# buckbaskin/parakeet_slam

Measured on AMD Instinct MI355X. Metric: particle*landmark EKF updates/sec (whole filter step), higher is better.
Workload: dtype f64

## Files before the change

### parakeet_slam_amd/csrc/pk_api.hip

```cpp
#include <hip/hip_runtime.h>

#include <cmath>
#include <cstdarg>
#include <cstdio>
#include <cstring>
#include <new>
#include <string>
#include <vector>

#include "../../include/parakeet_slam.h"
#include "pk_kernels.hpp"

using namespace pk;

extern "C" {
int pk_download_landmarks(pk_filter* f, int64_t p0, int64_t p1, double* means, double* covs, int32_t* counts);
int pk_upload_landmarks(pk_filter* f, int64_t p0, int64_t p1, const double* means, const double* covs, const int32_t* counts);
}

#ifdef PK_STAMPS
namespace pk { void debug_read_stamps(unsigned long long* out, bool reset); void debug_read_fused_stamps(unsigned long long* out, bool reset); void debug_read_regs_stamps(unsigned long long* out, bool reset); void debug_read_pub_stamps(unsigned long long* out, bool reset); void debug_read_pub_wave_stamps(unsigned long long* out, bool reset); }
#endif

namespace {

thread_local std::string g_last_error;

int fail(int code, const char* fmt, ...) {
  char buf[512];
  va_list ap;
  va_start(ap, fmt);
  vsnprintf(buf, sizeof(buf), fmt, ap);
  va_end(ap);
  g_last_error = buf;
  return code;
}

#define PK_HIP(call)                                                                         \
  do {                                                                                       \
    hipError_t e_ = (call);                                                                  \
    if (e_ != hipSuccess) {                                                                  \
      (void)hipGetLastError();                                                               \
      return fail(e_ == hipErrorOutOfMemory ? PK_ERR_NOMEM : PK_ERR_HIP, "%s failed: %s (%s:%d)", #call, \
                  hipGetErrorString(e_), __FILE__, __LINE__);                                \
    }                                                                                        \
  } while (0)

#define PK_LAUNCH_CHECK(what)                                                                \
  do {                                                                                       \
    hipError_t e_ = hipGetLastError();                                                       \
    if (e_ != hipSuccess)                                                                    \
      return fail(PK_ERR_HIP, "%s: a kernel launch failed: %s", what, hipGetErrorString(e_)); \
  } while (0)

struct TimedSpan {
  int slot;
  hipEvent_t a, b;
};

}

struct AssocLaunch {
  bool fused = false;
  bool regs = false;
  bool retry = false;
  bool big = false;
  BlobGrid grid{};
  int n9 = 0;
  const unsigned char* tables = nullptr;
  bool fast = false;
  const double* blobs = nullptr;
  const double* dir = nullptr;
  const double* exact = nullptr;
  const unsigned short* order = nullptr;
};

struct pk_filter {
  int device = 0;
  hipStream_t own_stream = nullptr;
  hipStream_t stream = nullptr;
  DeviceState d{};
  NoiseD qt{0.1, 0.1, 0.0, 0.0, 0.1, 0.0, 0.1};
  double qt16[16] = {0.1, 0, 0, 0, 0, 0.1, 0, 0, 0, 0, 0.1, 0, 0, 0, 0, 0.1};
  bool qt_dense = false;
  bool dense = false;
  std::vector<double> dense_staged;
  bool map_loaded = false;
  bool src_identity = true;
  int64_t nblocks = 0;
  int64_t device_bytes = 0;
  double* z_dev = nullptr;
  unsigned char* scan_dev = nullptr;
  size_t scan_cap = 0;
  bool gmax_fused = false;
// ... 17 lines not shown
  int64_t bal_loop_keep = -1;
  int assoc_kernel = 0;
  int assoc_dup = 1;
  struct Staged {
    bool valid = false;
    int B = 0;
    unsigned char* st = nullptr;
    int slot = 0;
    BlobGrid g{};
    int n9 = 0;
    bool use_grid = false;
    size_t tab_bytes = 0;
    bool uploaded = false;
  } staged;
  int route = PK_ROUTE_NONE;
  int upload_kernel = 1;
  int fused_step = 1;
  unsigned* bcnt_dev = nullptr;
  uint4* brec_dev = nullptr;
  int64_t bcand_cap = 0;
  int cand_lists = 1;
  int64_t loop_lo = INT64_MIN, loop_hi = INT64_MAX;
  uint4* cand_dev = nullptr;
  int regs_step = 1;
  int pub_step = 1;
  bool flag_folded = false;
  int pub_small = -1;
  int duo_park_limit = -1;
  int duo_on = 0;
  int pub_entry_limit = 0;
  uint4* erec_dev = nullptr;
  uint4* erec_dev2 = nullptr;
  unsigned* binfo_dev = nullptr;
  unsigned char* npass_dev = nullptr;
  unsigned* unm_dev = nullptr;
  int unm_words = 0;
  int64_t unm_cap = 0;
  bool grow_bits = false;
  uint4* prim_dev = nullptr;
  float4* gate4_dev = nullptr;
  uint4* far_dev = nullptr;
  int far_prune = 1;
  unsigned* glist_dev = nullptr;
  struct Split {
    bool active = false;
    AssocLaunch al;
    CandTable cand;
    int B = 0;
    bool reset = false;
  } split;
  bool adopt_local_done = false;
  int pub_ecap = 0;
  int split_reserve_cus = 16;
  int regs_retry = 1;
  int regs_warm = 1;
  int fast_observe = 1;
  uint4* sweep_results = nullptr;
  size_t sweep_cap = 0;
  unsigned* retry_seen = nullptr;
  int64_t retry_rows_min = 0;
  FastHandoff fh{};
  int64_t fh_cap_l = 0, fh_cap_b = 0;
  static constexpr int kRing = 8;
  unsigned char* stage[kRing] = {nullptr};
  hipEvent_t stage_done[kRing] = {nullptr};
  uint64_t upload_seq = 0;
  uint64_t slot_seq[kRing] = {0};
  uint64_t event_seq[kRing] = {0};
  size_t stage_cap = 0;
  int stage_next = 0;
  double* partial = nullptr;
  double* gmax = nullptr;
  double* clocal = nullptr;
  double* totals = nullptr;
  double* offsets = nullptr;
  double* sum = nullptr;
  double* out4 = nullptr;
  double* pose_part = nullptr;
  bool pose_part_ok = false;
  GrowState grow{};
  bool grow_on = false;
  int32_t* anc = nullptr;
  unsigned char* slot_tmp = nullptr;
  uint32_t timing_mask = 0;
  int timing_stride = 1;
  int64_t timing_seen[PK_T_COUNT] = {0};
  std::vector<TimedSpan> pending;
  std::vector<hipEvent_t> pool;
  double ms[PK_T_COUNT] = {0};
  int64_t launches[PK_T_COUNT] = {0};
};

namespace {

template <typename T>
int dev_alloc(pk_filter* f, T** p, size_t n) {
  *p = nullptr;
  if (n == 0) n = 1;
  hipError_t e = hipMalloc((void**)p, n * sizeof(T));
  if (e != hipSuccess) {
    (void)hipGetLastError();
    return fail(PK_ERR_NOMEM, "hipMalloc of %zu bytes failed: %s", n * sizeof(T), hipGetErrorString(e));
  }
  f->device_bytes += (int64_t)(n * sizeof(T));
  return PK_OK;
}

struct Span {
  pk_filter* f;
  int slot;
  hipEvent_t a = nullptr, b = nullptr;
  Span(pk_filter* f_, int slot_) : f(f_), slot(slot_) {
    if (!((f->timing_mask >> slot_) & 1u)) return;
    if (f->timing_seen[slot_]++ % f->timing_stride != 0) return;
    a = take();
    b = take();
    if (a) (void)hipEventRecord(a, f->stream);
  }
  hipEvent_t take() {
    if (!f->pool.empty()) {
      hipEvent_t e = f->pool.back();
      f->pool.pop_back();
      return e;
    }
    hipEvent_t e = nullptr;
    if (hipEventCreate(&e) != hipSuccess) return nullptr;
    return e;
  }
  ~Span() {
    if (!a || !b) return;
    (void)hipEventRecord(b, f->stream);
    f->pending.push_back(TimedSpan{slot, a, b});
  }
};

int drain_timings(pk_filter* f) {
  if (f->pending.empty()) return PK_OK;
  PK_HIP(hipStreamSynchronize(f->stream));
  for (auto& t : f->pending) {
    float ms = 0.f;
    if (hipEventElapsedTime(&ms, t.a, t.b) == hipSuccess) {
      f->ms[t.slot] += ms;
      f->launches[t.slot] += 1;
    }
    f->pool.push_back(t.a);
    f->pool.push_back(t.b);
  }
  f->pending.clear();
  return PK_OK;
}

int use_device(pk_filter* f) {
  PK_HIP(hipSetDevice(f->device));
  return PK_OK;
}

constexpr size_t kCtlBytes = 8 * kGmaxKeys + 64;
int ensure_scan_capacity(pk_filter* f, size_t bytes) {
  if (bytes <= f->scan_cap) return PK_OK;
  PK_HIP(hipStreamSynchronize(f->stream));
  if (f->scan_dev) (void)hipFree(f->scan_dev);
  f->scan_dev = nullptr;
  f->scan_cap = 0;
  const size_t cap = bytes + bytes / 4 + 4096;
  int rc;
  if ((rc = dev_alloc(f, &f->scan_dev, cap))) return rc;
// ... 390 lines not shown
      out->exact = reinterpret_cast<const double*>(f->scan_dev + o_exact);
      const size_t cs_b = ((size_t)(g.ncell + 1) * 2 + 15) & ~(size_t)15;
      out->order = reinterpret_cast<const unsigned short*>(f->scan_dev + o_tab + cs_b + (size_t)B * 16 + (size_t)n9 * 2);
      return PK_OK;
    }
    if (want_fast && !onepass_only && !finalize && f->fast_observe && B > 0 &&
        (sweep ? observe_sweep_plan(f->d, B).grid > 0 : observe_fast_lds_bytes(B) <= kMaxDynLds)) {
      const int slots = (sweep && (B >= 3000 || f->fast_observe == 3)) ? kSweepSlots : kFastSlots;
      if ((rc = ensure_handoff(f, B, slots))) return rc;
      f->fh.slots = slots;
      fh = f->fh;
      fh.n_flagged = ctl_n_flagged(f);
    }
    Span t(f, PK_T_ASSOC);
    CandTable cand;
    if (fh.lmpass && f->cand_lists && f->d.lay.L < 65535) {
      if (!f->cand_dev && (rc = dev_alloc(f, &f->cand_dev, ((size_t)f->d.lay.Lp + kCandSpare) * 3))) return rc;
      launch_summary_partials(f->stream, f->d, f->partial, f->out4);
      launch_candidates(f->stream, f->d, B, reinterpret_cast<const double*>(f->scan_dev + o_exact), 0, f->cand_dev, ctl_cand_over(f),
                        nullptr, nullptr, nullptr, 2 * kCandSlots, f->out4);
      cand.rec = f->cand_dev;
      cand.over = ctl_cand_over(f);
      cand.slots = 2 * kCandSlots;
    }
    launch_assoc_grid(f->stream, f->d, B, g, n9, f->scan_dev + o_tab, reinterpret_cast<const double*>(f->scan_dev + o_exact),
                      f->ids_dev, finalize, fh, cand);
    if (out) {
      out->fast = fh.lmpass != nullptr;
      out->exact = reinterpret_cast<const double*>(f->scan_dev + o_exact);
      const size_t cs_b = ((size_t)(g.ncell + 1) * 2 + 15) & ~(size_t)15;
      out->order = reinterpret_cast<const unsigned short*>(f->scan_dev + o_tab + cs_b + (size_t)B * 16 + (size_t)n9 * 2);
    }
    return PK_OK;
  }
  if (assoc_brute_lds_bytes(B) > kMaxDynLds)
    return fail(PK_ERR_UNSUPPORTED,
                "maximum-likelihood association of %d blobs: neither the colour-grid tables nor the brute-force kernel's "
                "%zu bytes of per-blob state fit the workgroup's %zu bytes of LDS", B, assoc_brute_lds_bytes(B), (size_t)kMaxDynLds);
  Span t(f, PK_T_ASSOC);
  launch_assoc_brute(f->stream, f->d, blobs_dev, dir_dev, B, f->ids_dev);
  return PK_OK;
}

int classify_covariance(const double* cov, int l) {
  double scale = 0.0;
  for (int i = 0; i < 25; ++i) {
    if (!std::isfinite(cov[i])) return fail(PK_ERR_INVALID, "landmark %d: covariance not finite", l + 1);
    if (i % 6 == 0) scale = fmax(scale, fabs(cov[i]));
  }
  const double tol = 1e-9 * (scale > 0 ? scale : 1.0);
  for (int i = 0; i < 2; ++i)
    for (int j = 2; j < 5; ++j)
      if (fabs(cov[i * 5 + j]) > 1e-14 * scale || fabs(cov[j * 5 + i]) > 1e-14 * scale) return 1;
  for (int i = 0; i < 5; ++i)
    for (int j = i + 1; j < 5; ++j)
      if (fabs(cov[i * 5 + j] - cov[j * 5 + i]) > tol) return 1;
  return 0;
}

int check_block_diagonal(const double* cov, int l) {
  double scale = 0.0;
  for (int i = 0; i < 5; ++i) scale = fmax(scale, fabs(cov[i * 6]));
  if (!(scale >= 0.0) || !std::isfinite(scale))
    return fail(PK_ERR_INVALID, "landmark %d: covariance diagonal is not finite", l + 1);
  const double tol = 1e-9 * (scale > 0 ? scale : 1.0);
  for (int i = 0; i < 2; ++i)
    for (int j = 2; j < 5; ++j)
      if (fabs(cov[i * 5 + j]) > 1e-14 * scale || fabs(cov[j * 5 + i]) > 1e-14 * scale)
        return fail(PK_ERR_UNSUPPORTED,
                    "landmark %d: covariance couples position and colour (entry [%d][%d]); the compact "
                    "device layout holds xy 2x2 (+) rgb 3x3 only",
                    l + 1, i, j);
  for (int i = 0; i < 5; ++i)
    for (int j = i + 1; j < 5; ++j) {
      if (!std::isfinite(cov[i * 5 + j])) return fail(PK_ERR_INVALID, "landmark %d: covariance not finite", l + 1);
      if (fabs(cov[i * 5 + j] - cov[j * 5 + i]) > tol)
        return fail(PK_ERR_UNSUPPORTED, "landmark %d: covariance is not symmetric", l + 1);
    }
  return PK_OK;
}

int relayout(pk_filter* f, bool dense, bool keep) {
  if (f->dense == dense) return PK_OK;
  int rc;
  DeviceState& d = f->d;
  const MapLayout old = d.lay;
  const MapLayout neu = MapLayout::make(old.L, sizeof(double), dense ? kDenseFields : (int)F_COUNT_FIELDS);
  const int64_t P = d.P;
  const int L = old.L;
  std::vector<double> means, covs;
  std::vector<int32_t> counts;
  if (keep && L > 0) {
    if ((rc = materialise(f))) return rc;
    if (!dense)
      return fail(PK_ERR_STATE, "relayout: a dense map cannot be folded back into the compact layout");
    try {
      means.resize((size_t)P * L * 5);
      covs.resize((size_t)P * L * 25);
      counts.resize((size_t)P * L);
    } catch (const std::bad_alloc&) {
      return fail(PK_ERR_NOMEM, "relayout: no host memory to stage %lld x %d landmarks for the layout conversion", (long long)P, L);
    }
    if ((rc = pk_download_landmarks(f, 0, P, means.data(), covs.data(), counts.data()))) return rc;
  }
  PK_HIP(hipStreamSynchronize(f->stream));
  for (int i = 0; i < 2; ++i) {
    if (d.map[i]) (void)hipFree(d.map[i]);
    d.map[i] = nullptr;
    f->device_bytes -= (int64_t)((size_t)P * old.slot_bytes);
  }
  if (f->slot_tmp) (void)hipFree(f->slot_tmp);
  f->slot_tmp = nullptr;
  f->device_bytes -= (int64_t)old.slot_bytes;
  d.lay = neu;
  f->dense = dense;
  d.alt = nullptr;
  for (int i = 0; i < 2; ++i) {
    if ((rc = dev_alloc(f, &d.map[i], (size_t)P * neu.slot_bytes))) return rc;
    PK_HIP(hipMemsetAsync(d.map[i], 0, (size_t)P * neu.slot_bytes, f->stream));
  }
  if ((rc = dev_alloc(f, &f->slot_tmp, neu.slot_bytes))) return rc;
  launch_iota(f->stream, d.src[0], P);
  launch_iota(f->stream, d.src[1], P);
  f->src_identity = true;
  d.mcur = 0;
  if (keep && L > 0) {
    const bool was_loaded = f->map_loaded;
    f->map_loaded = true;
    rc = pk_upload_landmarks(f, 0, P, means.data(), covs.data(), counts.data());
    f->map_loaded = was_loaded;
    if (rc) return rc;
  }
  PK_HIP(hipStreamSynchronize(f->stream));
  return PK_OK;
}

}

extern "C" {

int pk_abi_version(void) { return PK_ABI_VERSION; }

const char* pk_status_string(int status) {
  switch (status) {
    case PK_OK: return "ok";
    case PK_ERR_INVALID: return "invalid argument";
    case PK_ERR_HIP: return "HIP runtime error";
    case PK_ERR_STATE: return "invalid call order";
    case PK_ERR_UNSUPPORTED: return "unsupported by the device path";
    case PK_ERR_NOMEM: return "out of memory";
    default: return "unknown status";
  }
}

const char* pk_last_error(void) { return g_last_error.c_str(); }

int pk_device_count(void) {
  int n = 0;
  if (hipGetDeviceCount(&n) != hipSuccess) {
    (void)hipGetLastError();
    return 0;
  }
  return n;
}

int pk_create(int64_t P, int32_t L, int32_t device, pk_filter** out) {
// ... 13 lines not shown
    return code;
  };
  if ((rc = use_device(f))) return bail(rc);
  if (hipStreamCreateWithFlags(&f->own_stream, hipStreamNonBlocking) != hipSuccess)
    return bail(fail(PK_ERR_HIP, "hipStreamCreate failed"));
  f->stream = f->own_stream;
  DeviceState& d = f->d;
  d.P = P;
  d.lay = MapLayout::make(L, sizeof(double));
  d.cur = 0;
  d.mcur = 0;
  f->nblocks = (P + kScanBlock - 1) / kScanBlock;
  for (int i = 0; i < 2 && !rc; ++i) {
    if (!rc) rc = dev_alloc(f, &d.x[i], (size_t)P);
    if (!rc) rc = dev_alloc(f, &d.y[i], (size_t)P);
    if (!rc) rc = dev_alloc(f, &d.h[i], (size_t)P);
    if (!rc) rc = dev_alloc(f, &d.logw[i], (size_t)P);
    if (!rc) rc = dev_alloc(f, &d.src[i], (size_t)P);
    if (!rc) rc = dev_alloc(f, &d.map[i], (size_t)P * d.lay.slot_bytes);
  }
  if (!rc) rc = dev_alloc(f, &d.immutable, (size_t)d.lay.Lp);
  if (!rc) rc = dev_alloc(f, &f->z_dev, (size_t)P * 3);
  if (!rc) rc = dev_alloc(f, &f->partial, (size_t)4 * 1024);
  if (!rc) rc = dev_alloc(f, &f->gmax, 1);
  if (!rc) rc = dev_alloc(f, &f->clocal, (size_t)P);
  if (!rc) rc = dev_alloc(f, &f->totals, (size_t)f->nblocks);
  if (!rc) rc = dev_alloc(f, &f->offsets, (size_t)f->nblocks);
  if (!rc) rc = dev_alloc(f, &f->sum, 1);
  if (!rc) rc = dev_alloc(f, &f->out4, 4);
  if (!rc) rc = dev_alloc(f, &f->pose_part, (size_t)(4 * motion_pose_blocks(P)));
  if (!rc) rc = dev_alloc(f, &f->anc, (size_t)P);
  if (!rc) rc = dev_alloc(f, &f->slot_tmp, d.lay.slot_bytes);
  if (rc) return bail(rc);
  hipError_t e = hipSuccess;
  for (int i = 0; i < 2 && e == hipSuccess; ++i) {
    e = hipMemsetAsync(d.x[i], 0, P * sizeof(double), f->stream);
    if (e == hipSuccess) e = hipMemsetAsync(d.y[i], 0, P * sizeof(double), f->stream);
    if (e == hipSuccess) e = hipMemsetAsync(d.h[i], 0, P * sizeof(double), f->stream);
    if (e == hipSuccess) e = hipMemsetAsync(d.logw[i], 0, P * sizeof(double), f->stream);
    if (e == hipSuccess) e = hipMemsetAsync(d.map[i], 0, (size_t)P * d.lay.slot_bytes, f->stream);
  }
  if (e == hipSuccess) e = hipMemsetAsync(d.immutable, 0, d.lay.Lp, f->stream);
  if (e != hipSuccess) return bail(fail(PK_ERR_HIP, "pk_create: memset failed: %s", hipGetErrorString(e)));
  launch_iota(f->stream, d.src[0], P);
  launch_iota(f->stream, d.src[1], P);
  if (hipStreamSynchronize(f->stream) != hipSuccess) return bail(fail(PK_ERR_HIP, "pk_create: sync failed"));
  f->map_loaded = (L == 0);
  *out = f;
  return PK_OK;
}

int pk_destroy(pk_filter* f) {
  if (!f) return PK_OK;
  (void)hipSetDevice(f->device);
  if (f->stream) (void)hipStreamSynchronize(f->stream);
  for (auto& t : f->pending) {
    (void)hipEventDestroy(t.a);
    (void)hipEventDestroy(t.b);
  }
  for (auto e : f->pool) (void)hipEventDestroy(e);
  DeviceState& d = f->d;
  for (int i = 0; i < 2; ++i) {
    (void)hipFree(d.x[i]);
    (void)hipFree(d.y[i]);
    (void)hipFree(d.h[i]);
    (void)hipFree(d.logw[i]);
    (void)hipFree(d.src[i]);
    (void)hipFree(d.map[i]);
  }
  if (f->scan_dev) (void)hipFree(f->scan_dev);
  for (void* q : {(void*)f->fh.lmpass, (void*)f->fh.bcount, (void*)f->fh.pflag, (void*)f->fh.row_of, (void*)f->sweep_results, (void*)f->cand_dev, (void*)f->bcnt_dev, (void*)f->brec_dev, (void*)f->erec_dev, (void*)f->erec_dev2, (void*)f->binfo_dev, (void*)f->glist_dev, (void*)f->gate4_dev, (void*)f->npass_dev, (void*)f->far_dev, (void*)f->prim_dev, (void*)f->unm_dev})
    if (q) (void)hipFree(q);
  for (int i = 0; i < 2; ++i)
    for (void* q : {(void*)f->grow.hyp[i], (void*)f->grow.cnt[i], (void*)f->grow.slot_id[i]})
      if (q) (void)hipFree(q);
  for (void* q : {(void*)f->g_totals, (void*)f->g_offsets, (void*)f->hi_dev, (void*)f->gl_clocal, (void*)f->gl_totals, (void*)f->gl_offsets, (void*)f->plan_ticket, (void*)f->idx_dev, (void*)f->srcs_dev, (void*)f->rlohi_dev})
    if (q) (void)hipFree(q);
  for (void* q : {(void*)d.logical[0], (void*)d.logical[1], (void*)f->bal.glogw, (void*)f->bal.clocal, (void*)f->bal.totals, (void*)f->bal.offsets,
                  (void*)f->bal.sum, (void*)f->bal.H, (void*)f->bal.cloc, (void*)f->bal.ctot, (void*)f->bal.coff, (void*)f->bal.rel, (void*)f->bal.Hl,
                  (void*)f->bal.alive, (void*)f->bal.bad})
    if (q) (void)hipFree(q);
  void* rest[] = {d.immutable, f->z_dev,  f->ids_dev,
                  f->partial,  f->gmax,   f->clocal,    f->totals,      f->offsets,   f->sum,      f->out4, f->pose_part,
                  f->anc,      f->slot_tmp};
  for (void* p : rest)
    if (p) (void)hipFree(p);
  for (int i = 0; i < pk_filter::kRing; ++i) {
    if (f->stage[i]) (void)hipHostFree(f->stage[i]);
    if (f->stage_done[i]) (void)hipEventDestroy(f->stage_done[i]);
  }
  if (f->retry_seen) (void)hipHostFree(f->retry_seen);
  if (f->own_stream) (void)hipStreamDestroy(f->own_stream);
  delete f;
  return PK_OK;
}

int pk_set_stream(pk_filter* f, void* hip_stream) {
  if (!f) return fail(PK_ERR_INVALID, "pk_set_stream: NULL handle");
  int rc;
  if ((rc = use_device(f))) return rc;
  if ((rc = drain_timings(f))) return rc;
  PK_HIP(hipStreamSynchronize(f->stream));
  f->stream = hip_stream ? (hipStream_t)hip_stream : f->own_stream;
  return PK_OK;
}

int pk_synchronize(pk_filter* f) {
  if (!f) return fail(PK_ERR_INVALID, "pk_synchronize: NULL handle");
  int rc;
  if ((rc = use_device(f))) return rc;
  PK_HIP(hipStreamSynchronize(f->stream));
  return PK_OK;
}

int64_t pk_num_particles(const pk_filter* f) { return f ? f->d.P : -1; }
int32_t pk_num_landmarks(const pk_filter* f) { return f ? f->d.lay.L : -1; }
int64_t pk_device_bytes(const pk_filter* f) { return f ? f->device_bytes : -1; }

int pk_set_measurement_noise(pk_filter* f, const double Qt[16]) {
  if (!f || !Qt) return fail(PK_ERR_INVALID, "pk_set_measurement_noise: NULL argument");
  for (int i = 0; i < 16; ++i)
    if (!std::isfinite(Qt[i])) return fail(PK_ERR_INVALID, "Qt is not finite");
  double scale = 0;
  for (int i = 0; i < 4; ++i) scale = fmax(scale, fabs(Qt[i * 5]));
  bool coupled = false;
  for (int j = 1; j < 4; ++j)
    if (fabs(Qt[j]) > 1e-14 * scale || fabs(Qt[j * 4]) > 1e-14 * scale) coupled = true;
  for (int i = 1; i < 4; ++i)
    for (int j = i + 1; j < 4; ++j)
      if (fabs(Qt[i * 4 + j] - Qt[j * 4 + i]) > 1e-9 * (scale > 0 ? scale : 1.0)) coupled = true;
  int rc;
  if ((rc = use_device(f))) return rc;
  if (coupled && !f->dense && (rc = relayout(f, true, f->map_loaded))) return rc;
  for (int i = 0; i < 16; ++i) f->qt16[i] = Qt[i];
  f->qt_dense = coupled;
  f->qt = NoiseD{Qt[0], Qt[5], 0.5 * (Qt[6] + Qt[9]), 0.5 * (Qt[7] + Qt[13]), Qt[10], 0.5 * (Qt[11] + Qt[14]), Qt[15]};
  return PK_OK;
}

int pk_upload_map(pk_filter* f, const double* means, const double* covs, const uint8_t* immutable) {
  if (!f) return fail(PK_ERR_INVALID, "pk_upload_map: NULL handle");
  const MapLayout& lay = f->d.lay;
  const int L = lay.L;
  if (L > 0 && (!means || !covs)) return fail(PK_ERR_INVALID, "pk_upload_map: NULL means/covs");
  int rc;
  if ((rc = use_device(f))) return rc;
  bool need_dense = f->qt_dense;
  for (int l = 0; l < L; ++l) {
    for (int i = 0; i < 5; ++i)
      if (!std::isfinite(means[l * 5 + i])) return fail(PK_ERR_INVALID, "landmark %d: mean is not finite", l + 1);
    const int c = classify_covariance(covs + (size_t)l * 25, l);
    if (c < 0) return c;
    need_dense |= c == 1;
  }
  if ((rc = relayout(f, need_dense, false))) return rc;
  std::vector<unsigned char> slot(lay.slot_bytes, 0);
  std::vector<unsigned char> imm((size_t)lay.Lp, 0);
  for (int l = 0; l < L; ++l) {
    pack_landmark(lay, slot.data(), l, means + (size_t)l * 5, covs + (size_t)l * 25);
    imm[l] = immutable ? (immutable[l] != 0) : 0;
  }
  PK_HIP(hipMemcpyAsync(f->slot_tmp, slot.data(), lay.slot_bytes, hipMemcpyHostToDevice, f->stream));
  PK_HIP(hipMemcpyAsync(f->d.immutable, imm.data(), imm.size(), hipMemcpyHostToDevice, f->stream));
  launch_broadcast_slot(f->stream, f->d, f->slot_tmp);
  PK_HIP(hipStreamSynchronize(f->stream));
  f->src_identity = true;
  f->map_loaded = true;
  return PK_OK;
}

int pk_upload_poses(pk_filter* f, const double* xyhw) {
  if (f) f->pose_part_ok = false;
  if (!f || !xyhw) return fail(PK_ERR_INVALID, "pk_upload_poses: NULL argument");
  int rc;
  if ((rc = use_device(f))) return rc;
  const int64_t P = f->d.P;
  std::vector<double> soa((size_t)P * 4);
  for (int64_t i = 0; i < P; ++i) {
    soa[i] = xyhw[4 * i];
    soa[P + i] = xyhw[4 * i + 1];
    soa[2 * P + i] = xyhw[4 * i + 2];
    double w = xyhw[4 * i + 3];
    if (!(w >= 0.0) || !std::isfinite(w)) return fail(PK_ERR_INVALID, "pk_upload_poses: weight of particle %lld is negative, infinite or NaN", (long long)i);
    soa[3 * P + i] = std::log(w);
  }
  const int c = f->d.cur;
  PK_HIP(hipMemcpyAsync(f->d.x[c], soa.data(), P * 8, hipMemcpyHostToDevice, f->stream));
  PK_HIP(hipMemcpyAsync(f->d.y[c], soa.data() + P, P * 8, hipMemcpyHostToDevice, f->stream));
  PK_HIP(hipMemcpyAsync(f->d.h[c], soa.data() + 2 * P, P * 8, hipMemcpyHostToDevice, f->stream));
  PK_HIP(hipMemcpyAsync(f->d.logw[c], soa.data() + 3 * P, P * 8, hipMemcpyHostToDevice, f->stream));
  PK_HIP(hipStreamSynchronize(f->stream));
  f->gmax_fused = false;
  return PK_OK;
}

int pk_upload_pose(pk_filter* f, int64_t p, const double xyhw[4]) {
  if (!f || !xyhw) return fail(PK_ERR_INVALID, "pk_upload_pose: NULL argument");
  if (p < 0 || p >= f->d.P) return fail(PK_ERR_INVALID, "pk_upload_pose: particle %lld of %lld", (long long)p, (long long)f->d.P);
  for (int i = 0; i < 3; ++i)
    if (!std::isfinite(xyhw[i])) return fail(PK_ERR_INVALID, "pk_upload_pose: pose component %d is not finite", i);
  if (!(xyhw[3] >= 0.0) || !std::isfinite(xyhw[3])) return fail(PK_ERR_INVALID, "pk_upload_pose: the weight is negative, infinite or NaN");
  int rc;
  if ((rc = use_device(f))) return rc;
  f->pose_part_ok = false;
  const double v4[4] = {xyhw[0], xyhw[1], xyhw[2], std::log(xyhw[3])};
  const int c = f->d.cur;
  double* const dst[4] = {f->d.x[c] + p, f->d.y[c] + p, f->d.h[c] + p, f->d.logw[c] + p};
  for (int i = 0; i < 4; ++i) PK_HIP(hipMemcpyAsync(dst[i], &v4[i], 8, hipMemcpyHostToDevice, f->stream));
  PK_HIP(hipStreamSynchronize(f->stream));
  f->gmax_fused = false;
  return PK_OK;
}

int pk_download_poses(pk_filter* f, double* xyhw) {
  if (!f || !xyhw) return fail(PK_ERR_INVALID, "pk_download_poses: NULL argument");
  int rc;
  if ((rc = use_device(f))) return rc;
  const int64_t P = f->d.P;
  std::vector<double> soa((size_t)P * 4);
  const int c = f->d.cur;
  PK_HIP(hipMemcpyAsync(soa.data(), f->d.x[c], P * 8, hipMemcpyDeviceToHost, f->stream));
  PK_HIP(hipMemcpyAsync(soa.data() + P, f->d.y[c], P * 8, hipMemcpyDeviceToHost, f->stream));
  PK_HIP(hipMemcpyAsync(soa.data() + 2 * P, f->d.h[c], P * 8, hipMemcpyDeviceToHost, f->stream));
  PK_HIP(hipMemcpyAsync(soa.data() + 3 * P, f->d.logw[c], P * 8, hipMemcpyDeviceToHost, f->stream));
  PK_HIP(hipStreamSynchronize(f->stream));
  for (int64_t i = 0; i < P; ++i) {
    xyhw[4 * i] = soa[i];
    xyhw[4 * i + 1] = soa[P + i];
    xyhw[4 * i + 2] = soa[2 * P + i];
    xyhw[4 * i + 3] = std::exp(soa[3 * P + i]);
  }
  return PK_OK;
}

int pk_download_log_weights(pk_filter* f, double* logw) {
  if (!f || !logw) return fail(PK_ERR_INVALID, "pk_download_log_weights: NULL argument");
  int rc;
  if ((rc = use_device(f))) return rc;
  PK_HIP(hipMemcpyAsync(logw, f->d.logw[f->d.cur], (size_t)f->d.P * sizeof(double), hipMemcpyDeviceToHost, f->stream));
  PK_HIP(hipStreamSynchronize(f->stream));
  return PK_OK;
}

int pk_download_landmarks(pk_filter* f, int64_t p0, int64_t p1, double* means, double* covs, int32_t* counts) {
  if (!f) return fail(PK_ERR_INVALID, "pk_download_landmarks: NULL handle");
  if (p0 < 0 || p1 < p0 || p1 > f->d.P) return fail(PK_ERR_INVALID, "pk_download_landmarks: bad particle range");
  if (!f->map_loaded) return fail(PK_ERR_STATE, "pk_download_landmarks: no map uploaded");
  int rc;
  if ((rc = use_device(f))) return rc;
  if ((rc = materialise(f))) return rc;
  const MapLayout& lay = f->d.lay;
  const int L = lay.L;
  const int64_t chunk = std::max<int64_t>(1, (int64_t)(64u << 20) / (int64_t)lay.slot_bytes);
  std::vector<unsigned char> host((size_t)std::min<int64_t>(chunk, p1 - p0) * lay.slot_bytes);
  for (int64_t q0 = p0; q0 < p1; q0 += chunk) {
    int64_t q1 = std::min(p1, q0 + chunk);
    PK_HIP(hipMemcpyAsync(host.data(), f->d.map[f->d.mcur] + (size_t)q0 * lay.slot_bytes,
                          (size_t)(q1 - q0) * lay.slot_bytes, hipMemcpyDeviceToHost, f->stream));
    PK_HIP(hipStreamSynchronize(f->stream));
    for (int64_t q = q0; q < q1; ++q) {
      const unsigned char* slot = host.data() + (size_t)(q - q0) * lay.slot_bytes;
      const int32_t* cnt = reinterpret_cast<const int32_t*>(slot + lay.count_off);
      for (int l = 0; l < L; ++l) {
        size_t o = (size_t)(q - p0) * L + l;
        unpack_landmark(lay, slot, l, means ? means + o * 5 : nullptr, covs ? covs + o * 25 : nullptr);
        if (counts) counts[o] = cnt[l];
      }
    }
  }
  return PK_OK;
}

int pk_upload_landmarks(pk_filter* f, int64_t p0, int64_t p1, const double* means, const double* covs,
                        const int32_t* counts) {
  if (!f) return fail(PK_ERR_INVALID, "pk_upload_landmarks: NULL handle");
  if (p0 < 0 || p1 < p0 || p1 > f->d.P) return fail(PK_ERR_INVALID, "pk_upload_landmarks: bad particle range");
  if (!f->map_loaded) return fail(PK_ERR_STATE, "pk_upload_landmarks: no map uploaded");
  int rc;
  if ((rc = use_device(f))) return rc;
  if ((rc = materialise(f))) return rc;
  const int L = f->d.lay.L;
  if (means)
    for (int64_t o = 0; o < (p1 - p0) * L * 5; ++o)
      if (!std::isfinite(means[o])) return fail(PK_ERR_INVALID, "pk_upload_landmarks: mean of landmark %d not finite", (int)((o / 5) % L) + 1);
  if (covs) {
    bool need_dense = false;
    for (int64_t o = 0; o < (p1 - p0) * L; ++o) {
      const int c = classify_covariance(covs + (size_t)o * 25, (int)(o % L));
      if (c < 0) return c;
      need_dense |= c == 1;
    }
    if (need_dense && !f->dense && (rc = relayout(f, true, true))) return rc;
  }
  const MapLayout& lay = f->d.lay;
  const int64_t chunk = std::max<int64_t>(1, (int64_t)(64u << 20) / (int64_t)lay.slot_bytes);
  std::vector<unsigned char> host;
  try {
    host.resize((size_t)std::min<int64_t>(chunk, p1 - p0) * lay.slot_bytes);
  } catch (const std::bad_alloc&) {
    return fail(PK_ERR_NOMEM, "pk_upload_landmarks: no host memory for the staging buffer");
  }
  for (int64_t q0 = p0; q0 < p1; q0 += chunk) {
    int64_t q1 = std::min(p1, q0 + chunk);
    unsigned char* dev = f->d.map[f->d.mcur] + (size_t)q0 * lay.slot_bytes;
    PK_HIP(hipMemcpyAsync(host.data(), dev, (size_t)(q1 - q0) * lay.slot_bytes, hipMemcpyDeviceToHost, f->stream));
    PK_HIP(hipStreamSynchronize(f->stream));
    for (int64_t q = q0; q < q1; ++q) {
      unsigned char* slot = host.data() + (size_t)(q - q0) * lay.slot_bytes;
      int32_t* cnt = reinterpret_cast<int32_t*>(slot + lay.count_off);
      for (int l = 0; l < L; ++l) {
        size_t o = (size_t)(q - p0) * L + l;
        double m[5], c[25];
        unpack_landmark(lay, slot, l, m, c);
        pack_landmark(lay, slot, l, means ? means + o * 5 : m, covs ? covs + o * 25 : c);
        if (counts) cnt[l] = counts[o];
      }
    }
    PK_HIP(hipMemcpyAsync(dev, host.data(), (size_t)(q1 - q0) * lay.slot_bytes, hipMemcpyHostToDevice, f->stream));
    PK_HIP(hipStreamSynchronize(f->stream));
  }
  return PK_OK;
}

int pk_reset_weights(pk_filter* f) {
  if (!f) return fail(PK_ERR_INVALID, "pk_reset_weights: NULL handle");
  int rc;
  if ((rc = use_device(f))) return rc;
  launch_reset_weights(f->stream, f->d);
  f->gmax_fused = false;
  PK_LAUNCH_CHECK("pk_reset_weights");
  return PK_OK;
}

static size_t staged_upload_bytes(const pk_filter::Staged& sg) {
  const size_t o_exact = kCtlBytes + (size_t)sg.B * 6 * sizeof(double);
  const size_t o_tab = o_exact + (size_t)sg.B * 6 * sizeof(double);
  return sg.use_grid ? o_tab + sg.tab_bytes : o_exact;
}

int pk_motion(pk_filter* f, double v, double w, double dt, const double* z, uint64_t seed, uint64_t draw) {
  if (!f) return fail(PK_ERR_INVALID, "pk_motion: NULL handle");
  if (!std::isfinite(v) || !std::isfinite(w) || !std::isfinite(dt)) return fail(PK_ERR_INVALID, "pk_motion: non-finite control");
  int rc;
  if ((rc = use_device(f))) return rc;
  const double* zd = nullptr;
  if (z) {
    PK_HIP(hipMemcpyAsync(f->z_dev, z, (size_t)f->d.P * 3 * sizeof(double), hipMemcpyHostToDevice, f->stream));
    PK_HIP(hipStreamSynchronize(f->stream));
    zd = f->z_dev;
  }
  Span t(f, PK_T_MOTION);
  pk_filter::Staged& sg = f->staged;
  if (!z && sg.valid && !sg.uploaded && f->upload_kernel) {
    void* dev_view = nullptr;
    if (hipHostGetDevicePointer(&dev_view, sg.st, 0) == hipSuccess && dev_view) {
      launch_motion(f->stream, f->d, v, w, dt, nullptr, seed, draw, 0, f->scan_dev, dev_view, staged_upload_bytes(sg), f->pose_part);
      f->pose_part_ok = true;
// ... 465 lines not shown
    if ((rc = onepass_prepare(f, sp.al, sp.B, &sp.cand, p1 > p0 ? p0 : 0))) return rc;
    sp.active = true;
  } else if (!sp.active) {
    return fail(PK_ERR_STATE, "pk_observe_staged_range: no split observe in progress (first = 1)");
  }
  ObserveExtras ex;
  ex.reset = sp.reset;
  ex.gmax_key = ctl_gmax_key(f);
  if (p1 > p0 && (rc = onepass_launch(f, sp.al, sp.B, ex, sp.cand, p0, p1, (first && !last) ? f->split_reserve_cus : 0))) {
    sp.active = false;
    return rc;
  }
  if (last) {
    sp.active = false;
    if ((rc = onepass_finish(f, sp.al, sp.B, ex, sp.cand))) return rc;
    PK_LAUNCH_CHECK("pk_observe_staged_range");
    f->src_identity = true;
    f->d.alt = nullptr;
    f->gmax_fused = true;
  }
  return PK_OK;
}

int pk_motion_range(pk_filter* f, double v, double w, double dt, uint64_t seed, uint64_t draw, int64_t p0, int64_t p1) {
  if (f) f->pose_part_ok = false;
  if (!f) return fail(PK_ERR_INVALID, "pk_motion_range: NULL handle");
  if (!std::isfinite(v) || !std::isfinite(w) || !std::isfinite(dt)) return fail(PK_ERR_INVALID, "pk_motion_range: non-finite control");
  if (p0 < 0 || p1 < p0 || p1 > f->d.P) return fail(PK_ERR_INVALID, "pk_motion_range: bad particle range [%lld, %lld)", (long long)p0, (long long)p1);
  int rc;
  if ((rc = use_device(f))) return rc;
  Span t(f, PK_T_MOTION);
  launch_motion_range(f->stream, f->d, v, w, dt, seed, draw, p0, p1);
  PK_LAUNCH_CHECK("pk_motion_range");
  return PK_OK;
}

int pk_associate(pk_filter* f, const double* blobs, int32_t B, int32_t* ids_out) {
  if (!f || !ids_out) return fail(PK_ERR_INVALID, "pk_associate: NULL argument");
  if (B < 0 || (B > 0 && !blobs)) return fail(PK_ERR_INVALID, "pk_associate: bad blobs");
  if (!f->map_loaded) return fail(PK_ERR_STATE, "pk_associate: no map uploaded (pk_upload_map)");
  if (B == 0) return PK_OK;
  int rc;
  if ((rc = use_device(f))) return rc;
  for (int i = 0; i < 4 * B; ++i)
    if (!std::isfinite(blobs[i])) return fail(PK_ERR_INVALID, "pk_associate: blob %d is not finite", i / 4);
  if (f->dense) return dense_observe(f, blobs, B, nullptr, ids_out, false, false);
  if ((rc = enqueue_association(f, blobs, B, true, false, nullptr))) return rc;
  PK_LAUNCH_CHECK("pk_associate");
  PK_HIP(hipMemcpyAsync(ids_out, f->ids_dev, (size_t)f->d.P * B * 4, hipMemcpyDeviceToHost, f->stream));
  PK_HIP(hipStreamSynchronize(f->stream));
  return PK_OK;
}

int pk_set_option(pk_filter* f, const char* name, int64_t value) {
  if (!f || !name) return fail(PK_ERR_INVALID, "pk_set_option: NULL argument");
  if (!strcmp(name, "assoc_kernel")) {
    if (value != 0 && value != 1) return fail(PK_ERR_INVALID, "assoc_kernel: 0 (colour grid) or 1 (brute force)");
    f->assoc_kernel = (int)value;
    return PK_OK;
  }
  if (!strcmp(name, "fast_observe")) {
    if (value < 0 || value > 3)
      return fail(PK_ERR_INVALID, "fast_observe: 0 (general kernels), 1 (default), 2 (always the sweep kernel) or 3 (... with eight slots)");
    f->fast_observe = (int)value;
    return PK_OK;
  }
  if (!strcmp(name, "timing_stride")) {
    if (value < 1 || value > 1000000) return fail(PK_ERR_INVALID, "timing_stride: 1 .. 1000000");
    f->timing_stride = (int)value;
    return PK_OK;
  }
  if (!strcmp(name, "upload_kernel")) {
    f->upload_kernel = value != 0;
    return PK_OK;
  }
  if (!strcmp(name, "fused_step")) {
    f->fused_step = value != 0;
    return PK_OK;
  }
  if (!strcmp(name, "cand_lists")) {
    f->cand_lists = value != 0;
    return PK_OK;
  }
  if (!strcmp(name, "pub_step")) {
    f->pub_step = value != 0;
    return PK_OK;
  }
  if (!strcmp(name, "pub_small")) {
    f->pub_small = value < 0 ? -1 : (value != 0 ? 1 : 0);
    return PK_OK;
  }
  if (!strcmp(name, "far_prune")) {
    f->far_prune = value != 0;
    return PK_OK;
  }
  if (!strcmp(name, "pub_duo")) {
    if (value < 0 || value > 2) return fail(PK_ERR_INVALID, "pub_duo: 0 (off), 1 (two 512-lane workgroups per CU) or 2 (three 256-lane workgroups per CU)");
    f->duo_on = (int)value;
    return PK_OK;
  }
  if (!strcmp(name, "pub_duo_park_limit")) {
    if (value < -1 || value > 65535) return fail(PK_ERR_INVALID, "pub_duo_park_limit: -1 (what LDS holds) .. 65535");
    f->duo_park_limit = (int)value;
    return PK_OK;
  }
  if (!strcmp(name, "pub_entry_limit")) {
    if (value < 0 || value > 65534) return fail(PK_ERR_INVALID, "pub_entry_limit: 0 (what LDS holds) .. 65534");
    f->pub_entry_limit = (int)value;
    return PK_OK;
  }
  if (!strcmp(name, "regs_step")) {
    f->regs_step = value != 0;
    return PK_OK;
  }
  if (!strcmp(name, "split_loopback_lo") || !strcmp(name, "split_loopback_hi")) {
    if (value < 0 || value > f->d.P) return fail(PK_ERR_INVALID, "%s: 0..P", name);
    (name[15] == 'l' ? f->loop_lo : f->loop_hi) = value;
    return PK_OK;
  }
  if (!strcmp(name, "balanced_loopback_keep")) {
    if (value < -1 || value > f->d.P) return fail(PK_ERR_INVALID, "balanced_loopback_keep: -1 (off) .. P");
    f->bal_loop_keep = value;
    return PK_OK;
  }
  if (!strcmp(name, "split_reserve_cus")) {
    if (value < 0 || value > 128) return fail(PK_ERR_INVALID, "split_reserve_cus: 0..128");
    f->split_reserve_cus = (int)value;
    return PK_OK;
  }
  if (!strcmp(name, "regs_retry")) {
    if (value != 0 && value != 1) return fail(PK_ERR_INVALID, "regs_retry: 0 or 1");
    f->regs_retry = (int)value;
    return PK_OK;
  }
  if (!strcmp(name, "regs_warm")) {
    if (value < 0 || value > 2) return fail(PK_ERR_INVALID, "regs_warm: 0 (off), 1 (mean rows) or 2 (whole slot)");
    f->regs_warm = (int)value;
    return PK_OK;
  }
  if (!strcmp(name, "assoc_dup")) {
    f->assoc_dup = value != 0;
    return PK_OK;
  }
  if (!strcmp(name, "observe_landmarks_per_lane")) {
    if (value < 0 || value > 2) return fail(PK_ERR_INVALID, "observe_landmarks_per_lane: 0 (default), 1 or 2");
    g_observe_nv = (int)value;
    return PK_OK;
  }
  return fail(PK_ERR_INVALID, "pk_set_option: unknown option '%s'", name);
}

int pk_resample(pk_filter* f, double u, int32_t weight_domain, int64_t* ancestors_out) {
  if (f) f->pose_part_ok = false;
  if (!f) return fail(PK_ERR_INVALID, "pk_resample: NULL handle");
  if (!(u >= 0.0 && u < 1.0)) return fail(PK_ERR_INVALID, "pk_resample: u = %g outside [0,1)", u);
  if (weight_domain != PK_WEIGHTS_LINEAR && weight_domain != PK_WEIGHTS_LOG)
    return fail(PK_ERR_INVALID, "pk_resample: weight_domain %d", weight_domain);
  if (f->split.active) return fail(PK_ERR_STATE, "pk_resample: a split observe is in progress (half the particles observed)");
  if (f->d.logical[0]) return fail(PK_ERR_STATE, "pk_resample: the balanced placement is active on this filter (its slots carry logical indices): resample through pk_shard_plan_balanced_dev / pk_shard_adopt_balanced_dev");
  int rc;
  if ((rc = use_device(f))) return rc;
  DeviceState& d = f->d;
  {
    Span t(f, PK_T_WEIGHTS);
    const unsigned long long* key = nullptr;
    if (weight_domain == PK_WEIGHTS_LOG) {
// ... 8 lines not shown
    } else {
      launch_scan_blocks(f->stream, f->totals, f->nblocks, f->offsets, f->sum);
      launch_ancestors(f->stream, f->clocal, f->totals, f->offsets, f->sum, f->nblocks, d.P, d.P, u, 0, d.P, f->anc, &d);
    }
  }
  if (f->grow_on) launch_grow_gather(f->stream, f->grow, f->anc, d.P);
  PK_LAUNCH_CHECK("pk_resample");
  f->src_identity = false;
  f->gmax_fused = false;
  if (ancestors_out) {
    std::vector<int32_t> a((size_t)d.P);
    PK_HIP(hipMemcpyAsync(a.data(), f->anc, (size_t)d.P * 4, hipMemcpyDeviceToHost, f->stream));
    PK_HIP(hipStreamSynchronize(f->stream));
    for (int64_t i = 0; i < d.P; ++i) ancestors_out[i] = a[i];
  }
  return PK_OK;
}

int pk_summary(pk_filter* f, double out[3]) {
  if (!f || !out) return fail(PK_ERR_INVALID, "pk_summary: NULL argument");
  int rc;
  if ((rc = use_device(f))) return rc;
  {
    Span t(f, PK_T_SUMMARY);
    launch_summary_partials(f->stream, f->d, f->partial, f->out4);
  }
  double s[4];
  PK_HIP(hipMemcpyAsync(s, f->out4, sizeof(s), hipMemcpyDeviceToHost, f->stream));
  PK_HIP(hipStreamSynchronize(f->stream));
  const double n = (double)f->d.P;
  out[0] = s[0] / n;
  out[1] = s[1] / n;
  out[2] = std::atan2(s[2], s[3]);
  return PK_OK;
}

int pk_pose_sums(pk_filter* f, double out[4]) {
  if (!f || !out) return fail(PK_ERR_INVALID, "pk_pose_sums: NULL argument");
  int rc;
  if ((rc = use_device(f))) return rc;
  {
    Span t(f, PK_T_SUMMARY);
    launch_summary_partials(f->stream, f->d, f->partial, f->out4);
  }
  PK_HIP(hipMemcpyAsync(out, f->out4, 4 * sizeof(double), hipMemcpyDeviceToHost, f->stream));
  PK_HIP(hipStreamSynchronize(f->stream));
  return PK_OK;
}

int pk_step(pk_filter* f, double v, double w, double dt, const double* z, uint64_t seed, uint64_t draw,
            const double* blobs, int32_t B, const int32_t* ids, double u, int32_t weight_domain) {
  int rc;
  if (f && !f->dense && !f->grow_on && !z && !ids && B > 0 && blobs && f->map_loaded && f->upload_kernel && std::isfinite(v) && std::isfinite(w) &&
      std::isfinite(dt)) {
    bool finite = true;
    for (int i = 0; i < 4 * B && finite; ++i) finite = std::isfinite(blobs[i]);
    if (finite && B <= 65535) {
      if ((rc = use_device(f))) return rc;
      if ((rc = stage_ml_scan(f, blobs, B))) return rc;
      pk_filter::Staged& sg = f->staged;
      void* dev_view = nullptr;
      if (hipHostGetDevicePointer(&dev_view, sg.st, 0) == hipSuccess && dev_view) {
        {
          Span t(f, PK_T_MOTION);
          launch_motion(f->stream, f->d, v, w, dt, nullptr, seed, draw, 0, f->scan_dev, dev_view, staged_upload_bytes(sg), f->pose_part);
      f->pose_part_ok = true;
        }
        sg.uploaded = true;
        f->gmax_fused = false;
        if ((rc = note_upload(f, sg.slot))) return rc;
        const double* staged_blobs = reinterpret_cast<const double*>(sg.st + kCtlBytes);
        if ((rc = observe_impl(f, staged_blobs, B, nullptr, nullptr, true))) return rc;
        return pk_resample(f, u, weight_domain, nullptr);
      }
      (void)hipGetLastError();
    }
  }
  if ((rc = pk_motion(f, v, w, dt, z, seed, draw))) return rc;
  if ((rc = observe_impl(f, blobs, B, ids, nullptr, true))) return rc;
  return pk_resample(f, u, weight_domain, nullptr);
}

int pk_grow_enable(pk_filter* f, int32_t preset_landmarks, int32_t reading_capacity, double pair_threshold) {
  if (!f) return fail(PK_ERR_INVALID, "pk_grow_enable: NULL handle");
  const int L = f->d.lay.L;
  if (preset_landmarks < 0 || preset_landmarks >= L)
    return fail(PK_ERR_INVALID, "pk_grow_enable: %d preset landmarks leave no spare slot among the filter's %d", preset_landmarks, L);
  if (reading_capacity < 1 || reading_capacity > 65536) return fail(PK_ERR_INVALID, "pk_grow_enable: reading_capacity %d outside 1..65536", reading_capacity);
  if (!(pair_threshold >= 0.0)) return fail(PK_ERR_INVALID, "pk_grow_enable: pair_threshold %g", pair_threshold);
  if (f->grow_on) return fail(PK_ERR_STATE, "pk_grow_enable: already enabled on this filter");
  if (f->dense)
    return fail(PK_ERR_STATE, "pk_grow_enable: the bookkeeping kernel writes the compact landmark layout; this filter is on the dense one "
                              "(a covariance or Qt that couples position and colour)");
  int rc;
  if ((rc = use_device(f))) return rc;
  GrowState& g = f->grow;
  g.L0 = preset_landmarks;
  g.S = L - preset_landmarks;
  g.R = reading_capacity;
  g.pair_threshold = pair_threshold;
  g.cur = 0;
  const size_t P = (size_t)f->d.P;
  for (int i = 0; i < 2; ++i) {
    if ((rc = dev_alloc(f, &g.hyp[i], P * g.R * 8))) return rc;
    if ((rc = dev_alloc(f, &g.cnt[i], P * 4))) return rc;
    if ((rc = dev_alloc(f, &g.slot_id[i], P * g.S))) return rc;
  }
  std::vector<int32_t> c0(P * 4, 0);
  for (size_t p = 0; p < P; ++p) c0[4 * p + 2] = preset_landmarks + 1;
  PK_HIP(hipMemcpyAsync(g.cnt[0], c0.data(), P * 16, hipMemcpyHostToDevice, f->stream));
  PK_HIP(hipStreamSynchronize(f->stream));
  f->grow_on = true;
  return PK_OK;
}

static int grow_range(pk_filter* f, const char* who, int64_t p0, int64_t p1) {
  if (!f) return fail(PK_ERR_INVALID, "%s: NULL handle", who);
  if (!f->grow_on) return fail(PK_ERR_STATE, "%s: pk_grow_enable was not called on this filter", who);
  if (p0 < 0 || p1 < p0 || p1 > f->d.P) return fail(PK_ERR_INVALID, "%s: particles [%lld, %lld) of %lld", who, (long long)p0, (long long)p1, (long long)f->d.P);
  return use_device(f);
}

int pk_grow_download(pk_filter* f, int64_t p0, int64_t p1, int32_t* counters, double* readings, int32_t* slot_ids) {
  int rc;
  if ((rc = grow_range(f, "pk_grow_download", p0, p1))) return rc;
  const GrowState& g = f->grow;
  const size_t n = (size_t)(p1 - p0);
  if (n == 0) return PK_OK;
  if (counters) PK_HIP(hipMemcpyAsync(counters, g.cnt[g.cur] + 4 * p0, n * 16, hipMemcpyDeviceToHost, f->stream));
  if (readings) PK_HIP(hipMemcpyAsync(readings, g.hyp[g.cur] + (size_t)p0 * g.R * 8, n * g.R * 64, hipMemcpyDeviceToHost, f->stream));
  if (slot_ids) PK_HIP(hipMemcpyAsync(slot_ids, g.slot_id[g.cur] + (size_t)p0 * g.S, n * g.S * 4, hipMemcpyDeviceToHost, f->stream));
  PK_HIP(hipStreamSynchronize(f->stream));
  return PK_OK;
}

int pk_grow_upload(pk_filter* f, int64_t p0, int64_t p1, const int32_t* counters, const double* readings, const int32_t* slot_ids) {
  int rc;
  if ((rc = grow_range(f, "pk_grow_upload", p0, p1))) return rc;
  const GrowState& g = f->grow;
  const size_t n = (size_t)(p1 - p0);
  if (n == 0) return PK_OK;
  if (counters)
    for (size_t i = 0; i < n; ++i)
      if (counters[4 * i] < 0 || counters[4 * i] > g.R || counters[4 * i + 1] < 0 || counters[4 * i + 1] > g.S || counters[4 * i + 3] < 0)
        return fail(PK_ERR_INVALID, "pk_grow_upload: particle %lld: %d readings of %d, %d spare slots of %d in use", (long long)(p0 + (int64_t)i),
                    counters[4 * i], g.R, counters[4 * i + 1], g.S);
  if (counters) PK_HIP(hipMemcpyAsync(g.cnt[g.cur] + 4 * p0, counters, n * 16, hipMemcpyHostToDevice, f->stream));
  if (readings) PK_HIP(hipMemcpyAsync(g.hyp[g.cur] + (size_t)p0 * g.R * 8, readings, n * g.R * 64, hipMemcpyHostToDevice, f->stream));
  if (slot_ids) PK_HIP(hipMemcpyAsync(g.slot_id[g.cur] + (size_t)p0 * g.S, slot_ids, n * g.S * 4, hipMemcpyHostToDevice, f->stream));
  PK_HIP(hipStreamSynchronize(f->stream));
  return PK_OK;
}

int pk_grow_shape(const pk_filter* f, int32_t* preset_landmarks, int32_t* spare_slots, int32_t* reading_capacity) {
  if (!f) return fail(PK_ERR_INVALID, "pk_grow_shape: NULL handle");
  if (preset_landmarks) *preset_landmarks = f->grow_on ? f->grow.L0 : 0;
  if (spare_slots) *spare_slots = f->grow_on ? f->grow.S : 0;
  if (reading_capacity) *reading_capacity = f->grow_on ? f->grow.R : 0;
  return PK_OK;
}

int pk_shard_max_logw(pk_filter* f, double* max_logw) {
  if (!f || !max_logw) return fail(PK_ERR_INVALID, "pk_shard_max_logw: NULL argument");
  int rc;
  if ((rc = use_device(f))) return rc;
  launch_block_max(f->stream, f->d, f->partial, f->gmax);
  PK_HIP(hipMemcpyAsync(max_logw, f->gmax, sizeof(double), hipMemcpyDeviceToHost, f->stream));
  PK_HIP(hipStreamSynchronize(f->stream));
  return PK_OK;
}

int64_t pk_shard_num_blocks(const pk_filter* f) { return f ? f->nblocks : -1; }

int pk_shard_block_totals(pk_filter* f, double gmax, int32_t weight_domain, double* totals) {
  if (!f || !totals) return fail(PK_ERR_INVALID, "pk_shard_block_totals: NULL argument");
  int rc;
  if ((rc = use_device(f))) return rc;
  PK_HIP(hipMemcpyAsync(f->gmax, &gmax, sizeof(double), hipMemcpyHostToDevice, f->stream));
  launch_scan_local(f->stream, f->d, f->gmax, weight_domain, f->clocal, f->totals);
  PK_HIP(hipMemcpyAsync(totals, f->totals, (size_t)f->nblocks * sizeof(double), hipMemcpyDeviceToHost, f->stream));
  PK_HIP(hipStreamSynchronize(f->stream));
  return PK_OK;
}

int pk_set_shard(pk_filter* f, int64_t global_offset) {
  if (!f || global_offset < 0) return fail(PK_ERR_INVALID, "pk_set_shard: bad argument");
  f->d.global_offset = global_offset;
  return PK_OK;
}

int pk_shard_offspring(pk_filter* f, const double* global_totals, int64_t n_global_blocks, int64_t first_block,
                       int64_t global_particles, double u, int32_t last_shard, int64_t* slot_hi) {
  if (!f || !global_totals || !slot_hi) return fail(PK_ERR_INVALID, "pk_shard_offspring: NULL argument");
  if (!(u >= 0.0 && u < 1.0)) return fail(PK_ERR_INVALID, "pk_shard_offspring: u = %g outside [0,1)", u);
  if (first_block < 0 || first_block + f->nblocks > n_global_blocks || global_particles < f->d.P)
    return fail(PK_ERR_INVALID, "pk_shard_offspring: shard [%lld, +%lld) does not fit %lld global blocks",
                (long long)first_block, (long long)f->nblocks, (long long)n_global_blocks);
  int rc;
  if ((rc = use_device(f))) return rc;
  if (n_global_blocks > f->gblocks_cap) {
    PK_HIP(hipStreamSynchronize(f->stream));
    if (f->g_totals) (void)hipFree(f->g_totals);
    if (f->g_offsets) (void)hipFree(f->g_offsets);
    f->g_totals = f->g_offsets = nullptr;
    f->gblocks_cap = 0;
    if ((rc = dev_alloc(f, &f->g_totals, (size_t)n_global_blocks))) return rc;
    if ((rc = dev_alloc(f, &f->g_offsets, (size_t)n_global_blocks + 1))) return rc;
    f->gblocks_cap = n_global_blocks;
  }
  if (!f->hi_dev && (rc = dev_alloc(f, &f->hi_dev, (size_t)f->d.P + 1))) return rc;
  PK_HIP(hipMemcpyAsync(f->g_totals, global_totals, (size_t)n_global_blocks * sizeof(double), hipMemcpyHostToDevice,
                        f->stream));
  {
    Span t(f, PK_T_WEIGHTS);
    launch_scan_blocks(f->stream, f->g_totals, n_global_blocks, f->g_offsets, f->sum);
    launch_offspring(f->stream, f->clocal, f->g_offsets, f->sum, first_block, f->d.P, global_particles, u,
                     last_shard ? 1 : 0, f->hi_dev);
  }
  PK_HIP(hipMemcpyAsync(slot_hi, f->hi_dev, ((size_t)f->d.P + 1) * sizeof(int64_t), hipMemcpyDeviceToHost, f->stream));
  PK_HIP(hipStreamSynchronize(f->stream));
  return PK_OK;
}

static size_t record_stride(const pk_filter* f) { return kPoseRecordBytes + f->d.lay.slot_bytes + (f->grow_on ? grow_tail_bytes(f->grow) : 0); }
int64_t pk_particle_bytes(const pk_filter* f) { return f ? (int64_t)record_stride(f) : -1; }

int pk_pack_particles(pk_filter* f, const int64_t* local_idx, int64_t n, void* dev_buf) {
  if (!f || n < 0 || (n > 0 && (!local_idx || !dev_buf))) return fail(PK_ERR_INVALID, "pk_pack_particles: bad argument");
  if (f->grow_on) return fail(PK_ERR_STATE, "pk_pack_particles: the new-landmark bookkeeping (pk_grow_enable) travels with the balanced placement only (pk_shard_*_balanced_dev)");
  if (n > f->d.P) return fail(PK_ERR_INVALID, "pk_pack_particles: %lld records from %lld particles", (long long)n, (long long)f->d.P);
  for (int64_t i = 0; i < n; ++i)
    if (local_idx[i] < 0 || local_idx[i] >= f->d.P) return fail(PK_ERR_INVALID, "pk_pack_particles: index %lld out of range", (long long)local_idx[i]);
  if (n == 0) return PK_OK;
  int rc;
  if ((rc = use_device(f))) return rc;
  if (!f->idx_dev && (rc = dev_alloc(f, &f->idx_dev, (size_t)f->d.P))) return rc;
  PK_HIP(hipMemcpyAsync(f->idx_dev, local_idx, (size_t)n * sizeof(int64_t), hipMemcpyHostToDevice, f->stream));
  {
    Span t(f, PK_T_RESAMPLE);
    launch_pack(f->stream, f->d, f->idx_dev, n, static_cast<unsigned char*>(dev_buf));
  }
  PK_HIP(hipStreamSynchronize(f->stream));
  return PK_OK;
}

int pk_adopt_particles(pk_filter* f, const int64_t* src, const void* dev_buf, int64_t n_received) {
  if (f) f->pose_part_ok = false;
  if (!f || !src || n_received < 0 || (n_received > 0 && !dev_buf)) return fail(PK_ERR_INVALID, "pk_adopt_particles: bad argument");
  if (f->grow_on) return fail(PK_ERR_STATE, "pk_adopt_particles: the new-landmark bookkeeping (pk_grow_enable) travels with the balanced placement only (pk_shard_*_balanced_dev)");
  const int64_t P = f->d.P;
  for (int64_t k = 0; k < P; ++k)
    if (src[k] >= P || src[k] < -n_received) return fail(PK_ERR_INVALID, "pk_adopt_particles: src[%lld] = %lld out of range", (long long)k, (long long)src[k]);
  if (f->d.logical[0]) return fail(PK_ERR_STATE, "pk_adopt_particles: the balanced placement is active on this filter (its slots carry logical indices): resample through pk_shard_plan_balanced_dev / pk_shard_adopt_balanced_dev");
  int rc;
  if ((rc = use_device(f))) return rc;
  if (f->d.alt) {
    f->src_identity = false;
    if ((rc = materialise(f))) return rc;
  }
  if (!f->srcs_dev && (rc = dev_alloc(f, &f->srcs_dev, (size_t)P))) return rc;
  PK_HIP(hipMemcpyAsync(f->srcs_dev, src, (size_t)P * sizeof(int64_t), hipMemcpyHostToDevice, f->stream));
  {
    Span t(f, PK_T_RESAMPLE);
    launch_adopt(f->stream, f->d, f->srcs_dev, static_cast<const unsigned char*>(dev_buf));
  }
  if (n_received == 0) f->d.alt = nullptr;
  f->src_identity = false;
  f->gmax_fused = false;
  PK_HIP(hipStreamSynchronize(f->stream));
  return PK_OK;
}

int pk_shard_max_logw_dev(pk_filter* f, double* dev_out) {
  if (!f || !dev_out) return fail(PK_ERR_INVALID, "pk_shard_max_logw_dev: NULL argument");
  int rc;
  if ((rc = use_device(f))) return rc;
  Span t(f, PK_T_WEIGHTS);
  if (f->gmax_fused)
    launch_keys_max(f->stream, ctl_gmax_key(f), dev_out);
  else
    launch_block_max(f->stream, f->d, f->partial, dev_out);
  return PK_OK;
}

int pk_shard_block_totals_dev(pk_filter* f, const double* dev_gmax, int32_t weight_domain, double* dev_totals) {
  if (!f || !dev_totals || (weight_domain == PK_WEIGHTS_LOG && !dev_gmax))
    return fail(PK_ERR_INVALID, "pk_shard_block_totals_dev: NULL argument");
  int rc;
  if ((rc = use_device(f))) return rc;
  Span t(f, PK_T_WEIGHTS);
  launch_scan_local(f->stream, f->d, dev_gmax ? dev_gmax : f->gmax, weight_domain, f->clocal, dev_totals);
  return PK_OK;
}

int pk_shard_plan_dev(pk_filter* f, const double* dev_global_totals, int64_t n_global_blocks, int64_t first_block,
                      int64_t global_particles, double u, int32_t last_shard, int32_t world, int64_t* dev_ranges) {
  if (!f || !dev_global_totals || !dev_ranges || world < 1) return fail(PK_ERR_INVALID, "pk_shard_plan_dev: bad argument");
  if (!(u >= 0.0 && u < 1.0)) return fail(PK_ERR_INVALID, "pk_shard_plan_dev: u = %g outside [0,1)", u);
  if (first_block < 0 || first_block + f->nblocks > n_global_blocks || global_particles != (int64_t)world * f->d.P)
    return fail(PK_ERR_INVALID, "pk_shard_plan_dev: shard geometry (%lld blocks from %lld of %lld, %lld particles x %d)",
                (long long)f->nblocks, (long long)first_block, (long long)n_global_blocks, (long long)f->d.P, world);
  int rc;
  if ((rc = use_device(f))) return rc;
  if (n_global_blocks > f->gblocks_cap) {
    PK_HIP(hipStreamSynchronize(f->stream));
    if (f->g_totals) (void)hipFree(f->g_totals);
    if (f->g_offsets) (void)hipFree(f->g_offsets);
    f->g_totals = f->g_offsets = nullptr;
    f->gblocks_cap = 0;
    if ((rc = dev_alloc(f, &f->g_totals, (size_t)n_global_blocks))) return rc;
    if ((rc = dev_alloc(f, &f->g_offsets, (size_t)n_global_blocks + 1))) return rc;
    f->gblocks_cap = n_global_blocks;
  }
  if (!f->hi_dev && (rc = dev_alloc(f, &f->hi_dev, (size_t)f->d.P + 1))) return rc;
  if (!f->plan_ticket) {
    if ((rc = dev_alloc(f, &f->plan_ticket, (size_t)1))) return rc;
    PK_HIP(hipMemsetAsync(f->plan_ticket, 0, sizeof(unsigned), f->stream));
  }
  Span t(f, PK_T_WEIGHTS);
  if (n_global_blocks <= kAncestorsScanMaxBlocks) {
    launch_offspring_plan(f->stream, f->clocal, dev_global_totals, n_global_blocks, first_block, f->d.P, global_particles, u,
                          last_shard ? 1 : 0, f->hi_dev, world, dev_ranges, f->plan_ticket);
    return PK_OK;
  }
  launch_scan_blocks(f->stream, dev_global_totals, n_global_blocks, f->g_offsets, f->sum);
  launch_offspring(f->stream, f->clocal, f->g_offsets, f->sum, first_block, f->d.P, global_particles, u,
                   last_shard ? 1 : 0, f->hi_dev);
  launch_shard_ranges(f->stream, f->hi_dev, f->d.P, world, dev_ranges);
  return PK_OK;
// ... 9 lines not shown

int pk_shard_plan_global_dev(pk_filter* f, const double* dev_global_logw, int64_t global_particles, const double* dev_gmax,
                             int32_t weight_domain, double u, int32_t last_shard, int32_t world, int64_t* dev_ranges) {
  if (!f || !dev_global_logw || !dev_ranges || world < 1) return fail(PK_ERR_INVALID, "pk_shard_plan_global_dev: bad argument");
  if (weight_domain == PK_WEIGHTS_LOG && !dev_gmax) return fail(PK_ERR_INVALID, "pk_shard_plan_global_dev: NULL maximum");
  if (!(u >= 0.0 && u < 1.0)) return fail(PK_ERR_INVALID, "pk_shard_plan_global_dev: u = %g outside [0,1)", u);
  const int64_t P = f->d.P, goff = f->d.global_offset;
  if (global_particles != (int64_t)world * P || goff < 0 || goff + P > global_particles)
    return fail(PK_ERR_INVALID, "pk_shard_plan_global_dev: shard [%lld, +%lld) of %lld particles, world %d", (long long)goff,
                (long long)P, (long long)global_particles, world);
  int rc;
  if ((rc = use_device(f))) return rc;
  const int64_t nbg = (global_particles + kScanBlock - 1) / kScanBlock;
  if (global_particles > f->gl_cap) {
    PK_HIP(hipStreamSynchronize(f->stream));
    for (double** q : {&f->gl_clocal, &f->gl_totals, &f->gl_offsets}) {
      if (*q) (void)hipFree(*q);
      *q = nullptr;
    }
    f->gl_cap = 0;
    if ((rc = dev_alloc(f, &f->gl_clocal, (size_t)global_particles))) return rc;
    if ((rc = dev_alloc(f, &f->gl_totals, (size_t)nbg))) return rc;
    if ((rc = dev_alloc(f, &f->gl_offsets, (size_t)nbg + 1))) return rc;
    f->gl_cap = global_particles;
  }
  if (!f->hi_dev && (rc = dev_alloc(f, &f->hi_dev, (size_t)P + 1))) return rc;
  Span t(f, PK_T_WEIGHTS);
  launch_scan_local_of(f->stream, dev_global_logw, global_particles, dev_gmax ? dev_gmax : f->gmax, weight_domain, f->gl_clocal,
                       f->gl_totals);
  launch_scan_blocks(f->stream, f->gl_totals, nbg, f->gl_offsets, f->sum);
  launch_offspring_global(f->stream, f->gl_clocal, f->gl_offsets, f->sum, goff, P, global_particles, u, last_shard ? 1 : 0,
                          f->hi_dev);
  launch_shard_ranges(f->stream, f->hi_dev, P, world, dev_ranges);
  PK_LAUNCH_CHECK("pk_shard_plan_global_dev");
  return PK_OK;
}

int pk_shard_download_offspring(pk_filter* f, int64_t* slot_hi) {
  if (!f || !slot_hi) return fail(PK_ERR_INVALID, "pk_shard_download_offspring: NULL argument");
  if (!f->hi_dev) return fail(PK_ERR_STATE, "pk_shard_download_offspring: no plan yet");
  int rc;
  if ((rc = use_device(f))) return rc;
  PK_HIP(hipMemcpyAsync(slot_hi, f->hi_dev, ((size_t)f->d.P + 1) * sizeof(int64_t), hipMemcpyDeviceToHost, f->stream));
  PK_HIP(hipStreamSynchronize(f->stream));
  return PK_OK;
}

int pk_shard_pack_dev(pk_filter* f, const int64_t* ranges, int32_t world, int32_t rank, void* dev_buf) {
  if (f && f->grow_on) return fail(PK_ERR_STATE, "pk_shard_pack_dev: the new-landmark bookkeeping (pk_grow_enable) travels with the balanced placement only (pk_shard_*_balanced_dev)");
  if (!f || !ranges || world < 1 || rank < 0 || rank >= world) return fail(PK_ERR_INVALID, "pk_shard_pack_dev: bad argument");
  if (!f->hi_dev) return fail(PK_ERR_STATE, "pk_shard_pack_dev: call pk_shard_plan_dev first");
  int rc;
  if ((rc = use_device(f))) return rc;
  const int64_t P = f->d.P;
  const size_t stride = kPoseRecordBytes + f->d.lay.slot_bytes;
  int64_t rec = 0;
  Span t(f, PK_T_RESAMPLE);
  for (int d = 0; d < world; ++d) {
    if (d == rank) continue;
    const int64_t j0 = ranges[2 * d], j1 = ranges[2 * d + 1];
    if (j0 < 0 || j1 < j0 || j1 > P) return fail(PK_ERR_INVALID, "pk_shard_pack_dev: range [%lld, %lld) for rank %d", (long long)j0, (long long)j1, d);
    if (j1 > j0 && !dev_buf) return fail(PK_ERR_INVALID, "pk_shard_pack_dev: NULL buffer");
    launch_pack_range(f->stream, f->d, f->hi_dev, j0, j1 - j0, (int64_t)d * P, (int64_t)(d + 1) * P,
                      static_cast<unsigned char*>(dev_buf) + (size_t)rec * stride);
    rec += j1 - j0;
  }
  return PK_OK;
}

int pk_shard_pack_slots_dev(pk_filter* f, int64_t j0, int64_t j1, int64_t slot_lo, int64_t slot_hi, void* dev_buf) {
  if (f && f->grow_on) return fail(PK_ERR_STATE, "pk_shard_pack_slots_dev: the new-landmark bookkeeping (pk_grow_enable) travels with the balanced placement only (pk_shard_*_balanced_dev)");
  if (!f || j0 < 0 || j1 < j0 || j1 > f->d.P || slot_hi < slot_lo) return fail(PK_ERR_INVALID, "pk_shard_pack_slots_dev: bad argument");
  if (!f->hi_dev) return fail(PK_ERR_STATE, "pk_shard_pack_slots_dev: call pk_shard_plan_dev first");
  if (j1 > j0 && !dev_buf) return fail(PK_ERR_INVALID, "pk_shard_pack_slots_dev: NULL buffer");
  int rc;
  if ((rc = use_device(f))) return rc;
  Span t(f, PK_T_RESAMPLE);
  launch_pack_range(f->stream, f->d, f->hi_dev, j0, j1 - j0, slot_lo, slot_hi, static_cast<unsigned char*>(dev_buf));
  PK_LAUNCH_CHECK("pk_shard_pack_slots_dev");
  return PK_OK;
}

int pk_shard_adopt_dev(pk_filter* f, int32_t rank, const void* dev_recv, int64_t n_received) {
  if (f && f->grow_on) return fail(PK_ERR_STATE, "pk_shard_adopt_dev: the new-landmark bookkeeping (pk_grow_enable) travels with the balanced placement only (pk_shard_*_balanced_dev)");
  if (f) f->pose_part_ok = false;
  if (!f || rank < 0 || n_received < 0 || (n_received > 0 && !dev_recv)) return fail(PK_ERR_INVALID, "pk_shard_adopt_dev: bad argument");
  if (!f->hi_dev) return fail(PK_ERR_STATE, "pk_shard_adopt_dev: call pk_shard_plan_dev first");
  if (f->d.logical[0]) return fail(PK_ERR_STATE, "pk_shard_adopt_dev: the balanced placement is active on this filter (its slots carry logical indices): resample through pk_shard_plan_balanced_dev / pk_shard_adopt_balanced_dev");
  int rc;
  if ((rc = use_device(f))) return rc;
  if (f->d.alt) {
    f->src_identity = false;
    if ((rc = materialise(f))) return rc;
  }
  if (n_received > f->rlohi_cap) {
    PK_HIP(hipStreamSynchronize(f->stream));
    if (f->rlohi_dev) (void)hipFree(f->rlohi_dev);
    f->rlohi_dev = nullptr;
    f->rlohi_cap = 0;
    if ((rc = dev_alloc(f, &f->rlohi_dev, (size_t)(2 * n_received + 2 * n_received / 4 + 16)))) return rc;
    f->rlohi_cap = n_received + n_received / 4;
  }
  Span t(f, PK_T_RESAMPLE);
  launch_adopt_dev(f->stream, f->d, f->hi_dev, (int64_t)rank * f->d.P, static_cast<const unsigned char*>(dev_recv),
                   n_received, f->rlohi_dev);
  f->src_identity = false;
  f->gmax_fused = false;
  return PK_OK;
}

int pk_shard_adopt_local_dev(pk_filter* f, int32_t rank) {
  if (f && f->grow_on) return fail(PK_ERR_STATE, "pk_shard_adopt_local_dev: the new-landmark bookkeeping (pk_grow_enable) travels with the balanced placement only (pk_shard_*_balanced_dev)");
  if (f) f->pose_part_ok = false;
  if (!f || rank < 0) return fail(PK_ERR_INVALID, "pk_shard_adopt_local_dev: bad argument");
  if (!f->hi_dev) return fail(PK_ERR_STATE, "pk_shard_adopt_local_dev: call pk_shard_plan_dev first");
  if (f->d.logical[0]) return fail(PK_ERR_STATE, "pk_shard_adopt_local_dev: the balanced placement is active on this filter (its slots carry logical indices): resample through pk_shard_plan_balanced_dev / pk_shard_adopt_balanced_dev");
  int rc;
  if ((rc = use_device(f))) return rc;
  if (f->d.alt) {
    f->src_identity = false;
    if ((rc = materialise(f))) return rc;
  }
  Span t(f, PK_T_RESAMPLE);
  const int64_t base = (int64_t)rank * f->d.P;
  launch_adopt_dev(f->stream, f->d, f->hi_dev, base, nullptr, 0, nullptr, 1, f->loop_lo == INT64_MIN ? INT64_MIN : base + f->loop_lo,
                   f->loop_hi == INT64_MAX ? INT64_MAX : base + f->loop_hi);
  f->src_identity = false;
  f->gmax_fused = false;
  f->adopt_local_done = true;
  return PK_OK;
}

int pk_shard_adopt_remote_dev(pk_filter* f, int32_t rank, const void* dev_recv, int64_t n_received) {
  if (f && f->grow_on) return fail(PK_ERR_STATE, "pk_shard_adopt_remote_dev: the new-landmark bookkeeping (pk_grow_enable) travels with the balanced placement only (pk_shard_*_balanced_dev)");
  if (f) f->pose_part_ok = false;
  if (!f || rank < 0 || n_received < 0 || (n_received > 0 && !dev_recv)) return fail(PK_ERR_INVALID, "pk_shard_adopt_remote_dev: bad argument");
  if (!f->hi_dev) return fail(PK_ERR_STATE, "pk_shard_adopt_remote_dev: call pk_shard_plan_dev first");
  if (!f->adopt_local_done)
    return fail(PK_ERR_STATE, "pk_shard_adopt_remote_dev: pk_shard_adopt_local_dev first (it makes the new generation current)");
  f->adopt_local_done = false;
  int rc;
  if ((rc = use_device(f))) return rc;
  if (n_received > f->rlohi_cap) {
    PK_HIP(hipStreamSynchronize(f->stream));
    if (f->rlohi_dev) (void)hipFree(f->rlohi_dev);
    f->rlohi_dev = nullptr;
    f->rlohi_cap = 0;
    if ((rc = dev_alloc(f, &f->rlohi_dev, (size_t)(2 * n_received + 2 * n_received / 4 + 16)))) return rc;
    f->rlohi_cap = n_received + n_received / 4;
  }
  Span t(f, PK_T_RESAMPLE);
  const int64_t base = (int64_t)rank * f->d.P;
  launch_adopt_dev(f->stream, f->d, f->hi_dev, base, static_cast<const unsigned char*>(dev_recv), n_received, f->rlohi_dev, 2,
                   f->loop_lo == INT64_MIN ? INT64_MIN : base + f->loop_lo, f->loop_hi == INT64_MAX ? INT64_MAX : base + f->loop_hi);
  f->loop_lo = INT64_MIN;
  f->loop_hi = INT64_MAX;
  return PK_OK;
}

int pk_shard_local_span_dev(pk_filter* f, int64_t* dev_out2) {
  if (!f || !dev_out2) return fail(PK_ERR_INVALID, "pk_shard_local_span_dev: NULL argument");
  if (!f->hi_dev) return fail(PK_ERR_STATE, "pk_shard_local_span_dev: no plan yet");
  int rc;
  if ((rc = use_device(f))) return rc;
  PK_HIP(hipMemcpyAsync(dev_out2, f->hi_dev, sizeof(int64_t), hipMemcpyDeviceToDevice, f->stream));
  PK_HIP(hipMemcpyAsync(dev_out2 + 1, f->hi_dev + f->d.P, sizeof(int64_t), hipMemcpyDeviceToDevice, f->stream));
  return PK_OK;
}

static int ensure_logical(pk_filter* f) {
  DeviceState& d = f->d;
  if (d.logical[0]) return PK_OK;
  int rc;
  int64_t *a = nullptr, *b = nullptr;
  if ((rc = dev_alloc(f, &a, (size_t)d.P))) return rc;
  if ((rc = dev_alloc(f, &b, (size_t)d.P))) {
    (void)hipFree(a);
    return rc;
  }
  launch_iota64(f->stream, a, d.P, d.global_offset);
  launch_iota64(f->stream, b, d.P, d.global_offset);
  d.logical[0] = a;
  d.logical[1] = b;
  return PK_OK;
}

int pk_shard_reset_placement(pk_filter* f) {
  if (!f) return fail(PK_ERR_INVALID, "pk_shard_reset_placement: NULL handle");
  int rc;
  if ((rc = use_device(f))) return rc;
  if (f->d.logical[0]) launch_iota64(f->stream, f->d.logical[f->d.cur], f->d.P, f->d.global_offset);
  return PK_OK;
}

int pk_shard_download_logical(pk_filter* f, int64_t* logical) {
  if (!f || !logical) return fail(PK_ERR_INVALID, "pk_shard_download_logical: NULL argument");
  int rc;
  if ((rc = use_device(f))) return rc;
  if (!f->d.logical[0]) {
    for (int64_t j = 0; j < f->d.P; ++j) logical[j] = f->d.global_offset + j;
    return PK_OK;
  }
  PK_HIP(hipMemcpyAsync(logical, f->d.logical[f->d.cur], (size_t)f->d.P * sizeof(int64_t), hipMemcpyDeviceToHost, f->stream));
  PK_HIP(hipStreamSynchronize(f->stream));
  return PK_OK;
}

int pk_shard_upload_logical(pk_filter* f, const int64_t* logical) {
  if (!f || !logical) return fail(PK_ERR_INVALID, "pk_shard_upload_logical: NULL argument");
  for (int64_t j = 0; j < f->d.P; ++j)
    if (logical[j] < 0 || logical[j] >= ((int64_t)1 << 31)) return fail(PK_ERR_INVALID, "pk_shard_upload_logical: logical[%lld] = %lld", (long long)j, (long long)logical[j]);
  if (f->split.active) return fail(PK_ERR_STATE, "pk_shard_upload_logical: a split observe is in progress");
  int rc;
  if ((rc = use_device(f))) return rc;
  if ((rc = ensure_logical(f))) return rc;
  PK_HIP(hipMemcpyAsync(f->d.logical[f->d.cur], logical, (size_t)f->d.P * sizeof(int64_t), hipMemcpyHostToDevice, f->stream));
// ... 66 lines not shown
    if (!b.alive && (rc = dev_alloc(f, &b.alive, (size_t)P))) return rc;
    if (!b.bad) {
      if ((rc = dev_alloc(f, &b.bad, (size_t)1))) return rc;
      PK_HIP(hipMemsetAsync(b.bad, 0, sizeof(int), f->stream));
    }
    b.cap = Pg;
  }
  Span t(f, PK_T_WEIGHTS);
  launch_bal_plan(f->stream, f->d, dev_global_state, Pg, world, rank, dev_gmax ? dev_gmax : f->gmax, weight_domain, u, b, dev_table);
  PK_LAUNCH_CHECK("pk_shard_plan_balanced_dev");
  f->bal_m = -1;
  return PK_OK;
}

int pk_shard_download_balanced_offspring(pk_filter* f, int64_t global_particles, int64_t* H) {
  if (!f || !H) return fail(PK_ERR_INVALID, "pk_shard_download_balanced_offspring: NULL argument");
  if (!f->bal.H || global_particles != f->bal.cap) return fail(PK_ERR_STATE, "pk_shard_download_balanced_offspring: no balanced plan of %lld particles yet", (long long)global_particles);
  int rc;
  if ((rc = use_device(f))) return rc;
  PK_HIP(hipMemcpyAsync(H, f->bal.H, ((size_t)global_particles + 1) * sizeof(int64_t), hipMemcpyDeviceToHost, f->stream));
  PK_HIP(hipStreamSynchronize(f->stream));
  return PK_OK;
}

static int balanced_row_check(const int64_t* table, int world, int64_t P, const char* who) {
  const int row = 2 * world + 4;
  int64_t e_sum = 0, d_sum = 0;
  for (int r = 0; r < world; ++r) {
    const int64_t n = table[(size_t)r * row + 2 * world], m = table[(size_t)r * row + 2 * world + 1];
    if (n < 0 || m != (n < P ? n : P) || table[(size_t)r * row + 2 * world + 2] != e_sum || table[(size_t)r * row + 2 * world + 3] != d_sum)
      return fail(PK_ERR_INVALID, "%s: the plan table is not one pk_shard_plan_balanced_dev wrote (rank %d)", who, r);
    e_sum += n - m;
    d_sum += P - m;
    for (int d = 0; d < world; ++d) {
      const int64_t a0 = table[(size_t)r * row + 2 * d], a1 = table[(size_t)r * row + 2 * d + 1];
      if (a0 < 0 || a1 < a0 || a1 > P) return fail(PK_ERR_INVALID, "%s: range [%lld, %lld) from rank %d to rank %d", who, (long long)a0, (long long)a1, r, d);
    }
  }
  if (e_sum != d_sum) return fail(PK_ERR_INVALID, "%s: excess %lld and free slots %lld differ", who, (long long)e_sum, (long long)d_sum);
  return PK_OK;
}

int pk_shard_pack_balanced_dev(pk_filter* f, const int64_t* table, int32_t world, int32_t rank, void* dev_buf) {
  if (!f || !table || world < 1 || world > 64 || rank < 0 || rank >= world) return fail(PK_ERR_INVALID, "pk_shard_pack_balanced_dev: bad argument");
  if (!f->bal.rel || !f->d.logical[0]) return fail(PK_ERR_STATE, "pk_shard_pack_balanced_dev: call pk_shard_plan_balanced_dev first");
  int rc;
  const int64_t P = f->d.P;
  if ((rc = balanced_row_check(table, world, P, "pk_shard_pack_balanced_dev"))) return rc;
  if ((rc = use_device(f))) return rc;
  const int row = 2 * world + 4;
  const size_t stride = record_stride(f);
  const int64_t ebase_s = table[(size_t)rank * row + 2 * world + 2];
  int64_t rec = 0;
  Span t(f, PK_T_RESAMPLE);
  for (int d = 0; d < world; ++d) {
    if (d == rank) continue;
    const int64_t a0 = table[(size_t)rank * row + 2 * d], a1 = table[(size_t)rank * row + 2 * d + 1];
    if (a1 <= a0) continue;
    if (!dev_buf) return fail(PK_ERR_INVALID, "pk_shard_pack_balanced_dev: NULL buffer");
    const int64_t m_d = table[(size_t)d * row + 2 * world + 1], dbase_d = table[(size_t)d * row + 2 * world + 3];
    launch_bal_pack(f->stream, f->d, f->bal, a0, a1 - a0, ebase_s, dbase_d, P - m_d, m_d,
                    static_cast<unsigned char*>(dev_buf) + (size_t)rec * stride, stride, f->grow_on ? &f->grow : nullptr);
    rec += a1 - a0;
  }
  PK_LAUNCH_CHECK("pk_shard_pack_balanced_dev");
  return PK_OK;
}

int pk_shard_pack_balanced_loop_dev(pk_filter* f, int64_t keep, int64_t a0, int64_t a1, void* dev_buf) {
  if (!f || keep < 0 || keep > f->d.P || a0 < 0 || a1 < a0 || a1 > f->d.P || (a1 > a0 && !dev_buf))
    return fail(PK_ERR_INVALID, "pk_shard_pack_balanced_loop_dev: bad argument");
  if (!f->bal.rel || !f->d.logical[0]) return fail(PK_ERR_STATE, "pk_shard_pack_balanced_loop_dev: call pk_shard_plan_balanced_dev first");
  int rc;
  if ((rc = use_device(f))) return rc;
  Span t(f, PK_T_RESAMPLE);
  launch_bal_pack(f->stream, f->d, f->bal, a0, a1 - a0, 0, 0, f->d.P - keep, keep, static_cast<unsigned char*>(dev_buf), record_stride(f),
                  f->grow_on ? &f->grow : nullptr, keep);
  PK_LAUNCH_CHECK("pk_shard_pack_balanced_loop_dev");
  return PK_OK;
}

int pk_shard_adopt_balanced_dev(pk_filter* f, const int64_t* table, int32_t world, int32_t rank, const void* dev_recv,
                                int64_t n_received, int32_t mode) {
  if (f) f->pose_part_ok = false;
  if (!f || !table || world < 1 || world > 64 || rank < 0 || rank >= world || n_received < 0 || mode < 0 || mode > 2 ||
      (n_received > 0 && !dev_recv))
    return fail(PK_ERR_INVALID, "pk_shard_adopt_balanced_dev: bad argument");
  if (!f->bal.rel || !f->d.logical[0]) return fail(PK_ERR_STATE, "pk_shard_adopt_balanced_dev: call pk_shard_plan_balanced_dev first");
  if (f->grow_on && mode != 0) return fail(PK_ERR_STATE, "pk_shard_adopt_balanced_dev: the new-landmark bookkeeping (pk_grow_enable) is adopted whole (mode 0)");
  int rc;
  const int64_t P = f->d.P;
  if ((rc = balanced_row_check(table, world, P, "pk_shard_adopt_balanced_dev"))) return rc;
  const int row = 2 * world + 4;
  int64_t m = table[(size_t)rank * row + 2 * world + 1];
  const bool loop = f->bal_loop_keep >= 0 && world == 1;
  if (loop) m = f->bal_loop_keep < m ? f->bal_loop_keep : m;
  if (mode == 2) {
    if (!f->adopt_local_done) return fail(PK_ERR_STATE, "pk_shard_adopt_balanced_dev: mode 1 first (it makes the new generation current)");
    f->adopt_local_done = false;
  }
  if (mode != 1) {
    int64_t expect = 0;
    for (int s = 0; s < world; ++s)
      if (s != rank) expect += table[(size_t)s * row + 2 * rank + 1] - table[(size_t)s * row + 2 * rank];
    if (!loop && expect != n_received) return fail(PK_ERR_INVALID, "pk_shard_adopt_balanced_dev: %lld records received, the plan sends %lld", (long long)n_received, (long long)expect);
    if (m < P && n_received == 0) return fail(PK_ERR_INVALID, "pk_shard_adopt_balanced_dev: %lld free slots and no records", (long long)(P - m));
    f->bal_loop_keep = -1;
  }
  if ((rc = use_device(f))) return rc;
  if (mode != 2 && f->d.alt) {
    f->src_identity = false;
    if ((rc = materialise(f))) return rc;
  }
  if (3 * n_received > 2 * f->rlohi_cap) {
    PK_HIP(hipStreamSynchronize(f->stream));
    if (f->rlohi_dev) (void)hipFree(f->rlohi_dev);
    f->rlohi_dev = nullptr;
    f->rlohi_cap = 0;
    if ((rc = dev_alloc(f, &f->rlohi_dev, (size_t)(3 * n_received + 3 * n_received / 4 + 16)))) return rc;
    f->rlohi_cap = (3 * n_received + 3 * n_received / 4) / 2;
  }
  Span t(f, PK_T_RESAMPLE);
  const size_t stride = record_stride(f);
  launch_bal_adopt(f->stream, f->d, f->bal, m, static_cast<const unsigned char*>(dev_recv), n_received, f->rlohi_dev, mode, stride,
                   f->grow_on ? f->anc : nullptr);
  if (f->grow_on)
    launch_grow_gather(f->stream, f->grow, f->anc, P, static_cast<const unsigned char*>(dev_recv), stride, kPoseRecordBytes + f->d.lay.slot_bytes);
  PK_LAUNCH_CHECK("pk_shard_adopt_balanced_dev");
  f->src_identity = false;
  f->gmax_fused = false;
  if (mode == 1) f->adopt_local_done = true;
  return PK_OK;
}

int pk_shard_balanced_errors(pk_filter* f, int64_t* count) {
  if (!f || !count) return fail(PK_ERR_INVALID, "pk_shard_balanced_errors: NULL argument");
  *count = 0;
  if (!f->bal.bad) return PK_OK;
  int rc;
  if ((rc = use_device(f))) return rc;
  int v = 0;
  PK_HIP(hipMemcpyAsync(&v, f->bal.bad, sizeof(int), hipMemcpyDeviceToHost, f->stream));
  PK_HIP(hipStreamSynchronize(f->stream));
  *count = v;
  return PK_OK;
}

int pk_probe(int32_t device, const double pose[3], const double mean[5], const double cov[25],
             const double blob[4], const double Qt[16], double* out) {
  if (!pose || !mean || !cov || !blob || !Qt || !out) return fail(PK_ERR_INVALID, "pk_probe: NULL argument");
  int ndev = pk_device_count();
  if (ndev <= 0) return fail(PK_ERR_HIP, "pk_probe: no HIP device visible (the HIP path has no CPU fallback)");
  if (device < 0 || device >= ndev) return fail(PK_ERR_INVALID, "pk_probe: device %d of %d", device, ndev);
  const int cls = classify_covariance(cov, 0);
  if (cls < 0) return cls;
  for (int i = 0; i < 16; ++i)
    if (!std::isfinite(Qt[i])) return fail(PK_ERR_INVALID, "pk_probe: Qt is not finite");
  bool dense = cls == 1;
  {
    double scale = 0;
    for (int i = 0; i < 4; ++i) scale = fmax(scale, fabs(Qt[i * 5]));
    for (int j = 1; j < 4; ++j)
      if (fabs(Qt[j]) > 1e-14 * scale || fabs(Qt[j * 4]) > 1e-14 * scale) dense = true;
    for (int i = 1; i < 4; ++i)
      for (int j = i + 1; j < 4; ++j)
        if (fabs(Qt[i * 4 + j] - Qt[j * 4 + i]) > 1e-9 * (scale > 0 ? scale : 1.0)) dense = true;
// ... 153 lines not shown
```

### parakeet_slam_amd/csrc/pk_k_step_pub.hip

```cpp
#include <type_traits>

#include "pk_device.hpp"
#include "pk_pub_math.hpp"
#include "pk_pub_layout.hpp"

namespace pk {

#ifndef PK_PUB_ABLATE
#define PK_PUB_ABLATE 0
#endif

typedef double Double2 __attribute__((ext_vector_type(2)));
typedef int Int2 __attribute__((ext_vector_type(2)));

__device__ __forceinline__ double pose_scalar(const double* a, int64_t p) {
  return ((const __attribute__((address_space(4))) double*)a)[p];
}
__device__ __forceinline__ int32_t regs_source_pub(const int32_t* src, int64_t p) {
  return ((const __attribute__((address_space(4))) int32_t*)src)[p];
}

struct PubArgs {
  SlotSource ss;
  unsigned char* map_dst;
  size_t count_off;
  int32_t* src;
  const double *x, *y, *h;
  double* logw;
  const double* exact;
  const unsigned short* order;
  const unsigned char* immutable;
  const uint4* cand;
  const uint4* erec;
  const unsigned* glist;
  const unsigned* skip;
  const float4* gate4;
  const uint4* far;
  unsigned char* pflag_out;
  unsigned* n_flagged;
  int64_t P, p_begin;
  int L, Lp, B;
  int ecap;
  int reset;
  unsigned long long* gmax_key;
  Noise<double> qt;
  const unsigned* stats;
  int tbytes;
  const uint4* prim;
  unsigned* unm;
  int unm_words;
};

constexpr int kPubUnmWords = 176;
template <int THREADS>
__device__ __forceinline__ void pub_note_unmatched(int tid, const unsigned char* anyc, const unsigned short* order, int B, unsigned Bp, unsigned* ubits) {
  for (unsigned w = (unsigned)tid; w < Bp / 4u; w += THREADS) {
    const unsigned v = reinterpret_cast<const unsigned*>(anyc)[w];
#pragma unroll
    for (int b = 0; b < 4; ++b)
      if ((int)(4 * w + b) < B && ((v >> (8 * b)) & 0xFFu) == 0u) {
        const unsigned o = order[4 * w + b];
        atomicOr(&ubits[o >> 5], 1u << (o & 31u));
      }
  }
}
template <int THREADS>
__device__ __forceinline__ void pub_store_unmatched(int tid, unsigned* ubits, unsigned* row, int words) {
  for (int w = tid; w < words; w += THREADS) {
    row[w] = ubits[w];
    ubits[w] = 0u;
  }
}

struct PubPrim {
  const uint4* tab;
  size_t Lpp;
  int lc;
  __device__ __forceinline__ double2 z01(int j) const { return reinterpret_cast<const double2*>(tab + Lpp)[lc + j]; }
  __device__ __forceinline__ double2 z23(int j) const { return reinterpret_cast<const double2*>(tab + 2 * Lpp)[lc + j]; }
  __device__ __forceinline__ double2 dir(int j) const { return reinterpret_cast<const double2*>(tab + 3 * Lpp)[lc + j]; }
  __device__ __forceinline__ unsigned t0(int j) const { return reinterpret_cast<const unsigned*>(tab + 4 * Lpp)[lc + j]; }
};

constexpr size_t kPubImmBytes = 2048;
__host__ __device__ inline size_t pub_bound_lds_bytes(bool small) { return (small ? 512 : 2048) * 8; }
__host__ __device__ inline size_t pub_fixed_lds_bytes(int B, bool small = false) {
  const size_t Bp = ((size_t)B + 15) & ~(size_t)15;
  return Bp * 48 + 16 + Bp * 4 + Bp * 2 + 2 * (Bp + 16) + kPubImmBytes + pub_bound_lds_bytes(small);
}
size_t step_pub_lds_bytes(int B, int ecap, bool small) { return pub_fixed_lds_bytes(B, small) + (size_t)ecap * 8; }
int step_pub_entry_capacity(int B) {
  const size_t fixed = pub_fixed_lds_bytes(B);
  if (fixed + 64 * 8 > kMaxDynLds) return 0;
  const size_t e = (kMaxDynLds - fixed) / 8;
  return (int)(e > 65534 ? 65534 : e);
}

int step_pub_entry_capacity_small(int B) {
  const size_t budget = 52 * 1024, fixed = pub_fixed_lds_bytes(B, true);
  if (fixed + 64 * 8 > budget) return 0;
  return (int)((budget - fixed) / 8);
}

template <int SL>
struct PubSlotsT {
  unsigned s[SL];
  unsigned st;
};
using PubSlots = PubSlotsT<kPubSlots>;
constexpr PubSlots kPubNoSlots = {{0xFFFFFFFFu, 0xFFFFFFFFu, 0xFFFFFFFFu, 0xFFFFFFFFu}, 0u};
template <int SL>
__device__ __forceinline__ void pub_rotate(PubSlotsT<SL>& q) {
  const unsigned w = q.s[0];
#pragma unroll
  for (int k = 0; k + 1 < SL; ++k) q.s[k] = q.s[k + 1];
  q.s[SL - 1] = w;
  if constexpr (SL == 8) {
    q.st = (q.st >> 4) | (q.st << 28);
  } else {
    const unsigned lowmask = (1u << (4 * SL)) - 1u, low = q.st & lowmask;
    q.st = (((low >> 4) | (low << (4 * SL - 4))) & lowmask) | (q.st & ~lowmask);
  }
}

__device__ __forceinline__ double pub_inf() { return __longlong_as_double(0x7FF0000000000000ll); }

struct PubGateIn {
  uint4 ref;
  uint4 cw[2], ew[2];
  double mx, my, mr, mg, mb;
  bool has;
  double fk, fi;
};
// ... 622 lines not shown
      const double2 z23 = *reinterpret_cast<const double2*>(rec + 2);
      BlobT<double> z{z01.x, z01.y, z23.x, z23.y};
      acc += ekf_update(lm, sx, sy, z, qt, imm, (EkfAux<double>*)nullptr, fresh ? &pse : (const double*)nullptr, prod);
      fresh = imm;
    }
  }
  return acc;
}

template <bool PRIM = false>
__device__ __forceinline__ double pub_apply_loop(const PubSlots& q, const double* ex, const unsigned short* order, const Noise<double>& qt,
                                            Landmark<double>& lm, bool imm, double sx, double sy, double pse,
                                            const char* ptab = nullptr, size_t pstride = 0, int pidx = 0, unsigned t0 = 0xFFFFu,
                                            double* prod = nullptr) {
  double acc = 0.0;
  unsigned tk = q.st & 0x4444u;
  bool fresh = true;
#pragma unroll 1
  for (int it = 0; it < kPubSlots; ++it) {
    if (__ballot(tk != 0u) == 0ull) break;
    unsigned w, bit;
    if (__ballot((tk & (tk - 1u)) != 0u) == 0ull) {
      w = (tk & 0x0004u) ? q.s[0] : (tk & 0x0040u) ? q.s[1] : (tk & 0x0400u) ? q.s[2] : q.s[3];
      bit = tk;
    } else {
      const unsigned sw[kPubSlots] = {q.s[0], q.s[1], q.s[2], q.s[3]};
      unsigned best = 0xFFFFFFFFu;
      w = 0u;
      bit = 0u;
#pragma unroll
      for (int s = 0; s < kPubSlots; ++s) {
        const bool on = ((tk >> (4 * s)) & 4u) != 0u;
        const unsigned o = order[on ? (sw[s] & 0xFFFFu) : 0u];
        const bool first = on && o < best;
        best = first ? o : best;
        w = first ? sw[s] : w;
        bit = first ? (4u << (4 * s)) : bit;
      }
    }
    const char* rb0 = reinterpret_cast<const char*>(ex);
    size_t rks = 16;
    bool onp = false;
    if constexpr (PRIM) {
      onp = __ballot(tk != 0u && (w & 0xFFFFu) != t0) == 0ull;
      rb0 = onp ? ptab : rb0;
      rks = onp ? pstride : rks;
    }
    if (tk != 0u) {
      const unsigned roff = (PRIM && onp) ? (unsigned)pidx * 16u : (w & 0xFFFFu) * 48u;
      const double2 z01 = *reinterpret_cast<const double2*>(rb0 + roff);
      const double2 z23 = *reinterpret_cast<const double2*>(rb0 + rks + roff);
      BlobT<double> z{z01.x, z01.y, z23.x, z23.y};
      acc += ekf_update(lm, sx, sy, z, qt, imm, (EkfAux<double>*)nullptr, fresh ? &pse : (const double*)nullptr, prod);
      fresh = imm;
    }
    tk &= ~bit;
  }
  return acc;
}

#ifdef PK_STAMPS
__device__ unsigned long long pk_pstamp_wave[8][12];
#define PK_PSTAMP(slot, a, b) pst[slot] += (b) - (a);
void debug_read_pub_wave_stamps(unsigned long long* out, bool reset) {
  (void)hipDeviceSynchronize();
  (void)hipMemcpyFromSymbol(out, HIP_SYMBOL(pk_pstamp_wave), sizeof(unsigned long long) * 96);
  if (reset) {
    unsigned long long z[96] = {0};
    (void)hipMemcpyToSymbol(HIP_SYMBOL(pk_pstamp_wave), z, sizeof(z));
  }
}
void debug_read_pub_stamps(unsigned long long* out, bool reset) {
  (void)hipDeviceSynchronize();
  (void)hipMemcpyFromSymbol(out, HIP_SYMBOL(pk_pstamp_acc), sizeof(unsigned long long) * 16);
  if (reset) {
    unsigned long long z[16] = {0};
    (void)hipMemcpyToSymbol(HIP_SYMBOL(pk_pstamp_acc), z, sizeof(z));
  }
}
#else
#define PK_PSTAMP(slot, a, b)
#endif

typedef const __attribute__((address_space(4))) PubArgs* PubArgsPtr;
__device__ __forceinline__ PubArgsPtr pub_args_now(PubArgsPtr rp) {
  asm volatile("" : "+s"(rp));
  return rp;
}
__device__ __forceinline__ SlotSource pub_slot_source(PubArgsPtr R) {
  return SlotSource{R->ss.map, R->ss.slot_bytes, R->ss.alt, R->ss.alt_stride, R->ss.alt_off};
}
__device__ __forceinline__ Noise<double> pub_noise(PubArgsPtr R) {
  return Noise<double>{R->qt.q00, R->qt.rr, R->qt.rg, R->qt.rb, R->qt.gg, R->qt.gb, R->qt.bb, R->qt.diag};
}

#ifdef PK_DIAG_NO_XCD_RUNS
__device__ __forceinline__ int64_t pub_walk_first(int64_t p_begin, int64_t) { return p_begin + blockIdx.x; }
__device__ __forceinline__ int64_t pub_walk_stride() { return (int64_t)gridDim.x; }
__device__ __forceinline__ int64_t pub_walk_limit(int64_t, int64_t p_end) { return p_end; }
#else
__device__ __forceinline__ int64_t pub_walk_first(int64_t p_begin, int64_t p_end) {
  const unsigned g = gridDim.x, b = blockIdx.x;
  if ((g & 7u) != 0u) return p_begin + b;
  const int64_t chunk = (p_end - p_begin + 7) / 8;
  return p_begin + (int64_t)(b & 7u) * chunk + (int64_t)(b >> 3);
}
__device__ __forceinline__ int64_t pub_walk_stride() { return (gridDim.x & 7u) != 0u ? (int64_t)gridDim.x : (int64_t)(gridDim.x >> 3); }
__device__ __forceinline__ int64_t pub_walk_limit(int64_t p_begin, int64_t p_end) {
  const unsigned g = gridDim.x, b = blockIdx.x;
  if ((g & 7u) != 0u) return p_end;
  const int64_t chunk = (p_end - p_begin + 7) / 8, e = p_begin + (int64_t)((b & 7u) + 1u) * chunk;
  return e < p_end ? e : p_end;
}
#endif
template <int NP, int THREADS>
__global__ void __launch_bounds__(THREADS, THREADS == 256 ? 3 : 1) k_step_pub(PubArgs a_unused) {
  constexpr int kPubThreads = THREADS, kPubWaves = THREADS / kWave;
  extern __shared__ __align__(16) unsigned char smem[];
  __shared__ double red[2][kPubWaves];
  __shared__ int wg_flag[2];
  constexpr bool kPerm = NP == 2 && THREADS == 512;
  __shared__ unsigned short s_perm[kPerm ? 2 * kPubOctets : 1];
  __shared__ unsigned s_rb[kCandSlots];
  constexpr int kUnmWords = THREADS == kPubSmallThreads ? 32 : 96;
  __shared__ unsigned s_ubits[kUnmWords];
#define PK_PUB_L0(q_, t_) (!kPerm ? 2 * kPubThreads * (q_) + 2 * (t_) : (int)(((lw >> (16 + 8 * (q_))) & 0xFFu) << 4) + 2 * ((t_)&7))
  PubArgsPtr rp = (PubArgsPtr)__builtin_amdgcn_kernarg_segment_ptr();
  const int tid0 = threadIdx.x;
  int B, Lp, L, ecap;
  {
    PubArgsPtr R = pub_args_now(rp);
    if (*R->skip != 0u) return;
    B = R->B;
    Lp = R->Lp;
    L = R->L;
    ecap = R->ecap;
  }
  const unsigned Bp = ((unsigned)B + 15u) & ~15u;
  const unsigned o_pub = Bp * 48u, o_binfo = o_pub + ((unsigned)ecap + 2u) * 8u, o_order = o_binfo + Bp * 4u, o_any = o_order + Bp * 2u;
  const unsigned o_imm = o_any + 2u * (Bp + 16u);
  const unsigned o_bnd = o_imm + (unsigned)kPubImmBytes;
  const unsigned dump = (unsigned)ecap, anydump = Bp;
  unsigned G;
  {
    const int tid = tid0;
    PubArgsPtr R = pub_args_now(rp);
    {
      const uint4* gf = R->far;
      float2* bnd = reinterpret_cast<float2*>(smem + o_bnd);
      for (int i = tid; i < Lp; i += kPubThreads) {
        float2 v = make_float2(-3.0e38f, 0.f);
        if (gf) {
          const uint4 hdr = gf[2 * (size_t)i];
          if (hdr.z != 0u) v = make_float2(__uint_as_float(hdr.x), __uint_as_float(hdr.y));
        }
        bnd[i] = v;
      }
    }
    double* ex = reinterpret_cast<double*>(smem);
    const double* gex = R->exact;
    for (int i = tid; i < 6 * B; i += kPubThreads) ex[i] = gex[i];
    unsigned* glist = reinterpret_cast<unsigned*>(smem + o_binfo);
    unsigned short* order = reinterpret_cast<unsigned short*>(smem + o_order);
    const unsigned* gb = R->glist;
    const unsigned short* go = R->order;
    G = gb[B];
    for (int i = tid; i < B; i += kPubThreads) {
      glist[i] = (unsigned)i < G ? gb[i] : 0u;
      order[i] = go[i];
    }
    for (unsigned i = (unsigned)tid; i < 2u * (Bp + 16u) / 4u; i += kPubThreads) reinterpret_cast<unsigned*>(smem + o_any)[i] = 0u;
    const unsigned char* gi = R->immutable;
    for (int i = tid; i < Lp; i += kPubThreads) smem[o_imm + (unsigned)i] = i < L ? gi[i] : (unsigned char)0;
    if constexpr (kPerm) {
      if (tid < 2 * kPubOctets) s_perm[tid] = reinterpret_cast<const unsigned short*>(gb + B + 1)[tid];
    }
    if (tid < kCandSlots) s_rb[tid] = gb[B + 1 + kPubTailWords + tid];
    for (int i = tid; i < kUnmWords; i += kPubThreads) s_ubits[i] = 0u;
    if (tid == 0) {
      wg_flag[0] = 0;
      wg_flag[1] = 0;
    }
  }
  __syncthreads();

  int64_t prev = -1;
  int cur = 0;
  int32_t nsrc;
  {
    PubArgsPtr R = pub_args_now(rp);
    const int64_t p0 = pub_walk_first(R->p_begin, R->P), pl = pub_walk_limit(R->p_begin, R->P);
    nsrc = regs_source_pub(R->src, p0 < pl ? p0 : pl - 1);
  }
#ifdef PK_STAMPS
  unsigned long long pst[12] = {0, 0, 0, 0, 0, 0, 0, 0, 0, 0, 0, 0};
#endif
#define PK_PUB_ROW(q_, field, F)                                                                  \
  {                                                                                               \
    const Double2 v_ = *reinterpret_cast<const Double2*>(sf_ + (size_t)F * Lp + lbq_);            \
    S[2 * (q_)].field = v_.x;                                                                     \
    S[2 * (q_) + 1].field = v_.y;                                                                 \
  }
#define PK_PUB_LOAD_MEANS(q_, sslot_, lb_)                                                        \
  {                                                                                               \
    const double* sf_ = reinterpret_cast<const double*>(sslot_);                                  \
    const int lbq_ = (lb_);                                                                       \
    PK_PUB_ROW(q_, mx, F_MX)                                                                      \
    PK_PUB_ROW(q_, my, F_MY)                                                                      \
    PK_PUB_ROW(q_, mr, F_MR)                                                                      \
    PK_PUB_ROW(q_, mg, F_MG)                                                                      \
    PK_PUB_ROW(q_, mb, F_MB)                                                                      \
    asm volatile("" ::: "memory");                                                                \
  }
#define PK_PUB_LOAD_COVS(q_, sslot_, coff_, lb_)                                                  \
  {                                                                                               \
    const double* sf_ = reinterpret_cast<const double*>(sslot_);                                  \
    const int* sc_ = reinterpret_cast<const int*>((sslot_) + (coff_));                            \
    const int lbq_ = (lb_);                                                                       \
    PK_PUB_ROW(q_, pxx, F_PXX)                                                                    \
    PK_PUB_ROW(q_, pxy, F_PXY)                                                                    \
    PK_PUB_ROW(q_, pyy, F_PYY)                                                                    \
    PK_PUB_ROW(q_, crr, F_CRR)                                                                    \
    PK_PUB_ROW(q_, crg, F_CRG)                                                                    \
    PK_PUB_ROW(q_, crb, F_CRB)                                                                    \
    PK_PUB_ROW(q_, cgg, F_CGG)                                                                    \
    PK_PUB_ROW(q_, cgb, F_CGB)                                                                    \
    PK_PUB_ROW(q_, cbb, F_CBB)                                                                    \
    const Int2 c_ = *reinterpret_cast<const Int2*>(sc_ + lbq_);                                   \
    S[2 * (q_)].count = c_.x;                                                                     \
    S[2 * (q_) + 1].count = c_.y;                                                                 \
    asm volatile("" ::: "memory");                                                                \
  }
#define PK_PUB_LOAD_PAIR(q_, sslot_, coff_, lb_)                                                  \
  {                                                                                               \
    const double* sf_ = reinterpret_cast<const double*>(sslot_);                                  \
    const int* sc_ = reinterpret_cast<const int*>((sslot_) + (coff_));                            \
    const int lbq_ = (lb_);                                                                       \
    PK_PUB_ROW(q_, mx, F_MX)                                                                      \
    PK_PUB_ROW(q_, my, F_MY)                                                                      \
    PK_PUB_ROW(q_, mr, F_MR)                                                                      \
    PK_PUB_ROW(q_, mg, F_MG)                                                                      \
    PK_PUB_ROW(q_, mb, F_MB)                                                                      \
    asm volatile("" ::: "memory");                                                                \
    PK_PUB_ROW(q_, pxx, F_PXX)                                                                    \
    PK_PUB_ROW(q_, pxy, F_PXY)                                                                    \
    PK_PUB_ROW(q_, pyy, F_PYY)                                                                    \
    PK_PUB_ROW(q_, crr, F_CRR)                                                                    \
    PK_PUB_ROW(q_, crg, F_CRG)                                                                    \
    PK_PUB_ROW(q_, crb, F_CRB)                                                                    \
    PK_PUB_ROW(q_, cgg, F_CGG)                                                                    \
    PK_PUB_ROW(q_, cgb, F_CGB)                                                                    \
    PK_PUB_ROW(q_, cbb, F_CBB)                                                                    \
    const Int2 c_ = *reinterpret_cast<const Int2*>(sc_ + lbq_);                                   \
    S[2 * (q_)].count = c_.x;                                                                     \
    S[2 * (q_) + 1].count = c_.y;                                                                 \
    asm volatile("" ::: "memory");                                                                \
  }
  Landmark<double> S[2 * NP];
  constexpr int kPipe = 1;
  unsigned lane_word = (unsigned)tid0;
  if constexpr (kPerm) {
    const unsigned octs = (unsigned)(s_perm[tid0 >> 3] & 0xFFu) | ((unsigned)(s_perm[kPubOctets + (tid0 >> 3)] & 0xFFu) << 8);
    lane_word = (unsigned)tid0 | (octs << 16);
  }
  {
    const unsigned lw = lane_word;
    PubArgsPtr R = pub_args_now(rp);
    const unsigned char* ns = pub_slot_source(R).at(nsrc);
    const int coff = R->count_off;
#pragma unroll
    for (int q = 0; q < kPipe; ++q) PK_PUB_LOAD_PAIR(q, ns, coff, min(PK_PUB_L0(q, tid0), Lp - 2))
  }
  for (int64_t p = pub_walk_first(pub_args_now(rp)->p_begin, pub_args_now(rp)->P);; p += pub_walk_stride(), cur ^= 1) {
    unsigned lw = lane_word;
    asm volatile("" : "+v"(lw));
    int tid;
    if constexpr (!kPerm) {
      tid = (int)lw;
    } else {
      tid = (int)(lw & 0xFFFFu);
    }
    double* ex = reinterpret_cast<double*>(smem);
    double* pub = reinterpret_cast<double*>(smem + o_pub);
    const unsigned* glist = reinterpret_cast<const unsigned*>(smem + o_binfo);
    const unsigned short* order = reinterpret_cast<const unsigned short*>(smem + o_order);
    unsigned char* anyc = smem + o_any + (unsigned)cur * (Bp + 16u);
    PubSlots Q[2 * NP];
    double pse[2 * NP];
    bool done;
    PK_STAMP(s0)
#ifdef PK_STAMPS
    unsigned long long s3 = s0;
#endif
    {
      PubArgsPtr R = pub_args_now(rp);
      const int64_t Pn = pub_walk_limit(R->p_begin, R->P);
      done = p >= Pn;
      const int64_t pc = done ? Pn - 1 : p;
      {
        const SlotSource ss = pub_slot_source(R);
        const unsigned char* sslot = ss.at(nsrc);
        const double sx = pose_scalar(R->x, pc), sy = pose_scalar(R->y, pc), sh = pose_scalar(R->h, pc);
        int lbase[NP];
#pragma unroll
        for (int q = 0; q < NP; ++q) lbase[q] = min(PK_PUB_L0(q, tid), Lp - 2);
        uint4 cref[2 * NP], ccw[2 * NP], cew[2 * NP];
        auto request_cand = [&](int q) {
          PubArgsPtr R2 = pub_args_now(rp);
#ifdef PK_DIAG_TAIL_LISTS
          const int lc = lbase[q];
#else
          const int lc = min(PK_PUB_L0(q, tid), Lp);
#endif
          const uint4* cr = R2->cand + 2 * (size_t)lc;
          const uint4* er = R2->erec + lc;
          cref[2 * q] = cr[0];
          ccw[2 * q] = cr[1];
          cref[2 * q + 1] = cr[2];
          ccw[2 * q + 1] = cr[3];
          cew[2 * q] = er[0];
          cew[2 * q + 1] = er[1];
        };
        request_cand(0);
        asm volatile("" ::: "memory");
        {
          PubArgsPtr R4 = pub_args_now(rp);
          const int64_t pn = p + pub_walk_stride(), pl = pub_walk_limit(R4->p_begin, R4->P);
          nsrc = regs_source_pub(R4->src, pn < pl ? pn : pl - 1);
          asm volatile("" : "+s"(nsrc));
        }
        PK_STAMP(s1)
        PK_PSTAMP(0, s0, s1)
        auto do_pair = [&](auto qc) {
          constexpr int q = decltype(qc)::value;

    const int l0 = PK_PUB_L0(q, tid);
    const PubGateIn gi[2] = {{cref[2 * q], {ccw[2 * q], ccw[2 * q]}, {cew[2 * q], cew[2 * q]}, S[2 * q].mx, S[2 * q].my,
                              S[2 * q].mr, S[2 * q].mg, S[2 * q].mb, l0 < L},
                             {cref[2 * q + 1], {ccw[2 * q + 1], ccw[2 * q + 1]}, {cew[2 * q + 1], cew[2 * q + 1]},
                              S[2 * q + 1].mx, S[2 * q + 1].my, S[2 * q + 1].mr, S[2 * q + 1].mg, S[2 * q + 1].mb,
                              l0 + 1 < L}};
    PubSlots qq[2] = {kPubNoSlots,
                      kPubNoSlots};
    double pp[2] = {0.0, 0.0};
    if constexpr (THREADS == kPubSmallThreads) {
      
#pragma unroll
      for (int j_ = 0; j_ < 2; ++j_) {
        const PubGateIn g1[1] = {gi[j_]};
        PubSlots q1[1] = {qq[j_]};
        double p1[1] = {0.0};
        const Landmark<double>* const l1[1] = {&S[2 * q + j_]};
        if (PK_PUB_ABLATE < 4) pub_gatesN<1>(q1, p1, g1, ex, pub, dump, &wg_flag[cur], sx, sy, sh);
        if (PK_PUB_ABLATE < 3) {
          struct Chk1 {
            const float2* bnd_;
            int l_, L_, Lp_;
            PubArgsPtr rp_;
            double sh;
            __device__ __forceinline__ float2 bnd(int) const { return bnd_[min(l_, Lp_ - 1)]; }
            __device__ __forceinline__ bool has(int) const { return l_ < L_; }
            __device__ __forceinline__ const uint4* far_row() const {
              const uint4* fr = pub_args_now(rp_)->far;
              return fr ? fr + 2 * (size_t)min(l_, Lp_) : nullptr;
            }
          };
          const Chk1 chk{reinterpret_cast<const float2*>(smem + o_bnd), l0 + j_, L, Lp, rp, sh};
          pub_keysN<1, kPubSlots, false, true, 1, Chk1>(q1, l1, p1, ex, pub, dump, anyc, anydump, &wg_flag[cur], sx, sy, nullptr, nullptr, chk);
        }
        qq[j_] = q1[0];
        pp[j_] = p1[0];
      }
    } else {
      const Landmark<double>* const l2[2] = {&S[2 * q], &S[2 * q + 1]};
      if (PK_PUB_ABLATE < 4) pub_gatesN<2, 1, kPubSlots, true>(qq, pp, gi, ex, pub, dump, &wg_flag[cur], sx, sy, sh);
      PK_STAMP(sk0_)
      if (PK_PUB_ABLATE < 3) {
        struct Chk2 {
          const float2* bnd_;
          unsigned lw, tid_;
          int L_, Lp_;
          PubArgsPtr rp_;
          double sh;
          __device__ __forceinline__ int l0() const { const unsigned lw = this->lw; const int tid = (int)tid_; (void)tid; return PK_PUB_L0(q, tid); }
          __device__ __forceinline__ float2 bnd(int j) const { return bnd_[min(l0() + j, Lp_ - 1)]; }
          __device__ __forceinline__ bool has(int j) const { return l0() + j < L_; }
          __device__ __forceinline__ const uint4* far_row() const {
            const uint4* fr = pub_args_now(rp_)->far;
            return fr ? fr + 2 * (size_t)min(l0(), Lp_) : nullptr;
          }
        };
        const Chk2 chk{reinterpret_cast<const float2*>(smem + o_bnd), lw, (unsigned)tid, L, Lp, rp, sh};
        pub_keysN<2, kPubSlots, false, true, 1, Chk2>(qq, l2, pp, ex, pub, dump, anyc, anydump, &wg_flag[cur], sx, sy, nullptr, nullptr, chk);
        {
          PubArgsPtr R9 = pub_args_now(rp);
          const int lc9 = min(l0, Lp);
          if (pub_refill_slots<2>(qq, R9->cand + 2 * (size_t)lc9, R9->erec + lc9, &wg_flag[cur]))
            pub_keysN<2>(qq, l2, pp, ex, pub, dump, anyc, anydump, &wg_flag[cur], sx, sy);
        }
      }
      PK_STAMP(sk1_)
      PK_PSTAMP(2, sk0_, sk1_)
    }
    Q[2 * q] = qq[0];
    Q[2 * q + 1] = qq[1];
    pse[2 * q] = pp[0];
    pse[2 * q + 1] = pp[1];
  
        };
        if (!done) {
          do_pair(std::integral_constant<int, 0>{});
          if constexpr (NP > 1) {
            PK_PUB_LOAD_MEANS(1, sslot, lbase[1])
            request_cand(NP - 1);
            {
              asm volatile("" ::: "memory");
              PubArgsPtr R7 = pub_args_now(rp);
              PK_PUB_LOAD_COVS(1, sslot, R7->count_off, lbase[1])
            }
            do_pair(std::integral_constant<int, 1>{});
          }
        }
        PK_STAMP(s2)
        PK_PSTAMP(1, s1, s2)
#ifdef PK_STAMPS
        s3 = s2;
#endif
      }
    }
    lds_barrier();
    PK_STAMP(s4)
    PK_PSTAMP(3, s3, s4)
    if (prev >= 0 && tid == 0) {
      PubArgsPtr R = pub_args_now(rp);
      double tot = red[cur ^ 1][0];
#pragma unroll
      for (int i = 1; i < kPubWaves; ++i) tot += red[cur ^ 1][i];
      double* logw = R->logw;
      const double w = (R->reset ? 0.0 : logw[prev]) + tot;
      logw[prev] = w;
      unsigned long long* gk = R->gmax_key;
      if (gk) atomicMax(gk + (prev & (kGmaxKeys - 1)), double_to_key(w));
      R->src[prev] = (int32_t)prev;
    }
    if (done) break;
    prev = -1;
    double acc;
    {
      int nun = 0;
      for (unsigned w = (unsigned)tid; w < Bp / 4u; w += kPubThreads) {
        const unsigned v = reinterpret_cast<const unsigned*>(anyc)[w];
#pragma unroll
        for (int b = 0; b < 4; ++b) nun += ((int)(4 * w + b) < B && ((v >> (8 * b)) & 0xFFu) == 0u) ? 1 : 0;
      }
      acc = (double)nun * Consts<double>::log_no_match;
      unsigned* anyn = reinterpret_cast<unsigned*>(smem + o_any + (unsigned)(cur ^ 1) * (Bp + 16u));
      for (unsigned w = (unsigned)tid; w < Bp / 4u; w += kPubThreads) anyn[w] = 0u;
      if (tid == 0) wg_flag[cur ^ 1] = 0;
    }
    if (pub_args_now(rp)->unm != nullptr) pub_note_unmatched<THREADS>(tid, anyc, order, B, Bp, s_ubits);
    if (PK_PUB_ABLATE < 2) pub_settle_blobs<THREADS>(tid, glist, G, pub, dump, &wg_flag[cur], s_rb);
    PK_STAMP(s5)
    PK_PSTAMP(4, s4, s5)
    lds_barrier();
    {
      PubArgsPtr Ru = pub_args_now(rp);
      if (Ru->unm != nullptr) pub_store_unmatched<THREADS>(tid, s_ubits, Ru->unm + (size_t)p * Ru->unm_words, Ru->unm_words);
    }
#pragma unroll
    for (int i = 0; i < 2 * NP; ++i)
      if (PK_PUB_ABLATE < 2) pub_take(Q[i], pub, dump);
    lds_barrier();
    PK_STAMP(s6)
    PK_PSTAMP(5, s5, s6)
    if (wg_flag[cur] && PK_PUB_ABLATE == 0) {
      if (tid == 0) {
        PubArgsPtr R = pub_args_now(rp);
        R->pflag_out[p] = 1;
        atomicAdd(R->n_flagged, 1u);
      }
      {
        PubArgsPtr R6 = pub_args_now(rp);
        const unsigned char* ns = pub_slot_source(R6).at(nsrc);
        const int coff = R6->count_off;
#pragma unroll
        for (int q = 0; q < kPipe; ++q) PK_PUB_LOAD_PAIR(q, ns, coff, min(PK_PUB_L0(q, tid), Lp - 2))
      }
      continue;
    }
    {
      PubArgsPtr R = pub_args_now(rp);
      if (tid == 0) R->pflag_out[p] = 0;
      const Noise<double> qt = pub_noise(R);
      const double sx = pose_scalar(R->x, p), sy = pose_scalar(R->y, p);
      unsigned char* dslot = R->map_dst + (size_t)p * R->ss.slot_bytes;
      double* df = reinterpret_cast<double*>(dslot);
      int* dc = reinterpret_cast<int*>(dslot + R->count_off);
      const unsigned char* immutable = smem + o_imm;
      {
        double nprod = 1.0;
        auto do_apply = [&](auto qc) {
          constexpr int q = decltype(qc)::value;
          const int l0 = PK_PUB_L0(q, tid);
#pragma unroll
          for (int j = 0; j < 2; ++j) {
            const int i = 2 * q + j;
            const bool imm = immutable[min(l0 + j, Lp - 1)] != 0;
            if (PK_PUB_ABLATE < 1)
              acc += THREADS == kPubSmallThreads ? pub_apply_loop(Q[i], ex, order, qt, S[i], imm, sx, sy, pse[i], nullptr, 0, 0, 0xFFFFu, PK_PROD_PTR(nprod))
                                                 : pub_apply(Q[i], ex, order, qt, S[i], imm, sx, sy, pse[i], PK_PROD_PTR(nprod));
          }
          pub_fold_norms(acc, nprod, q == NP - 1);
        };
        auto do_store = [&](auto qc) {
          constexpr int q = decltype(qc)::value;
          const int l0 = PK_PUB_L0(q, tid);
          PK_STAMP(su0_)
          if (l0 < Lp) {
#define PK_PUB_STORE(field, F)                                                             \
    {                                                                                        \
      const Double2 v = {S[2 * q].field, S[2 * q + 1].field};                                \
      __builtin_nontemporal_store(v, reinterpret_cast<Double2*>(df + (size_t)F * Lp + l0)); \
    }
            PK_PUB_STORE(mx, F_MX)
            PK_PUB_STORE(my, F_MY)
            PK_PUB_STORE(mr, F_MR)
            PK_PUB_STORE(mg, F_MG)
            PK_PUB_STORE(mb, F_MB)
            PK_PUB_STORE(pxx, F_PXX)
            PK_PUB_STORE(pxy, F_PXY)
            PK_PUB_STORE(pyy, F_PYY)
            PK_PUB_STORE(crr, F_CRR)
            PK_PUB_STORE(crg, F_CRG)
            PK_PUB_STORE(crb, F_CRB)
            PK_PUB_STORE(cgg, F_CGG)
            PK_PUB_STORE(cgb, F_CGB)
            PK_PUB_STORE(cbb, F_CBB)
#undef PK_PUB_STORE
            const Int2 c = {S[2 * q].count, S[2 * q + 1].count};
            __builtin_nontemporal_store(c, reinterpret_cast<Int2*>(dc + l0));
          }
          if (q < kPipe) {
            PubArgsPtr R6 = pub_args_now(rp);
            const unsigned char* ns = pub_slot_source(R6).at(nsrc);
            PK_PUB_LOAD_PAIR(q, ns, R6->count_off, min(PK_PUB_L0(q, tid), Lp - 2))
          }
          PK_STAMP(su1_)
          PK_PSTAMP(10, su0_, su1_)
        };
        using Q0 = std::integral_constant<int, 0>;
        using Q1 = std::integral_constant<int, 1>;
        do_apply(Q0{});
        do_store(Q0{});
        if constexpr (NP == 2) {
          do_apply(Q1{});
          do_store(Q1{});
        }
      }
    }
    PK_STAMP(s7)
    PK_PSTAMP(6, s6, s7)
    {
      const double ws = wave_sum(acc);
      if ((tid & (kWave - 1)) == 0) red[cur][tid / kWave] = ws;
      prev = p;
    }
    PK_STAMP(s8)
    PK_PSTAMP(7, s7, s8)
    PK_PSTAMP(8, s0, s8)
#ifdef PK_STAMPS
    pst[9] += 1ull;
#endif
  }
#ifdef PK_STAMPS
  if ((tid0 & 63) == 0)
    for (int k = 0; k < 12; ++k) {
      atomicAdd(&pk_pstamp_acc[k], pst[k]);
      if (THREADS == 512) atomicAdd(&pk_pstamp_wave[tid0 >> 6][k], pst[k]);
    }
#endif
}

constexpr int kPubBigSlots = 2 * kCandSlots;
constexpr int kPubBigGateSlots = 8;
__device__ __forceinline__ PubSlots pub_keep_positive(const PubSlotsT<kPubBigGateSlots>& g, int* flag) {
  PubSlots o = kPubNoSlots;
#pragma unroll
  for (int k = kPubBigGateSlots - 1; k >= 0; --k) {
    const bool pos = ((g.st >> (4 * k)) & 1u) != 0u;
    o.s[3] = pos ? o.s[2] : o.s[3];
    o.s[2] = pos ? o.s[1] : o.s[2];
    o.s[1] = pos ? o.s[0] : o.s[1];
    o.s[0] = pos ? g.s[k] : o.s[0];
    o.st = pos ? ((o.st << 4) | 1u) : o.st;
  }
  if (flag && __popc(g.st & 0x11111111u) > kPubSlots) *flag = 1;
  o.st &= 0xFFFFu;
  return o;
}
__device__ __forceinline__ uint4 pub_positive_beyond_four(const PubSlotsT<kPubBigGateSlots>& g) {
  unsigned x[4] = {0xFFFFFFFFu, 0xFFFFFFFFu, 0xFFFFFFFFu, 0xFFFFFFFFu};
  int c = 0;
#pragma unroll
  for (int k = 0; k < kPubBigGateSlots; ++k) {
    const bool pos = ((g.st >> (4 * k)) & 1u) != 0u;
    x[0] = (pos && c == 4) ? g.s[k] : x[0];
    x[1] = (pos && c == 5) ? g.s[k] : x[1];
    x[2] = (pos && c == 6) ? g.s[k] : x[2];
    x[3] = (pos && c == 7) ? g.s[k] : x[3];
    c += pos ? 1 : 0;
  }
  return make_uint4(x[0], x[1], x[2], x[3]);
}
__device__ __forceinline__ void pub_park_beyond_four(PubSlots& q, const PubSlotsT<kPubBigGateSlots>& g, uint4* ovf, unsigned n_places, unsigned* counter,
                                                     int* flag) {
  if (__popc(g.st & 0x11111111u) > kPubSlots) {
    const unsigned place = atomicAdd(counter, 1u);
    if (place < n_places) {
      ovf[place] = pub_positive_beyond_four(g);
      q.st |= (place + 1u) << 16;
    } else {
      *flag = 1;
    }
  }
}
__device__ __forceinline__ void pub_take_parked(PubSlots& q, const uint4* ovf, const double* pub, unsigned dump, int* flag) {
  const unsigned pl = q.st >> 16;
  if (__ballot(pl != 0u) == 0ull) return;
  if (pl != 0u) {
    const uint4 s4 = ovf[pl - 1u];
    const unsigned xw[4] = {s4.x, s4.y, s4.z, s4.w};
    double m[4];
#pragma unroll
    for (int x = 0; x < 4; ++x) {
      const unsigned e = xw[x] >> 16;
      m[x] = pub[e == 0xFFFFu ? dump : e];
    }
#pragma unroll
    for (int x = 0; x < 4; ++x) {
      const unsigned e = xw[x] >> 16;
      const bool take = (xw[x] & 0xFFFFu) != 0xFFFFu && (e == 0xFFFFu || m[x] == pub_marker());
      bool placed = !take;
#pragma unroll
      for (int sidx = 0; sidx < kPubSlots; ++sidx) {
        const bool here = !placed && ((q.st >> (4 * sidx)) & 4u) == 0u;
        q.s[sidx] = here ? xw[x] : q.s[sidx];
        q.st = here ? ((q.st & ~(0xFu << (4 * sidx))) | (5u << (4 * sidx))) : q.st;
        placed |= here;
      }
      if (!placed) *flag = 1;
    }
  }
  q.st &= 0xFFFFu;
}
__host__ __device__ inline size_t pub_big_fixed_lds_bytes(int B) {
  const size_t Bp = ((size_t)B + 15) & ~(size_t)15;
  return 16 + Bp * 4 + 2 * (Bp + 16);
}
int step_pub_big_entry_capacity(int B) {
  const size_t fixed = pub_big_fixed_lds_bytes(B);
  if (fixed + 64 * 8 > kMaxDynLds) return 0;
  const size_t e = (kMaxDynLds - fixed) / 8;
  return (int)(e > 65534 ? 65534 : e);
}
// ... 405 lines not shown
          PK_BIG_STORE(crr, F_CRR)
          PK_BIG_STORE(crg, F_CRG)
          PK_BIG_STORE(crb, F_CRB)
          PK_BIG_STORE(cgg, F_CGG)
          PK_BIG_STORE(cgb, F_CGB)
          PK_BIG_STORE(cbb, F_CBB)
          const Int2 c2_ = {SA.count, SB.count};
          __builtin_nontemporal_store(c2_, reinterpret_cast<Int2*>(dc + l0));
        }
        {
          const bool more = kBack ? q > 0 : (q + 1 < NCH && 2 * kPubThreads * (q + 1) < Lp);
          const int ln = min(PK_BIG_L0(more ? (kBack ? q - 1 : q + 1) : 0, tid), Lp - 2);
          const int32_t sn = more ? csrc : nsrc;
          PK_BIG_ROWS(SA, SB, ln, sn)
        }
        PK_STAMP(d3)
        PK_PSTAMP(10, d2, d3)
      }
#pragma unroll
      for (int i = 0; i + 2 < 2 * NCH; ++i) {
        Q[i] = Q[i + 2];
        pse[i] = pse[i + 2];
      }
    }
#undef PK_BIG_STORE
#undef PK_BIG_ROWS
#undef PK_BIG_LOAD
    pub_fold_norms(acc, nprod, true);
    {
      const double ws = wave_sum(acc);
      if ((tid & (kWave - 1)) == 0) red[cur][tid / kWave] = ws;
      prev = p;
    }
#ifdef PK_STAMPS
    {
      PK_STAMP(b5)
      PK_PSTAMP(11, b0, b5)
      pst[9] += 1ull;
    }
#endif
  }
#ifdef PK_STAMPS
  if ((tid0 & 63) == 0)
    for (int k = 0; k < 12; ++k) atomicAdd(&pk_pstamp_wave[tid0 >> 6][k], pst[k]);
#endif
#undef PK_BIG_WAIT_ALL
}

void launch_step_pub_big(hipStream_t s, DeviceState& d, int B, const double* exact_dev, const unsigned short* order_dev,
                         const FastHandoff& fh, const NoiseD& qt, const ObserveExtras& ex, const CandTable& cand, const uint4* erec_dev,
                         const unsigned* glist_dev, const unsigned* skip_dev, int ecap, const float4* gate4_dev, int64_t p0, int64_t p1,
                         int reserve_cus, const uint4* prim_dev, const unsigned* stats_dev) {
  if (p1 < 0) p1 = d.P;
  if (d.P == 0 || p1 <= p0 || !prim_dev || !stats_dev) return;
  static bool attr_set[kMaxDevices] = {false};
  if (first_time_on_this_device(attr_set)) {
    for (const void* fn : {reinterpret_cast<const void*>(k_step_pub_big<3>), reinterpret_cast<const void*>(k_step_pub_big<5>),
                           reinterpret_cast<const void*>(k_step_pub_big<6>)})
      if (hipFuncSetAttribute(fn, hipFuncAttributeMaxDynamicSharedMemorySize, (int)kMaxDynLds) != hipSuccess) (void)hipGetLastError();
  }
  PubArgs a;
  a.ss = slot_source(d);
  a.map_dst = d.map[d.mcur ^ 1];
  a.count_off = d.lay.count_off;
  a.src = d.src[d.cur];
  a.x = d.x[d.cur];
  a.y = d.y[d.cur];
  a.h = d.h[d.cur];
  a.logw = d.logw[d.cur];
  a.exact = exact_dev;
  a.order = order_dev;
  a.immutable = d.immutable;
  a.cand = cand.rec;
  a.erec = erec_dev;
  a.glist = glist_dev;
  a.skip = skip_dev;
  a.gate4 = gate4_dev;
  a.far = cand.far;
  a.prim = prim_dev;
  a.stats = stats_dev;
  a.tbytes = 0;
  a.unm = ex.unm;
  a.unm_words = ex.unm_words;
  a.pflag_out = fh.pflag;
  a.n_flagged = fh.n_flagged;
  a.P = p1;
  a.p_begin = p0;
  a.L = d.lay.L;
  a.Lp = d.lay.Lp;
  a.B = B;
  a.ecap = ecap;
  a.reset = ex.reset ? 1 : 0;
  a.gmax_key = ex.gmax_key;
  a.qt = make_noise(qt.q00, qt.rr, qt.rg, qt.rb, qt.gg, qt.gb, qt.bb);
  const int n_cu = device_cu_count();
  int64_t grid_n = n_cu - (reserve_cus > 0 && reserve_cus < n_cu ? reserve_cus : 0);
  if (grid_n > p1 - p0) grid_n = p1 - p0;
  const size_t lds = step_pub_big_lds_bytes(B, ecap);
  const int nch = (d.lay.Lp + 2 * kPubThreads - 1) / (2 * kPubThreads);
  if (nch <= 3)
    hipLaunchKernelGGL(k_step_pub_big<3>, dim3((unsigned)grid_n), dim3(kPubThreads), lds, s, a);
  else if (nch <= 5)
    hipLaunchKernelGGL(k_step_pub_big<5>, dim3((unsigned)grid_n), dim3(kPubThreads), lds, s, a);
  else
    hipLaunchKernelGGL(k_step_pub_big<6>, dim3((unsigned)grid_n), dim3(kPubThreads), lds, s, a);
}

void launch_step_pub(hipStream_t s, DeviceState& d, int B, const double* exact_dev, const unsigned short* order_dev,
                     const FastHandoff& fh, const NoiseD& qt, const ObserveExtras& ex, const CandTable& cand, const uint4* erec_dev,
                     const unsigned* glist_dev, const unsigned* skip_dev, int ecap, int64_t p0, int64_t p1, int reserve_cus) {
  if (p1 < 0) p1 = d.P;
  if (d.P == 0 || p1 <= p0) return;
  static bool attr_set[kMaxDevices] = {false};
  if (first_time_on_this_device(attr_set)) {
    for (const void* fn : {reinterpret_cast<const void*>(k_step_pub<1, kPubSmallThreads>), reinterpret_cast<const void*>(k_step_pub<1, kPubThreads>),
                           reinterpret_cast<const void*>(k_step_pub<2, kPubThreads>)})
      if (hipFuncSetAttribute(fn, hipFuncAttributeMaxDynamicSharedMemorySize, (int)kMaxDynLds) != hipSuccess) (void)hipGetLastError();
  }
  PubArgs a;
  a.ss = slot_source(d);
  a.map_dst = d.map[d.mcur ^ 1];
  a.count_off = d.lay.count_off;
  a.src = d.src[d.cur];
  a.x = d.x[d.cur];
  a.y = d.y[d.cur];
  a.h = d.h[d.cur];
  a.logw = d.logw[d.cur];
  a.exact = exact_dev;
  a.order = order_dev;
  a.immutable = d.immutable;
  a.cand = cand.rec;
  a.erec = erec_dev;
  a.glist = glist_dev;
  a.skip = skip_dev;
  a.gate4 = nullptr;
  a.prim = nullptr;
  a.stats = nullptr;
  a.tbytes = 0;
  a.unm = ex.unm;
  a.unm_words = ex.unm_words;
  a.far = cand.far;
  a.pflag_out = fh.pflag;
  a.n_flagged = fh.n_flagged;
  a.P = p1;
  a.p_begin = p0;
  a.L = d.lay.L;
  a.Lp = d.lay.Lp;
  a.B = B;
  a.ecap = ecap;
  a.reset = ex.reset ? 1 : 0;
  a.gmax_key = ex.gmax_key;
  a.qt = make_noise(qt.q00, qt.rr, qt.rg, qt.rb, qt.gg, qt.gb, qt.bb);
  const int n_cu = device_cu_count();
  const bool small = d.lay.Lp <= 2 * kPubSmallThreads;
  const size_t lds = step_pub_lds_bytes(B, ecap, small);
  int per_cu = 1;
  if (small) per_cu = (int)std::min<size_t>(3, std::max<size_t>(1, (160 * 1024 - 1024) / (lds + 256)));
  int64_t grid_n = (int64_t)(n_cu - (reserve_cus > 0 && reserve_cus < n_cu ? reserve_cus : 0)) * per_cu;
  if (grid_n > p1 - p0) grid_n = p1 - p0;
  if (small)
    hipLaunchKernelGGL((k_step_pub<1, kPubSmallThreads>), dim3((unsigned)grid_n), dim3(kPubSmallThreads), lds, s, a);
  else if (d.lay.Lp <= 2 * kPubThreads)
    hipLaunchKernelGGL((k_step_pub<1, kPubThreads>), dim3((unsigned)grid_n), dim3(kPubThreads), lds, s, a);
  else
    hipLaunchKernelGGL((k_step_pub<2, kPubThreads>), dim3((unsigned)grid_n), dim3(kPubThreads), lds, s, a);
}

#include "pk_k_step_duo.inl"

}
```

### parakeet_slam_amd/csrc/pk_kernels.hpp

```cpp
#pragma once
#include <hip/hip_runtime.h>

#include <cstdint>

#include "pk_layout.hpp"

namespace pk {

struct NoiseD {
  double q00, rr, rg, rb, gg, gb, bb;
};

struct DeviceState {
  int64_t P;
  MapLayout lay;
  double* x[2];
  double* y[2];
  double* h[2];
  double* logw[2];
  int32_t* src[2];
  int cur;
  unsigned char* map[2];
  int mcur;
  unsigned char* immutable;
  const unsigned char* alt = nullptr;
  size_t alt_stride = 0, alt_off = 0;
  int64_t global_offset = 0;
  int64_t* logical[2] = {nullptr, nullptr};
};

struct GrowState {
  double* hyp[2] = {nullptr, nullptr};
  int32_t* cnt[2] = {nullptr, nullptr};
  int32_t* slot_id[2] = {nullptr, nullptr};
  int cur = 0;
  int L0 = 0, S = 0, R = 0;
  double pair_threshold = 0.0;
};
__host__ __device__ inline size_t grow_tail_readings_off(int S) { return 16 + (((size_t)S * 4 + 15) & ~(size_t)15); }
inline size_t grow_tail_bytes(const GrowState& g) { return g.R > 0 ? grow_tail_readings_off(g.S) + (size_t)g.R * 64 : 0; }

struct SlotSource {
  const unsigned char* map;
  size_t slot_bytes;
  const unsigned char* alt;
  size_t alt_stride, alt_off;
  __host__ __device__ const unsigned char* at(int32_t src) const {
    return src >= 0 ? map + (size_t)src * slot_bytes : alt + (size_t)(-(src + 1)) * alt_stride + alt_off;
  }
};
inline SlotSource slot_source(const DeviceState& d) {
  return SlotSource{d.map[d.mcur], d.lay.slot_bytes, d.alt, d.alt_stride, d.alt_off};
}

constexpr int kScanBlock = 1024;

void launch_motion(hipStream_t s, DeviceState& d, double v, double w, double dt, const double* z_dev,
                   uint64_t seed, uint64_t draw, int64_t global_offset, void* up_dst_dev = nullptr,
                   const void* up_src_host_mapped = nullptr, size_t up_bytes = 0, double* pose_part_dev = nullptr);
inline int64_t motion_pose_blocks(int64_t P) { return (P + 255) / 256; }
void launch_motion_range(hipStream_t s, DeviceState& d, double v, double w, double dt, uint64_t seed, uint64_t draw,
                         int64_t p0, int64_t p1);
void launch_reset_weights(hipStream_t s, DeviceState& d);
void launch_assoc_brute(hipStream_t s, DeviceState& d, const double* blobs_dev, const double* blobdir_dev,
                        int B, int32_t* ids_dev);
struct BlobGrid {
  double lo[3];
  double inv_h;
  int G[3];
  int ncell;
  float thr32;
  float thrb32;
};
constexpr double kGridCell = 17.5;
constexpr int kGridMax = 16;
__host__ __device__ inline size_t grid_cs_bytes(int ncell) { return ((size_t)(ncell + 1) * 2 + 15) & ~(size_t)15; }
size_t blob_grid_table_bytes(int ncell, int B, int n9);
size_t assoc_grid_lds_bytes(int ncell, int B, int n9);
constexpr size_t kMaxDynLds = 156 * 1024;
constexpr int kMaxDevices = 64;
inline bool first_time_on_this_device(bool (&done)[kMaxDevices]) {
  int dev = 0;
  if (hipGetDevice(&dev) != hipSuccess || dev < 0 || dev >= kMaxDevices) return true;
  if (done[dev]) return false;
  done[dev] = true;
  return true;
}
inline int device_cu_count() {
  static int n_cu[kMaxDevices] = {0};
  int dev = 0;
  const bool known = hipGetDevice(&dev) == hipSuccess && dev >= 0 && dev < kMaxDevices;
  if (known && n_cu[dev] > 0) return n_cu[dev];
  int n = 256;
  hipDeviceProp_t prop;
  if (known && hipGetDeviceProperties(&prop, dev) == hipSuccess && prop.multiProcessorCount > 0) n = prop.multiProcessorCount;
  (void)hipGetLastError();
  if (known) n_cu[dev] = n;
  return n;
}
struct FastHandoff {
  uint4* lmpass = nullptr;
  int slots = 4;
  bool flags_only = false;
  unsigned char* bcount = nullptr;
  unsigned char* pflag = nullptr;
  unsigned* n_flagged = nullptr;
  int32_t* row_of = nullptr;
  unsigned* row_next = nullptr;
  int64_t row_cap = 0;
  bool retry = false;
};
// ... 2 lines not shown
  const unsigned char* only_flagged = nullptr;
  const unsigned* n_flagged = nullptr;
  int sweep_only_value = 0;
  bool flip = true;
  bool reset = false;
  unsigned long long* gmax_key = nullptr;
  bool single_sightings = false;
  unsigned* unm = nullptr;
  int unm_words = 0;
};
constexpr int kFastSlots = 4;
constexpr int kSweepSlots = 8;
constexpr int kFastMaxL = 512;
void launch_assoc_grid(hipStream_t s, DeviceState& d, int B, const BlobGrid& grid, int n9,
                       const unsigned char* tables_dev, const double* exact_dev, int32_t* ids_dev,
                       bool finalize, const FastHandoff& fh);
size_t observe_fast_lds_bytes(int B);
void launch_observe_fast(hipStream_t s, DeviceState& d, int B, const double* exact_dev,
                         const unsigned short* order_dev, const FastHandoff& fh, const NoiseD& qt,
                         const ObserveExtras& ex = ObserveExtras());
void launch_observe(hipStream_t s, DeviceState& d, const double* blobs_dev, const double* blobdir_dev, int B,
                    const int32_t* first_dev, const int32_t* next_dev, int n_unmatched,
                    int32_t* ids_dev, const NoiseD& qt, const ObserveExtras& ex = ObserveExtras());
struct SweepPlan {
  int grid = 0;
  size_t lds = 0;
  int qcap = 0;
  size_t results_per_wg = 0;
};
SweepPlan observe_sweep_plan(const DeviceState& d, int B);
void launch_observe_sweep(hipStream_t s, DeviceState& d, int B, const double* exact_dev,
                          const unsigned short* order_dev, const FastHandoff& fh, const NoiseD& qt,
                          const ObserveExtras& ex, const SweepPlan& plan, uint4* results_dev);
size_t fused_lds_bytes(int ncell, int B, int n9, bool exact_lds = false);
constexpr size_t kFusedMaxLds = 78 * 1024;
void launch_step_fused(hipStream_t s, DeviceState& d, int B, const BlobGrid& grid, int n9,
                       const unsigned char* tables_dev, const double* exact_dev, const unsigned short* order_dev,
                       const FastHandoff& fh, const NoiseD& qt, const ObserveExtras& ex, const unsigned* pub_skipped_dev = nullptr);
constexpr int kCandSlots = 8;
constexpr int kCandSpare = 2;
constexpr double kCandBearing = 0.2;
constexpr double kCandColour = 1.5;
struct CandTable {
  const uint4* rec = nullptr;
  const uint4* brec = nullptr;
  const unsigned* over = nullptr;
  const unsigned* skip_cand = nullptr;
  const unsigned* n_stray = nullptr;
  const uint4* far = nullptr;
  int slots = kCandSlots;
};
void launch_assoc_grid(hipStream_t s, DeviceState& d, int B, const BlobGrid& grid, int n9,
                       const unsigned char* tables_dev, const double* exact_dev, int32_t* ids_dev,
                       bool finalize, const FastHandoff& fh, const CandTable& cand);
void launch_candidates(hipStream_t s, DeviceState& d, int B, const double* exact_dev, int64_t ref_particle, uint4* rec_dev,
                       unsigned* over_dev, unsigned* bcnt_dev = nullptr, uint4* brec_dev = nullptr, unsigned* stray_dev = nullptr,
                       int slots = kCandSlots, const double* pose_sums4_dev = nullptr, unsigned char* npass_dev = nullptr,
                       uint4* far_dev = nullptr, const double* pose_part_dev = nullptr);
constexpr int kRegsMaxL = 2048;
size_t regs_lds_bytes(int ncell, int B, int n9);
size_t regs_cand_lds_bytes(int Lp, int B);
void launch_step_regs(hipStream_t s, DeviceState& d, int B, const BlobGrid& grid, int n9, const unsigned char* tables_dev,
                      const double* exact_dev, const unsigned short* order_dev, const FastHandoff& fh, const NoiseD& qt,
                      const ObserveExtras& ex, int warm, const CandTable& cand = CandTable(), int64_t p0 = 0, int64_t p1 = -1,
                      int reserve_cus = 0);
int step_pub_entry_capacity(int B);
int step_pub_entry_capacity_small(int B);
size_t step_pub_lds_bytes(int B, int ecap, bool small = false);
struct DuoLimits {
  int tbytes = 0;
  int ecap = 0;
  int gcap = 0;
  int nl = 1;
  int park_limit = -1;
};
void launch_cand_entries(hipStream_t s, const DeviceState& d, int B, const uint4* cand_dev, uint4* erec_dev, unsigned* bcnt_dev,
                         uint4* brec_dev, unsigned* binfo_dev, unsigned* glist_dev, const unsigned* over_dev, unsigned* skip_pub_dev,
                         unsigned* skip_cand_dev, int ecap, int slots = kCandSlots, const double* exact_dev = nullptr,
                         float4* gate4_dev = nullptr, const unsigned char* npass_dev = nullptr, bool pruned = false,
                         unsigned* stats_dev = nullptr, unsigned* skip_duo_dev = nullptr, unsigned* skip_big_dev = nullptr,
                         const DuoLimits& duo = DuoLimits(), uint4* prim_dev = nullptr, unsigned char* flag_all_dev = nullptr,
                         unsigned* n_flagged_dev = nullptr);
inline size_t prim_table_uint4(int Lp) { const size_t Lpp = (size_t)Lp + kCandSpare; return 4 * Lpp + (Lpp + 3) / 4; }
void launch_step_pub(hipStream_t s, DeviceState& d, int B, const double* exact_dev, const unsigned short* order_dev,
                     const FastHandoff& fh, const NoiseD& qt, const ObserveExtras& ex, const CandTable& cand, const uint4* erec_dev,
                     const unsigned* glist_dev, const unsigned* skip_dev, int ecap, int64_t p0 = 0, int64_t p1 = -1,
                     int reserve_cus = 0);
void launch_flag_range_if(hipStream_t s, const unsigned* over_dev, unsigned char* pflag_dev, unsigned* n_flagged_dev, int64_t p0, int64_t p1);
constexpr int kPubBigMaxL = 6144;
int step_pub_big_entry_capacity(int B);
size_t step_pub_big_lds_bytes(int B, int ecap);
void launch_step_pub_big(hipStream_t s, DeviceState& d, int B, const double* exact_dev, const unsigned short* order_dev,
                         const FastHandoff& fh, const NoiseD& qt, const ObserveExtras& ex, const CandTable& cand, const uint4* erec_dev,
                         const unsigned* glist_dev, const unsigned* skip_dev, int ecap, const float4* gate4_dev = nullptr, int64_t p0 = 0,
                         int64_t p1 = -1, int reserve_cus = 0, const uint4* prim_dev = nullptr, const unsigned* stats_dev = nullptr);
void step_pub_duo_limits(int B, int Lp, int nl, DuoLimits* out);
size_t step_pub_duo_lds_bytes(int B, const DuoLimits& lim);
void launch_step_pub_duo(hipStream_t s, DeviceState& d, int B, const double* exact_dev, const unsigned short* order_dev,
                         const FastHandoff& fh, const NoiseD& qt, const ObserveExtras& ex, const CandTable& cand, const uint4* erec_dev,
                         const unsigned* glist_dev, const unsigned* skip_duo_dev, const unsigned* stats_dev, const DuoLimits& lim,
                         const float4* gate4_dev, const uint4* prim_dev, int64_t p0 = 0, int64_t p1 = -1, int reserve_cus = 0);
extern int g_observe_nv;
inline size_t observe_general_lds_bytes(int Lp, int B) { return sizeof(int32_t) * ((size_t)Lp + 2 * (size_t)B); }
inline size_t assoc_brute_lds_bytes(int B) { return (size_t)B * 12; }
void launch_block_max(hipStream_t s, DeviceState& d, double* partial_dev, double* gmax_dev);
void launch_keys_max(hipStream_t s, const unsigned long long* keys_dev, double* gmax_dev);
void launch_scan_local(hipStream_t s, DeviceState& d, const double* gmax_dev, int domain,
                       double* clocal_dev, double* totals_dev, const unsigned long long* gmax_key_dev = nullptr);
void launch_scan_blocks(hipStream_t s, const double* totals_dev, int64_t nb, double* offsets_dev,
                        double* sum_dev);
constexpr int64_t kAncestorsScanMaxBlocks = 256;
void launch_ancestors(hipStream_t s, const double* clocal_dev, const double* totals_dev,
                      const double* offsets_dev, const double* sum_dev, int64_t nb, int64_t P_global,
                      int64_t P_scan, double u, int64_t slot0, int64_t n, int32_t* anc_dev,
                      DeviceState* gather = nullptr);
void launch_summary_partials(hipStream_t s, DeviceState& d, double* partial_dev, double* out4_dev);
void launch_materialise(hipStream_t s, DeviceState& d);
void launch_broadcast_slot(hipStream_t s, DeviceState& d, const unsigned char* slot_dev);
void launch_probe(hipStream_t s, const double* in_dev, double* out_dev);
size_t dense_lds_bytes(int Lp, int B);
void launch_observe_dense(hipStream_t s, DeviceState& d, const double* blobs_dev, const double* blobdir_dev, int B,
                          const int32_t* ids_in_dev, int32_t* ids_out_dev, const double Qt[16], bool update,
                          const ObserveExtras& ex);
void launch_probe_dense(hipStream_t s, const double* in_dev, double* out_dev);
constexpr size_t kPoseRecordBytes = 8 * sizeof(double);
struct BalancedBuffers {
  double* glogw = nullptr;
  double* clocal = nullptr;
  double* totals = nullptr;
  double* offsets = nullptr;
  double* sum = nullptr;
  int64_t* H = nullptr;
  long long* cloc = nullptr;
  long long* ctot = nullptr;
  long long* coff = nullptr;
  int64_t* rel = nullptr;
  int64_t* Hl = nullptr;
  int32_t* alive = nullptr;
  int* bad = nullptr;
  int64_t cap = 0;
};
void launch_iota64(hipStream_t s, int64_t* p, int64_t n, int64_t off);
void launch_bal_state(hipStream_t s, const DeviceState& d, double* out_dev);
void launch_bal_plan(hipStream_t s, const DeviceState& d, const double* gstate_dev, int64_t Pg, int world, int rank,
                     const double* gmax_dev, int domain, double u, BalancedBuffers& b, int64_t* table_dev);
void launch_bal_pack(hipStream_t s, DeviceState& d, const BalancedBuffers& b, int64_t a0, int64_t n, int64_t ebase_s,
                     int64_t dbase_d, int64_t dd_d, int64_t m_d, unsigned char* buf_dev, size_t stride, const GrowState* g,
                     int64_t keep = -1);
void launch_bal_adopt(hipStream_t s, DeviceState& d, const BalancedBuffers& b, int64_t m, const unsigned char* buf_dev,
                      int64_t n_recv, int64_t* rh_dev, int mode, size_t stride, int32_t* anc_dev);
void launch_offspring(hipStream_t s, const double* clocal_dev, const double* offsets_dev, const double* sum_dev,
                      int64_t first_block, int64_t P_local, int64_t P_global, double u, int last_shard,
                      int64_t* hi_dev);
void launch_offspring_plan(hipStream_t s, const double* clocal_dev, const double* global_totals_dev,
                           int64_t n_global_blocks, int64_t first_block, int64_t P_local, int64_t P_global, double u,
                           int last_shard, int64_t* hi_dev, int world, int64_t* ranges_dev, unsigned* ticket_dev);
void launch_offspring_global(hipStream_t s, const double* clocal_global_dev, const double* offsets_dev, const double* sum_dev,
                             int64_t goff, int64_t P_local, int64_t P_global, double u, int last_shard, int64_t* hi_dev);
void launch_scan_local_of(hipStream_t s, const double* logw_dev, int64_t n, const double* gmax_dev, int domain,
                          double* clocal_dev, double* totals_dev);
void launch_pack(hipStream_t s, DeviceState& d, const int64_t* idx_dev, int64_t n, unsigned char* buf_dev);
void launch_adopt(hipStream_t s, DeviceState& d, const int64_t* src_dev, const unsigned char* buf_dev);
void launch_shard_ranges(hipStream_t s, const int64_t* hi_dev, int64_t P_local, int world, int64_t* ranges_dev);
void launch_pack_range(hipStream_t s, DeviceState& d, const int64_t* hi_dev, int64_t j0, int64_t n, int64_t slot_start,
                       int64_t slot_end, unsigned char* buf_dev);
void launch_adopt_dev(hipStream_t s, DeviceState& d, const int64_t* hi_dev, int64_t slot_start,
// ... 10 lines not shown
```

### parakeet_slam_amd/csrc/pk_math.hpp

```cpp
#pragma once
#include <hip/hip_runtime.h>

namespace pk {

template <typename T>
struct Consts;
template <>
struct Consts<double> {
  static constexpr double two_pi = 6.283185307179586476925286766559;
  static constexpr double half_pi = 1.5707963267948966192313216916398;
  static constexpr double log_two_pi = 1.8378770664093454835606594728112;
  static constexpr double log_no_match = -2.3025850929940456840179914546844;
};

template <typename T>
struct Landmark {
  T mx, my, mr, mg, mb;
  T pxx, pxy, pyy;
  T crr, crg, crb, cgg, cgb, cbb;
  int count;
};

constexpr int kPotentialBit = 0x40000000;
__device__ __forceinline__ void count_update(int& count) {
// ... 108 lines not shown
    ny = sy;
  } else {
    nx = sx + ux * mag;
    ny = sy + uy * mag;
  }
}

template <typename T>
__device__ __forceinline__ T prob_position_match(const Landmark<T>& f, T sx, T sy, T pse, T bearing,
                                                 T ux, T uy, T* near_xy = nullptr) {
  T nx, ny;
  closest_point(f.mx, f.my, sx, sy, ux, uy, nx, ny);
  if (near_xy) {
    near_xy[0] = nx;
    near_xy[1] = ny;
  }
  if (fabs(pse - bearing) > Consts<T>::half_pi) return T(0);
  T ex = nx - f.mx, ey = ny - f.my;
  T det = f.pxx * f.pyy - f.pxy * f.pxy;
  T maha = (f.pyy * ex * ex - T(2) * f.pxy * ex * ey + f.pxx * ey * ey) / det;
  return exp(T(-0.5) * (T(2) * Consts<T>::log_two_pi + log(det) + maha));
}

template <typename T>
__device__ __forceinline__ T prob_color_match(const Landmark<T>& f, T r, T g, T b) {
  T det;
  Sym3<T> inv = sym3_inverse(Sym3<T>{f.crr, f.crg, f.crb, f.cgg, f.cgb, f.cbb}, det);
  T maha = sym3_quad(inv, r - f.mr, g - f.mg, b - f.mb);
  return exp(T(-0.5) * (T(3) * Consts<T>::log_two_pi + log(det) + maha));
}

template <typename T>
__device__ __forceinline__ T color_distance2(T mr, T mg, T mb, T r, T g, T b) {
  T dr = r - mr, dg = g - mg, db = b - mb;
  return dr * dr + dg * dg + db * db;
}

template <typename T>
__device__ __forceinline__ T probability_of_match(const Landmark<T>& f, T sx, T sy, T heading,
                                                  const BlobT<T>& z, T ux, T uy) {
  T pse = pk_atan2(f.my - sy, f.mx - sx);
  T delb = z.bearing - (pse - heading);
  if (fabs(delb) > T(0.5)) return T(0);
  T cd = color_distance2(f.mr, f.mg, f.mb, z.r, z.g, z.b);
  if (fabs(cd) > T(300)) return T(0);
  T bp = T(500) * prob_position_match(f, sx, sy, pse, z.bearing, ux, uy);
  T cp = T(500) * prob_color_match(f, z.r, z.g, z.b);
  return bp * cp / T(250000);
}

__device__ __forceinline__ double log_few_ulp(double x) {
  if (!(x > 2.3e-308 && x < 1.7e308)) return log(x);
  int e = 0;
  double m = frexp(x, &e);
  if (m < 0.70710678118654752440) {
    m *= 2.0;
    e -= 1;
  }
  const double s = (m - 1.0) / (m + 1.0);
  const double z = s * s;
  double p = 1.0 / 21.0;
  p = fma_k(p, z, 1.0 / 19.0);
  p = fma_k(p, z, 1.0 / 17.0);
  p = fma_k(p, z, 1.0 / 15.0);
  p = fma_k(p, z, 1.0 / 13.0);
  p = fma_k(p, z, 1.0 / 11.0);
  p = fma_k(p, z, 1.0 / 9.0);
  p = fma_k(p, z, 1.0 / 7.0);
  p = fma_k(p, z, 1.0 / 5.0);
  p = fma_k(p, z, 1.0 / 3.0);
  const double lm = 2.0 * s + 2.0 * s * (z * p);
  const double ed = (double)e;
  return ed * 0.69314718055994528623 + (ed * 2.3190468138462995584e-17 + lm);
}

__device__ __forceinline__ double pr_from_parts(double det2, double det3, double num2, double num3) {
  const double maha2 = num2 / det2, maha3 = num3 / det3;
  const double bp = 500.0 * exp(-0.5 * (2.0 * Consts<double>::log_two_pi + log_few_ulp(det2) + maha2));
  const double cp = 500.0 * exp(-0.5 * (3.0 * Consts<double>::log_two_pi + log_few_ulp(det3) + maha3));
  return bp * cp / 250000.0;
}

template <typename T>
struct EkfAux {
  T zhat0, h0, h1;
  T q00;
  Sym3<T> qc;
  T k0, k1;
  T kc[9];
};

template <typename T>
__device__ __forceinline__ T ekf_update(Landmark<T>& f, T sx, T sy, const BlobT<T>& z,
                                        const Noise<T>& qt, bool immutable,
                                        EkfAux<T>* aux = nullptr, const T* zhat0_known = nullptr, T* fro_prod = nullptr) {
  T dx = f.mx - sx, dy = f.my - sy;
  T zhat0 = zhat0_known ? *zhat0_known : pk_atan2(dy, dx);
  T q = dx * dx + dy * dy;
  T h0, h1;
  if (q == T(0)) {
    h0 = T(0);
    h1 = T(0);
  } else {
    T iq = T(1) / q;
    h0 = dy * iq;
    h1 = dx * iq;
  }
  T a0 = f.pxx * h0 + f.pxy * h1;
  T a1 = f.pxy * h0 + f.pyy * h1;
  T q00 = h0 * a0 + h1 * a1 + qt.q00;
  Sym3<T> qc{f.crr + qt.rr, f.crg + qt.rg, f.crb + qt.rb, f.cgg + qt.gg, f.cgb + qt.gb, f.cbb + qt.bb};
  T detc;
  Sym3<T> qci = sym3_inverse(qc, detc);
  T iq00 = T(1) / q00;

  T d0 = z.bearing - zhat0;
  T d1 = z.r - f.mr, d2 = z.g - f.mg, d3 = z.b - f.mb;

  T fro2 = q00 * q00 + qc.a * qc.a + qc.d * qc.d + qc.f * qc.f +
           T(2) * (qc.b * qc.b + qc.c * qc.c + qc.e * qc.e);
  T v0 = qci.a * d1 + qci.b * d2 + qci.c * d3;
  T v1 = qci.b * d1 + qci.d * d2 + qci.e * d3;
  T v2 = qci.c * d1 + qci.e * d2 + qci.f * d3;
  T maha = d0 * d0 * iq00 + (d1 * v0 + d2 * v1 + d3 * v2);
  T logw;
  if (fro_prod) {
    logw = T(-0.5) * Consts<T>::log_two_pi - T(0.5) * maha;
    if (f.count & kPotentialBit)
      logw = (T)Consts<double>::log_no_match;
    else
      *fro_prod *= fro2;
  } else {
    logw = T(-0.5) * (Consts<T>::log_two_pi + T(0.5) * log_few_ulp(fro2)) - T(0.5) * maha;
    if (f.count & kPotentialBit) logw = (T)Consts<double>::log_no_match;
  }
  T k0 = a0 * iq00, k1 = a1 * iq00;

  if (aux) {
    aux->zhat0 = zhat0;
    aux->h0 = h0;
    aux->h1 = h1;
    aux->q00 = q00;
    aux->qc = qc;
    aux->k0 = k0;
    aux->k1 = k1;
    const T C[3][3] = {{f.crr, f.crg, f.crb}, {f.crg, f.cgg, f.cgb}, {f.crb, f.cgb, f.cbb}};
    const T I[3][3] = {{qci.a, qci.b, qci.c}, {qci.b, qci.d, qci.e}, {qci.c, qci.e, qci.f}};
    for (int i = 0; i < 3; ++i)
      for (int j = 0; j < 3; ++j) aux->kc[i * 3 + j] = C[i][0] * I[0][j] + C[i][1] * I[1][j] + C[i][2] * I[2][j];
  }

  if (!immutable) {
    f.mx += k0 * d0;
    f.my += k1 * d0;
    T nr = f.mr + (f.crr * v0 + f.crg * v1 + f.crb * v2);
    T ng = f.mg + (f.crg * v0 + f.cgg * v1 + f.cgb * v2);
    T nb = f.mb + (f.crb * v0 + f.cgb * v1 + f.cbb * v2);
    T nxx = f.pxx - k0 * a0;
    T nxy = f.pxy - T(0.5) * (k0 * a1 + k1 * a0);
    T nyy = f.pyy - k1 * a1;
    T nrr, nrg, nrb, ngg, ngb, nbb;
    T m00 = qci.a * f.crr + qci.b * f.crg + qci.c * f.crb;
    T m01 = qci.a * f.crg + qci.b * f.cgg + qci.c * f.cgb;
    T m02 = qci.a * f.crb + qci.b * f.cgb + qci.c * f.cbb;
    T m11 = qci.b * f.crg + qci.d * f.cgg + qci.e * f.cgb;
    T m12 = qci.b * f.crb + qci.d * f.cgb + qci.e * f.cbb;
    T m22 = qci.c * f.crb + qci.e * f.cgb + qci.f * f.cbb;
    if (qt.diag) {
      nrr = qt.rr * m00;
      nrg = qt.rr * m01;
      nrb = qt.rr * m02;
      ngg = qt.gg * m11;
      ngb = qt.gg * m12;
      nbb = qt.bb * m22;
    } else {
      T m10 = qci.b * f.crr + qci.d * f.crg + qci.e * f.crb;
      T m20 = qci.c * f.crr + qci.e * f.crg + qci.f * f.crb;
      T m21 = qci.c * f.crg + qci.e * f.cgg + qci.f * f.cgb;
      nrr = f.crr - (f.crr * m00 + f.crg * m10 + f.crb * m20);
      nrg = f.crg - (f.crr * m01 + f.crg * m11 + f.crb * m21);
      nrb = f.crb - (f.crr * m02 + f.crg * m12 + f.crb * m22);
      ngg = f.cgg - (f.crg * m01 + f.cgg * m11 + f.cgb * m21);
      ngb = f.cgb - (f.crg * m02 + f.cgg * m12 + f.cgb * m22);
      nbb = f.cbb - (f.crb * m02 + f.cgb * m12 + f.cbb * m22);
    }
    f.mr = nr;
    f.mg = ng;
    f.mb = nb;
    f.pxx = nxx;
    f.pxy = nxy;
    f.pyy = nyy;
    f.crr = nrr;
    f.crg = nrg;
    f.crb = nrb;
    f.cgg = ngg;
    f.cgb = ngb;
    f.cbb = nbb;
    count_update(f.count);
  }
  return logw;
}

template <typename T>
__device__ __forceinline__ void motion_model(T& x, T& y, T& h, T v, T w, T dt, T n0, T n1, T n2) {
  T dheading = w * dt;
  T ds = v * dt + n0;
  T h1 = h + dheading / T(2) + n1;
  T h2 = h1 + dheading / T(2) + n2;
  T s, c;
  sincos(h1, &s, &c);
  x += ds * c;
  y += ds * s;
  h = wrap_heading(h2);
}

}
```

Baseline: 19.52 billion.

## Share per-generation colour covariance table across particles in the pub step

The colour block of each landmark covariance evolves deterministically with its update count and does not depend on pose. So a small per-landmark, per-generation table is precomputed once at map upload. A new k_step_pub_tab variant reads the colour covariance from this table instead of loading six per-particle rows, which cuts global memory reads in the memory-bound step. The table is turned off on any event that could break the shared-state assumption (uploads, grow, adoption, noise change, relayout), and a landmark whose generation is past the table size falls back to the slot rows. Only maps with Lp between 2x and 4x the pub thread count take the new path.

```diff
diff --git a/parakeet_slam_amd/csrc/pk_api.hip b/parakeet_slam_amd/csrc/pk_api.hip
--- a/parakeet_slam_amd/csrc/pk_api.hip
+++ b/parakeet_slam_amd/csrc/pk_api.hip
@@ -10,6 +10,7 @@
 
 #include "../../include/parakeet_slam.h"
 #include "pk_kernels.hpp"
+#include "pk_pub_layout.hpp"
 
 using namespace pk;
 
@@ -193,6 +194,10 @@
   bool grow_on = false;
   int32_t* anc = nullptr;
   unsigned char* slot_tmp = nullptr;
+  double* ctab_dev = nullptr;
+  int ctab_cap = 0;
+  int shared_colour = 1;
+  int shared_colour_gens = 0;
   uint32_t timing_mask = 0;
   int timing_stride = 1;
   int64_t timing_seen[PK_T_COUNT] = {0};
@@ -749,6 +754,7 @@
 
 int relayout(pk_filter* f, bool dense, bool keep) {
   if (f->dense == dense) return PK_OK;
+  f->d.ctab_gens = 0;
   int rc;
   DeviceState& d = f->d;
   const MapLayout old = d.lay;
@@ -928,7 +934,7 @@
     if (q) (void)hipFree(q);
   void* rest[] = {d.immutable, f->z_dev,  f->ids_dev,
                   f->partial,  f->gmax,   f->clocal,    f->totals,      f->offsets,   f->sum,      f->out4, f->pose_part,
-                  f->anc,      f->slot_tmp};
+                  f->anc,      f->slot_tmp, f->ctab_dev};
   for (void* p : rest)
     if (p) (void)hipFree(p);
   for (int i = 0; i < pk_filter::kRing; ++i) {
@@ -963,6 +969,33 @@
 int32_t pk_num_landmarks(const pk_filter* f) { return f ? f->d.lay.L : -1; }
 int64_t pk_device_bytes(const pk_filter* f) { return f ? f->device_bytes : -1; }
 
+constexpr int kColourTableGens = 128;
+constexpr int kColourTableMaxGens = 1024;
+static void colour_table_off(pk_filter* f) { f->d.ctab_gens = 0; }
+static bool colour_table_route(const pk_filter* f) {
+  return !f->dense && !f->qt_dense && !f->grow_on && f->d.lay.Lp > 2 * kPubThreads && f->d.lay.Lp <= 4 * kPubThreads;
+}
+static int colour_table_build(pk_filter* f) {
+  colour_table_off(f);
+  if (!f->shared_colour || !colour_table_route(f)) return PK_OK;
+  const int gens = f->shared_colour_gens > 0 ? f->shared_colour_gens : kColourTableGens;
+  if (f->ctab_cap < gens) {
+    if (f->ctab_dev) {
+      PK_HIP(hipStreamSynchronize(f->stream));
+      (void)hipFree(f->ctab_dev);
+      f->device_bytes -= (int64_t)f->ctab_cap * f->d.lay.Lp * 6 * (int64_t)sizeof(double);
+      f->ctab_dev = nullptr;
+      f->ctab_cap = 0;
+    }
+    int rc;
+    if ((rc = dev_alloc(f, &f->ctab_dev, (size_t)gens * f->d.lay.Lp * 6))) return rc;
+    f->ctab_cap = gens;
+  }
+  launch_colour_table(f->stream, f->d, f->slot_tmp, f->qt, f->ctab_dev, 0, gens);
+  f->d.ctab = f->ctab_dev;
+  f->d.ctab_gens = gens;
+  return PK_OK;
+}
 int pk_set_measurement_noise(pk_filter* f, const double Qt[16]) {
   if (!f || !Qt) return fail(PK_ERR_INVALID, "pk_set_measurement_noise: NULL argument");
   for (int i = 0; i < 16; ++i)
@@ -980,6 +1013,7 @@
   if (coupled && !f->dense && (rc = relayout(f, true, f->map_loaded))) return rc;
   for (int i = 0; i < 16; ++i) f->qt16[i] = Qt[i];
   f->qt_dense = coupled;
+  colour_table_off(f);
   f->qt = NoiseD{Qt[0], Qt[5], 0.5 * (Qt[6] + Qt[9]), 0.5 * (Qt[7] + Qt[13]), Qt[10], 0.5 * (Qt[11] + Qt[14]), Qt[15]};
   return PK_OK;
 }
@@ -1009,6 +1043,7 @@
   PK_HIP(hipMemcpyAsync(f->slot_tmp, slot.data(), lay.slot_bytes, hipMemcpyHostToDevice, f->stream));
   PK_HIP(hipMemcpyAsync(f->d.immutable, imm.data(), imm.size(), hipMemcpyHostToDevice, f->stream));
   launch_broadcast_slot(f->stream, f->d, f->slot_tmp);
+  if ((rc = colour_table_build(f))) return rc;
   PK_HIP(hipStreamSynchronize(f->stream));
   f->src_identity = true;
   f->map_loaded = true;
@@ -1119,6 +1154,7 @@
 
 int pk_upload_landmarks(pk_filter* f, int64_t p0, int64_t p1, const double* means, const double* covs,
                         const int32_t* counts) {
+  if (f) colour_table_off(f);
   if (!f) return fail(PK_ERR_INVALID, "pk_upload_landmarks: NULL handle");
   if (p0 < 0 || p1 < p0 || p1 > f->d.P) return fail(PK_ERR_INVALID, "pk_upload_landmarks: bad particle range");
   if (!f->map_loaded) return fail(PK_ERR_STATE, "pk_upload_landmarks: no map uploaded");
@@ -1750,6 +1786,16 @@
     f->cand_lists = value != 0;
     return PK_OK;
   }
+  if (!strcmp(name, "shared_colour")) {
+    f->shared_colour = value != 0;
+    if (!f->shared_colour) colour_table_off(f);
+    return PK_OK;
+  }
+  if (!strcmp(name, "shared_colour_gens")) {
+    if (value < 0 || value > kColourTableMaxGens) return fail(PK_ERR_INVALID, "shared_colour_gens: 0 .. %d", kColourTableMaxGens);
+    f->shared_colour_gens = (int)value;
+    return PK_OK;
+  }
   if (!strcmp(name, "pub_step")) {
     f->pub_step = value != 0;
     return PK_OK;
@@ -1924,6 +1970,7 @@
 }
 
 int pk_grow_enable(pk_filter* f, int32_t preset_landmarks, int32_t reading_capacity, double pair_threshold) {
+  if (f) colour_table_off(f);
   if (!f) return fail(PK_ERR_INVALID, "pk_grow_enable: NULL handle");
   const int L = f->d.lay.L;
   if (preset_landmarks < 0 || preset_landmarks >= L)
@@ -1977,6 +2024,7 @@
 }
 
 int pk_grow_upload(pk_filter* f, int64_t p0, int64_t p1, const int32_t* counters, const double* readings, const int32_t* slot_ids) {
+  if (f) colour_table_off(f);
   int rc;
   if ((rc = grow_range(f, "pk_grow_upload", p0, p1))) return rc;
   const GrowState& g = f->grow;
@@ -2087,6 +2135,7 @@
 }
 
 int pk_adopt_particles(pk_filter* f, const int64_t* src, const void* dev_buf, int64_t n_received) {
+  if (f) colour_table_off(f);
   if (f) f->pose_part_ok = false;
   if (!f || !src || n_received < 0 || (n_received > 0 && !dev_buf)) return fail(PK_ERR_INVALID, "pk_adopt_particles: bad argument");
   if (f->grow_on) return fail(PK_ERR_STATE, "pk_adopt_particles: the new-landmark bookkeeping (pk_grow_enable) travels with the balanced placement only (pk_shard_*_balanced_dev)");
@@ -2262,6 +2311,7 @@
 }
 
 int pk_shard_adopt_dev(pk_filter* f, int32_t rank, const void* dev_recv, int64_t n_received) {
+  if (f) colour_table_off(f);
   if (f && f->grow_on) return fail(PK_ERR_STATE, "pk_shard_adopt_dev: the new-landmark bookkeeping (pk_grow_enable) travels with the balanced placement only (pk_shard_*_balanced_dev)");
   if (f) f->pose_part_ok = false;
   if (!f || rank < 0 || n_received < 0 || (n_received > 0 && !dev_recv)) return fail(PK_ERR_INVALID, "pk_shard_adopt_dev: bad argument");
@@ -2312,6 +2362,7 @@
 }
 
 int pk_shard_adopt_remote_dev(pk_filter* f, int32_t rank, const void* dev_recv, int64_t n_received) {
+  if (f) colour_table_off(f);
   if (f && f->grow_on) return fail(PK_ERR_STATE, "pk_shard_adopt_remote_dev: the new-landmark bookkeeping (pk_grow_enable) travels with the balanced placement only (pk_shard_*_balanced_dev)");
   if (f) f->pose_part_ok = false;
   if (!f || rank < 0 || n_received < 0 || (n_received > 0 && !dev_recv)) return fail(PK_ERR_INVALID, "pk_shard_adopt_remote_dev: bad argument");
@@ -2544,6 +2595,7 @@
 
 int pk_shard_adopt_balanced_dev(pk_filter* f, const int64_t* table, int32_t world, int32_t rank, const void* dev_recv,
                                 int64_t n_received, int32_t mode) {
+  if (f) colour_table_off(f);
   if (f) f->pose_part_ok = false;
   if (!f || !table || world < 1 || world > 64 || rank < 0 || rank >= world || n_received < 0 || mode < 0 || mode > 2 ||
       (n_received > 0 && !dev_recv))
diff --git a/parakeet_slam_amd/csrc/pk_k_step_pub.hip b/parakeet_slam_amd/csrc/pk_k_step_pub.hip
--- a/parakeet_slam_amd/csrc/pk_k_step_pub.hip
+++ b/parakeet_slam_amd/csrc/pk_k_step_pub.hip
@@ -49,6 +49,8 @@
   const uint4* prim;
   unsigned* unm;
   int unm_words;
+  const double* ctab;
+  int ctab_gens;
 };
 
 constexpr int kPubUnmWords = 176;
@@ -837,6 +839,64 @@
 #define PK_PSTAMP(slot, a, b)
 #endif
 
+__global__ void k_colour_table(const double* slot0, int Lp, Noise<double> qt, double* tab, int g0, int g1) {
+  const int l = blockIdx.x * blockDim.x + threadIdx.x;
+  if (l >= Lp || g1 <= g0) return;
+  Sym3<double> c;
+  if (g0 == 0) {
+    c = Sym3<double>{slot0[(size_t)F_CRR * Lp + l], slot0[(size_t)F_CRG * Lp + l], slot0[(size_t)F_CRB * Lp + l],
+                     slot0[(size_t)F_CGG * Lp + l], slot0[(size_t)F_CGB * Lp + l], slot0[(size_t)F_CBB * Lp + l]};
+  } else {
+    const double* t = tab + ((size_t)(g0 - 1) * Lp + l) * 6;
+    c = Sym3<double>{t[0], t[1], t[2], t[3], t[4], t[5]};
+  }
+  for (int g = g0; g < g1; ++g) {
+    if (g > 0) {
+      double detc;
+      const Sym3<double> qci = sym3_inverse(colour_innovation_cov(c, qt), detc);
+      c = colour_covar_next(c, qci, qt);
+    }
+    double* t = tab + ((size_t)g * Lp + l) * 6;
+    t[0] = c.a;
+    t[1] = c.b;
+    t[2] = c.c;
+    t[3] = c.d;
+    t[4] = c.e;
+    t[5] = c.f;
+  }
+}
+void launch_colour_table(hipStream_t s, const DeviceState& d, const unsigned char* slot0_dev, const NoiseD& qt, double* tab, int g0, int g1) {
+  if (g1 <= g0) return;
+  const int Lp = d.lay.Lp;
+  hipLaunchKernelGGL(k_colour_table, dim3((unsigned)((Lp + 255) / 256)), dim3(256), 0, s, reinterpret_cast<const double*>(slot0_dev), Lp,
+                     make_noise(qt.q00, qt.rr, qt.rg, qt.rb, qt.gg, qt.gb, qt.bb), tab, g0, g1);
+}
+__device__ __forceinline__ void pub_colour_pair(Landmark<double>& A, Landmark<double>& Bq, const double* tab, int gens, int Lp, int l,
+                                                const double* sf) {
+  const unsigned g0 = (unsigned)(A.count & ~kPotentialBit) >> 1, g1 = (unsigned)(Bq.count & ~kPotentialBit) >> 1;
+  const bool in0 = g0 < (unsigned)gens, in1 = g1 < (unsigned)gens;
+  const Double2* t0 = reinterpret_cast<const Double2*>(tab + ((size_t)(in0 ? g0 : 0u) * Lp + l) * 6);
+  const Double2* t1 = reinterpret_cast<const Double2*>(tab + ((size_t)(in1 ? g1 : 0u) * Lp + l + 1) * 6);
+  const Double2 a0 = t0[0], a1 = t0[1], a2 = t0[2], b0 = t1[0], b1 = t1[1], b2 = t1[2];
+  A.crr = a0.x, A.crg = a0.y, A.crb = a1.x, A.cgg = a1.y, A.cgb = a2.x, A.cbb = a2.y;
+  Bq.crr = b0.x, Bq.crg = b0.y, Bq.crb = b1.x, Bq.cgg = b1.y, Bq.cgb = b2.x, Bq.cbb = b2.y;
+  if (!(in0 && in1)) {
+#define PK_PUB_COLOUR_ROW(field, F)                                                  \
+    {                                                                                \
+      const Double2 v_ = *reinterpret_cast<const Double2*>(sf + (size_t)F * Lp + l); \
+      A.field = in0 ? A.field : v_.x;                                                \
+      Bq.field = in1 ? Bq.field : v_.y;                                              \
+    }
+    PK_PUB_COLOUR_ROW(crr, F_CRR)
+    PK_PUB_COLOUR_ROW(crg, F_CRG)
+    PK_PUB_COLOUR_ROW(crb, F_CRB)
+    PK_PUB_COLOUR_ROW(cgg, F_CGG)
+    PK_PUB_COLOUR_ROW(cgb, F_CGB)
+    PK_PUB_COLOUR_ROW(cbb, F_CBB)
+#undef PK_PUB_COLOUR_ROW
+  }
+}
+
 typedef const __attribute__((address_space(4))) PubArgs* PubArgsPtr;
 __device__ __forceinline__ PubArgsPtr pub_args_now(PubArgsPtr rp) {
   asm volatile("" : "+s"(rp));
@@ -868,8 +928,8 @@
   return e < p_end ? e : p_end;
 }
 #endif
-template <int NP, int THREADS>
-__global__ void __launch_bounds__(THREADS, THREADS == 256 ? 3 : 1) k_step_pub(PubArgs a_unused) {
+template <int NP, int THREADS, bool kTab>
+__device__ __forceinline__ void step_pub_body() {
   constexpr int kPubThreads = THREADS, kPubWaves = THREADS / kWave;
   extern __shared__ __align__(16) unsigned char smem[];
   __shared__ double red[2][kPubWaves];
@@ -975,12 +1035,14 @@
     PK_PUB_ROW(q_, pxx, F_PXX)                                                                    \
     PK_PUB_ROW(q_, pxy, F_PXY)                                                                    \
     PK_PUB_ROW(q_, pyy, F_PYY)                                                                    \
-    PK_PUB_ROW(q_, crr, F_CRR)                                                                    \
-    PK_PUB_ROW(q_, crg, F_CRG)                                                                    \
-    PK_PUB_ROW(q_, crb, F_CRB)                                                                    \
-    PK_PUB_ROW(q_, cgg, F_CGG)                                                                    \
-    PK_PUB_ROW(q_, cgb, F_CGB)                                                                    \
-    PK_PUB_ROW(q_, cbb, F_CBB)                                                                    \
+    if constexpr (!kTab) {                                   \
+      PK_PUB_ROW(q_, crr, F_CRR)                                                                  \
+      PK_PUB_ROW(q_, crg, F_CRG)                                                                  \
+      PK_PUB_ROW(q_, crb, F_CRB)                                                                  \
+      PK_PUB_ROW(q_, cgg, F_CGG)                                                                  \
+      PK_PUB_ROW(q_, cgb, F_CGB)                                                                  \
+      PK_PUB_ROW(q_, cbb, F_CBB)                                                                  \
+    }                                                                                             \
     const Int2 c_ = *reinterpret_cast<const Int2*>(sc_ + lbq_);                                   \
     S[2 * (q_)].count = c_.x;                                                                     \
     S[2 * (q_) + 1].count = c_.y;                                                                 \
@@ -1000,12 +1062,14 @@
     PK_PUB_ROW(q_, pxx, F_PXX)                                                                    \
     PK_PUB_ROW(q_, pxy, F_PXY)                                                                    \
     PK_PUB_ROW(q_, pyy, F_PYY)                                                                    \
-    PK_PUB_ROW(q_, crr, F_CRR)                                                                    \
-    PK_PUB_ROW(q_, crg, F_CRG)                                                                    \
-    PK_PUB_ROW(q_, crb, F_CRB)                                                                    \
-    PK_PUB_ROW(q_, cgg, F_CGG)                                                                    \
-    PK_PUB_ROW(q_, cgb, F_CGB)                                                                    \
-    PK_PUB_ROW(q_, cbb, F_CBB)                                                                    \
+    if constexpr (!kTab) {                                   \
+      PK_PUB_ROW(q_, crr, F_CRR)                                                                  \
+      PK_PUB_ROW(q_, crg, F_CRG)                                                                  \
+      PK_PUB_ROW(q_, crb, F_CRB)                                                                  \
+      PK_PUB_ROW(q_, cgg, F_CGG)                                                                  \
+      PK_PUB_ROW(q_, cgb, F_CGB)                                                                  \
+      PK_PUB_ROW(q_, cbb, F_CBB)                                                                  \
+    }                                                                                             \
     const Int2 c_ = *reinterpret_cast<const Int2*>(sc_ + lbq_);                                   \
     S[2 * (q_)].count = c_.x;                                                                     \
     S[2 * (q_) + 1].count = c_.y;                                                                 \
@@ -1078,6 +1142,10 @@
         };
         request_cand(0);
         asm volatile("" ::: "memory");
+        if constexpr (kTab) {
+          PubArgsPtr R3 = pub_args_now(rp);
+          pub_colour_pair(S[0], S[1], R3->ctab, R3->ctab_gens, Lp, lbase[0], reinterpret_cast<const double*>(sslot));
+        }
         {
           PubArgsPtr R4 = pub_args_now(rp);
           const int64_t pn = p + pub_walk_stride(), pl = pub_walk_limit(R4->p_begin, R4->P);
@@ -1172,6 +1240,10 @@
               asm volatile("" ::: "memory");
               PubArgsPtr R7 = pub_args_now(rp);
               PK_PUB_LOAD_COVS(1, sslot, R7->count_off, lbase[1])
+            }
+            if constexpr (kTab) {
+              PubArgsPtr R8 = pub_args_now(rp);
+              pub_colour_pair(S[2], S[3], R8->ctab, R8->ctab_gens, Lp, lbase[1], reinterpret_cast<const double*>(sslot));
             }
             do_pair(std::integral_constant<int, 1>{});
           }
@@ -1335,6 +1407,12 @@
     }
 #endif
 }
+
+template <int NP, int THREADS>
+__global__ void __launch_bounds__(THREADS, THREADS == 256 ? 3 : 1) k_step_pub(PubArgs) {
+  step_pub_body<NP, THREADS, false>();
+}
+__global__ void __launch_bounds__(kPubThreads, 1) k_step_pub_tab(PubArgs) { step_pub_body<2, kPubThreads, true>(); }
 
 constexpr int kPubBigSlots = 2 * kCandSlots;
 constexpr int kPubBigGateSlots = 8;
@@ -1906,6 +1984,8 @@
   a.tbytes = 0;
   a.unm = ex.unm;
   a.unm_words = ex.unm_words;
+  a.ctab = nullptr;
+  a.ctab_gens = 0;
   a.pflag_out = fh.pflag;
   a.n_flagged = fh.n_flagged;
   a.P = p1;
@@ -1938,7 +2018,7 @@
   static bool attr_set[kMaxDevices] = {false};
   if (first_time_on_this_device(attr_set)) {
     for (const void* fn : {reinterpret_cast<const void*>(k_step_pub<1, kPubSmallThreads>), reinterpret_cast<const void*>(k_step_pub<1, kPubThreads>),
-                           reinterpret_cast<const void*>(k_step_pub<2, kPubThreads>)})
+                           reinterpret_cast<const void*>(k_step_pub<2, kPubThreads>), reinterpret_cast<const void*>(k_step_pub_tab)})
       if (hipFuncSetAttribute(fn, hipFuncAttributeMaxDynamicSharedMemorySize, (int)kMaxDynLds) != hipSuccess) (void)hipGetLastError();
   }
   PubArgs a;
@@ -1963,6 +2043,8 @@
   a.tbytes = 0;
   a.unm = ex.unm;
   a.unm_words = ex.unm_words;
+  a.ctab = nullptr;
+  a.ctab_gens = 0;
   a.far = cand.far;
   a.pflag_out = fh.pflag;
   a.n_flagged = fh.n_flagged;
@@ -1986,7 +2068,11 @@
     hipLaunchKernelGGL((k_step_pub<1, kPubSmallThreads>), dim3((unsigned)grid_n), dim3(kPubSmallThreads), lds, s, a);
   else if (d.lay.Lp <= 2 * kPubThreads)
     hipLaunchKernelGGL((k_step_pub<1, kPubThreads>), dim3((unsigned)grid_n), dim3(kPubThreads), lds, s, a);
-  else
+  else if (d.ctab_gens > 0) {
+    a.ctab = d.ctab;
+    a.ctab_gens = d.ctab_gens;
+    hipLaunchKernelGGL(k_step_pub_tab, dim3((unsigned)grid_n), dim3(kPubThreads), lds, s, a);
+  } else
     hipLaunchKernelGGL((k_step_pub<2, kPubThreads>), dim3((unsigned)grid_n), dim3(kPubThreads), lds, s, a);
 }
 
diff --git a/parakeet_slam_amd/csrc/pk_kernels.hpp b/parakeet_slam_amd/csrc/pk_kernels.hpp
--- a/parakeet_slam_amd/csrc/pk_kernels.hpp
+++ b/parakeet_slam_amd/csrc/pk_kernels.hpp
@@ -27,6 +27,8 @@
   size_t alt_stride = 0, alt_off = 0;
   int64_t global_offset = 0;
   int64_t* logical[2] = {nullptr, nullptr};
+  const double* ctab = nullptr;
+  int ctab_gens = 0;
 };
 
 struct GrowState {
@@ -195,6 +197,7 @@
                          const DuoLimits& duo = DuoLimits(), uint4* prim_dev = nullptr, unsigned char* flag_all_dev = nullptr,
                          unsigned* n_flagged_dev = nullptr);
 inline size_t prim_table_uint4(int Lp) { const size_t Lpp = (size_t)Lp + kCandSpare; return 4 * Lpp + (Lpp + 3) / 4; }
+void launch_colour_table(hipStream_t s, const DeviceState& d, const unsigned char* slot0_dev, const NoiseD& qt, double* tab, int g0, int g1);
 void launch_step_pub(hipStream_t s, DeviceState& d, int B, const double* exact_dev, const unsigned short* order_dev,
                      const FastHandoff& fh, const NoiseD& qt, const ObserveExtras& ex, const CandTable& cand, const uint4* erec_dev,
                      const unsigned* glist_dev, const unsigned* skip_dev, int ecap, int64_t p0 = 0, int64_t p1 = -1,
diff --git a/parakeet_slam_amd/csrc/pk_math.hpp b/parakeet_slam_amd/csrc/pk_math.hpp
--- a/parakeet_slam_amd/csrc/pk_math.hpp
+++ b/parakeet_slam_amd/csrc/pk_math.hpp
@@ -214,6 +214,40 @@
 }
 
 template <typename T>
+__device__ __forceinline__ Sym3<T> colour_innovation_cov(const Sym3<T>& c, const Noise<T>& qt) {
+  return Sym3<T>{c.a + qt.rr, c.b + qt.rg, c.c + qt.rb, c.d + qt.gg, c.e + qt.gb, c.f + qt.bb};
+}
+template <typename T>
+__device__ __forceinline__ Sym3<T> colour_covar_next(const Sym3<T>& c, const Sym3<T>& qci, const Noise<T>& qt) {
+  T nrr, nrg, nrb, ngg, ngb, nbb;
+  T m00 = qci.a * c.a + qci.b * c.b + qci.c * c.c;
+  T m01 = qci.a * c.b + qci.b * c.d + qci.c * c.e;
+  T m02 = qci.a * c.c + qci.b * c.e + qci.c * c.f;
+  T m11 = qci.b * c.b + qci.d * c.d + qci.e * c.e;
+  T m12 = qci.b * c.c + qci.d * c.e + qci.e * c.f;
+  T m22 = qci.c * c.c + qci.e * c.e + qci.f * c.f;
+  if (qt.diag) {
+    nrr = qt.rr * m00;
+    nrg = qt.rr * m01;
+    nrb = qt.rr * m02;
+    ngg = qt.gg * m11;
+    ngb = qt.gg * m12;
+    nbb = qt.bb * m22;
+  } else {
+    T m10 = qci.b * c.a + qci.d * c.b + qci.e * c.c;
+    T m20 = qci.c * c.a + qci.e * c.b + qci.f * c.c;
+    T m21 = qci.c * c.b + qci.e * c.d + qci.f * c.e;
+    nrr = c.a - (c.a * m00 + c.b * m10 + c.c * m20);
+    nrg = c.b - (c.a * m01 + c.b * m11 + c.c * m21);
+    nrb = c.c - (c.a * m02 + c.b * m12 + c.c * m22);
+    ngg = c.d - (c.b * m01 + c.d * m11 + c.e * m21);
+    ngb = c.e - (c.b * m02 + c.d * m12 + c.e * m22);
+    nbb = c.f - (c.c * m02 + c.e * m12 + c.f * m22);
+  }
+  return Sym3<T>{nrr, nrg, nrb, ngg, ngb, nbb};
+}
+
+template <typename T>
 struct EkfAux {
   T zhat0, h0, h1;
   T q00;
@@ -241,7 +275,7 @@
   T a0 = f.pxx * h0 + f.pxy * h1;
   T a1 = f.pxy * h0 + f.pyy * h1;
   T q00 = h0 * a0 + h1 * a1 + qt.q00;
-  Sym3<T> qc{f.crr + qt.rr, f.crg + qt.rg, f.crb + qt.rb, f.cgg + qt.gg, f.cgb + qt.gb, f.cbb + qt.bb};
+  Sym3<T> qc = colour_innovation_cov(Sym3<T>{f.crr, f.crg, f.crb, f.cgg, f.cgb, f.cbb}, qt);
   T detc;
   Sym3<T> qci = sym3_inverse(qc, detc);
   T iq00 = T(1) / q00;
@@ -291,43 +325,19 @@
     T nxx = f.pxx - k0 * a0;
     T nxy = f.pxy - T(0.5) * (k0 * a1 + k1 * a0);
     T nyy = f.pyy - k1 * a1;
-    T nrr, nrg, nrb, ngg, ngb, nbb;
-    T m00 = qci.a * f.crr + qci.b * f.crg + qci.c * f.crb;
-    T m01 = qci.a * f.crg + qci.b * f.cgg + qci.c * f.cgb;
-    T m02 = qci.a * f.crb + qci.b * f.cgb + qci.c * f.cbb;
-    T m11 = qci.b * f.crg + qci.d * f.cgg + qci.e * f.cgb;
-    T m12 = qci.b * f.crb + qci.d * f.cgb + qci.e * f.cbb;
-    T m22 = qci.c * f.crb + qci.e * f.cgb + qci.f * f.cbb;
-    if (qt.diag) {
-      nrr = qt.rr * m00;
-      nrg = qt.rr * m01;
-      nrb = qt.rr * m02;
-      ngg = qt.gg * m11;
-      ngb = qt.gg * m12;
-      nbb = qt.bb * m22;
-    } else {
-      T m10 = qci.b * f.crr + qci.d * f.crg + qci.e * f.crb;
-      T m20 = qci.c * f.crr + qci.e * f.crg + qci.f * f.crb;
-      T m21 = qci.c * f.crg + qci.e * f.cgg + qci.f * f.cgb;
-      nrr = f.crr - (f.crr * m00 + f.crg * m10 + f.crb * m20);
-      nrg = f.crg - (f.crr * m01 + f.crg * m11 + f.crb * m21);
-      nrb = f.crb - (f.crr * m02 + f.crg * m12 + f.crb * m22);
-      ngg = f.cgg - (f.crg * m01 + f.cgg * m11 + f.cgb * m21);
-      ngb = f.cgb - (f.crg * m02 + f.cgg * m12 + f.cgb * m22);
-      nbb = f.cbb - (f.crb * m02 + f.cgb * m12 + f.cbb * m22);
-    }
+    const Sym3<T> cn = colour_covar_next(Sym3<T>{f.crr, f.crg, f.crb, f.cgg, f.cgb, f.cbb}, qci, qt);
     f.mr = nr;
     f.mg = ng;
     f.mb = nb;
     f.pxx = nxx;
     f.pxy = nxy;
     f.pyy = nyy;
-    f.crr = nrr;
-    f.crg = nrg;
-    f.crb = nrb;
-    f.cgg = ngg;
-    f.cgb = ngb;
-    f.cbb = nbb;
+    f.crr = cn.a;
+    f.crg = cn.b;
+    f.crb = cn.c;
+    f.cgg = cn.d;
+    f.cgb = cn.e;
+    f.cbb = cn.f;
     count_update(f.count);
   }
   return logw;
```

After: 18.14 billion, median of 2. 0.929x the previous value.
